# real-stanford/dgdm

Hardware: AMD Instinct MI355X
Metric: guided samples/sec (full DDIM chain) (higher is better)
Workload: dtype f32_split_f16x3; 1 GPU; 3d_guided BASELINE configs[2] (configs[3] at 8 GPUs): B=32 G=45 P=5 R=36000 sub_bs=512 N=512 T=15/S=5, fresh object per pair; contraction_flag=f32, fingers_per_pair=32, denoise_steps=5, rows_per_cond_fn=36000, cond_fn_per_chain_step=1, eps_net_form=f32_f16x3 batched, parallelism=pairs-sharded x1

## Files before the change

### dgdm_amd/_lib.py

```python
from __future__ import annotations

import ctypes as C
import os
from typing import Dict, List, Sequence

import numpy as np
import torch

_HERE = os.path.dirname(os.path.abspath(__file__))
LIB_PATH = os.path.join(_HERE, "csrc", "libdgdm_hip.so")

OK, EINVAL, EKEY, EHIP, EOBJECTIVE, EMODE, ENODEVICE = 0, -1, -2, -3, -4, -5, -6


class DgdmError(RuntimeError):
    pass


class Tensor(C.Structure):
    _fields_ = [("name", C.c_char_p), ("data", C.c_void_p), ("numel", C.c_int64), ("dtype", C.c_int32)]


class Objective(C.Structure):
    _fields_ = [("lin", C.c_float * 3), ("quad", C.c_float * 3), ("use_rowcoef", C.c_int32), ("object", C.c_int32)]


class GoalSpec(C.Structure):
    _fields_ = [("weight", C.c_float * 3), ("ori_window", C.c_float), ("pos_window", C.c_float), ("profile", C.c_int32)]


OBJ_ROWFIELD = 2


class TrainGroups(C.Structure):
    _fields_ = [("t_index_dev", C.c_void_p), ("t_values_dev", C.c_void_p), ("n_t", C.c_int32), ("rows_per_object", C.c_int32)]


class DynamicsStore(C.Structure):
    _fields_ = [("ctrl_dev", C.c_void_p), ("object_dev", C.c_void_p), ("scores_dev", C.c_void_p), ("ori_dev", C.c_void_p), ("pos_dev", C.c_void_p),
                ("object_of_sample_host", C.c_void_p), ("n_samples", C.c_int64), ("n_objects", C.c_int64), ("cells", C.c_int32),
                ("n_ctrl", C.c_int32), ("n_object_points", C.c_int32), ("fingers_3d", C.c_int32)]


class GuidanceConfig(C.Structure):
    _fields_ = [("batch", C.c_int32), ("grid_size", C.c_int32), ("num_pos", C.c_int32), ("ori_lo", C.c_float),
                ("ori_hi", C.c_float), ("max_chains", C.c_int32), ("num_train_timesteps", C.c_int32),
                ("sub_batch_size", C.c_int32), ("num_object_points", C.c_int32), ("max_objects", C.c_int32)]


_P = C.c_void_p
PROTOTYPES = {
    "dgdm_version": (C.c_int, []),
    "dgdm_last_error": (C.c_char_p, []),
    "dgdm_device_init": (C.c_int, [C.c_int]),
    "dgdm_objective_from_name": (C.c_int, [C.c_char_p, C.POINTER(Objective)]),
    "dgdm_unet1d_create": (C.c_int, [C.POINTER(_P), C.POINTER(Tensor), C.c_int, C.POINTER(C.c_int32), C.c_int, C.c_int, C.c_int, C.c_int]),
    "dgdm_unet1d_destroy": (None, [_P]),
    "dgdm_unet1d_forward": (C.c_int, [_P, _P, _P, _P, C.c_int, C.c_int, _P]),
    "dgdm_unet1d_global_cond_dim": (C.c_int, [_P]),
    "dgdm_unet1d_forward_cond": (C.c_int, [_P, _P, _P, _P, _P, C.c_int, C.c_int, _P]),
    "dgdm_cfg_mix": (C.c_int, [_P, _P, C.c_float, _P, C.c_int64, _P]),
    "dgdm_ddim_guided_step": (C.c_int, [_P, _P, _P, C.c_int, _P, C.c_int64, C.c_float, C.c_float, C.c_float, C.c_float, C.c_float, _P]),
    "dgdm_ddim_add_noise": (C.c_int, [_P, _P, _P, C.c_int64, C.c_float, C.c_float, _P]),
    "dgdm_dynamics_create": (C.c_int, [C.POINTER(_P), C.c_int, C.POINTER(Tensor), C.c_int, C.c_int, C.c_int]),
    "dgdm_dynamics_destroy": (None, [_P]),
    "dgdm_dyn2d_forward": (C.c_int, [_P, _P, _P, _P, _P, _P, _P, C.c_int, _P]),
    "dgdm_pointnet2_forward": (C.c_int, [_P, _P, _P, _P, _P, C.c_int, C.c_int, _P]),
    "dgdm_dyn3d_forward": (C.c_int, [_P, _P, _P, _P, _P, _P, _P, _P, _P, C.c_int, C.c_int, _P]),
    "dgdm_farthest_point_sample": (C.c_int, [_P, _P, C.c_int, C.c_int, C.c_int, _P, _P]),
    "dgdm_query_ball_point": (C.c_int, [C.c_float, C.c_int, _P, _P, C.c_int, C.c_int, C.c_int, _P, _P]),
    "dgdm_square_distance": (C.c_int, [_P, _P, C.c_int, C.c_int, C.c_int, _P, _P]),
    "dgdm_index_points": (C.c_int, [_P, _P, C.c_int, C.c_int, C.c_int, C.c_int, _P, _P]),
    "dgdm_linear_act": (C.c_int, [_P, C.c_int, _P, _P, _P, C.c_int, C.c_int, C.c_int, C.c_int, C.c_int, _P]),
    "dgdm_group_max": (C.c_int, [_P, C.c_int64, C.c_int, C.c_int, _P, _P]),
    "dgdm_guidance_create": (C.c_int, [C.POINTER(_P), _P, C.POINTER(GuidanceConfig)]),
    "dgdm_guidance_destroy": (None, [_P]),
    "dgdm_debug_chain_layer": (C.c_int, [_P, _P, _P, _P, _P]),
    "dgdm_unet1d_set_contraction_dtype": (C.c_int, [_P, C.c_int]),
    "dgdm_unet1d_effective_form": (C.c_int, [_P, C.c_int, C.c_int]),
    "dgdm_finger_decode_2d": (C.c_int, [_P, C.c_int, C.c_int, C.c_int, C.c_float, C.c_float, _P, _P]),
    "dgdm_finger_decode_3d": (C.c_int, [_P, C.c_int, C.c_int, C.c_int, C.c_float, C.c_float, _P, _P]),
    "dgdm_guidance_set_contraction_dtype": (C.c_int, [_P, C.c_int]),
    "dgdm_guidance_set_objects": (C.c_int, [_P, _P, C.c_int, _P]),
    "dgdm_guidance_rows": (C.c_int64, [_P]),
    "dgdm_guidance_starts_per_call": (C.c_int64, [_P]),
    "dgdm_dyn2d_guidance_grad": (C.c_int, [_P, _P, C.c_int, C.POINTER(Objective), _P, C.c_int, _P, _P]),
    "dgdm_dyn3d_guidance_grad": (C.c_int, [_P, _P, C.c_int, C.POINTER(Objective), _P, _P, C.c_int, _P, _P]),
    "dgdm_guidance_set_row_field": (C.c_int, [_P, _P, C.c_int, _P]),
    "dgdm_guidance_goal_field": (C.c_int, [_P, _P, C.POINTER(GoalSpec), C.c_int, _P, _P]),
    "dgdm_guidance_score": (C.c_int, [_P, _P, C.c_int, C.POINTER(C.c_int32), _P, C.POINTER(C.c_float), C.c_int, _P, _P, _P, _P]),
    "dgdm_guided_chains_run": (C.c_int, [_P, _P, _P, C.c_int, C.c_int, C.POINTER(Objective), _P, _P, C.POINTER(C.c_int32), C.POINTER(C.c_float),
                                         C.POINTER(C.c_float), C.c_int, _P, _P]),
    "dgdm_guided_chains_run_cond": (C.c_int, [_P, _P, _P, C.c_int, C.c_int, C.POINTER(Objective), _P, _P, C.POINTER(C.c_int32), C.POINTER(C.c_float),
                                              C.POINTER(C.c_float), C.c_int, _P, _P, C.c_int64, C.c_float, _P]),
    "dgdm_guidance_orientation_sweep": (C.c_int, [_P, _P, _P, _P, C.c_int, _P, _P]),
    "dgdm_guidance_rollout": (C.c_int, [_P, _P, C.POINTER(C.c_int32), _P, C.POINTER(C.c_double), C.c_int, C.c_int, _P, _P, _P, _P, _P, _P]),
    "dgdm_guidance_debug_rollout_table": (C.c_int, [_P, C.c_int, _P, _P, C.POINTER(C.c_int32), C.POINTER(C.c_int32), _P]),
    "dgdm_convergence_rowcoef": (C.c_int, [_P, C.c_int, C.c_int, C.c_int, C.c_int64, C.c_int64, _P]),
    "dgdm_torch_rng_seed": (C.c_int, [_P, C.c_int64, C.c_uint64]),
    "dgdm_torch_rng_randint": (C.c_int, [_P, C.c_int64, C.c_uint32, C.c_int64, _P]),
    "dgdm_torch_rng_fps_starts": (C.c_int, [_P, C.c_int64, C.c_int, C.c_int64, C.c_int64, C.c_int64, _P, C.c_int64]),
    "dgdm_prof_enable": (C.c_int, [C.c_int]),
    "dgdm_guidance_debug_fps_path": (C.c_int, [_P, C.c_int, C.POINTER(C.c_int32)]),
    "dgdm_debug_pointnet_indices": (C.c_int, [_P, _P, C.c_int, _P, C.c_int, _P, _P, _P, _P, _P, _P, _P, _P]),
    "dgdm_guidance_debug_partials": (C.c_int, [_P, C.c_int, _P, C.POINTER(C.c_int32), C.POINTER(C.c_int32), _P]),
    "dgdm_prof_read_stage": (C.c_int, [C.c_int, C.POINTER(C.c_int64), C.POINTER(C.c_double), C.POINTER(C.c_double)]),
    "dgdm_prof_read": (C.c_int, [C.POINTER(C.c_int64), C.POINTER(C.c_double), C.POINTER(C.c_double)]),
    "dgdm_trainer2d_create": (C.c_int, [C.POINTER(_P), C.POINTER(Tensor), C.c_int, C.c_int, C.c_int, C.c_float, C.c_float, C.c_float, C.c_float]),
    "dgdm_trainer2d_destroy": (None, [_P]),
    "dgdm_trainer2d_step": (C.c_int, [_P, _P, _P, _P, _P, _P, _P, _P, _P, _P, C.c_int64, C.c_float, C.c_int, _P, C.POINTER(C.c_float), _P]),
    "dgdm_trainer2d_forward_backward": (C.c_int, [_P, _P, _P, _P, _P, _P, _P, _P, _P, _P, C.c_int64, C.c_int64, _P, C.POINTER(C.c_float), _P]),
    "dgdm_trainer2d_set_groups": (C.c_int, [_P, C.POINTER(TrainGroups)]),
    "dgdm_trainer2d_gradient_count": (C.c_int64, [_P]),
    "dgdm_trainer2d_gradients": (C.c_int, [_P, _P, C.c_int64, C.c_int, _P]),
    "dgdm_trainer2d_apply": (C.c_int, [_P, C.c_float, _P]),
    "dgdm_trainer2d_running_stats": (C.c_int, [_P, _P, C.c_int64, C.c_int, _P]),
    "dgdm_trainer2d_export": (C.c_int, [_P, C.c_int, C.POINTER(Tensor), C.c_int]),
    "dgdm_trainer2d_steps": (C.c_int64, [_P]),
    "dgdm_dynamics_batch_rows": (C.c_int, [C.POINTER(DynamicsStore), _P, C.c_int, _P, _P, _P, _P, _P, _P, _P]),
    "dgdm_class_agreement": (C.c_int, [_P, _P, C.c_int64, C.POINTER(C.c_float), _P, _P]),
    "dgdm_unet_trainer_create": (C.c_int, [C.POINTER(_P), C.POINTER(Tensor), C.c_int, C.c_int, C.POINTER(C.c_int32), C.c_int, C.c_int, C.c_int, C.c_int,
                                           C.c_float, C.c_float, C.c_float, C.c_float]),
    "dgdm_unet_trainer_destroy": (None, [_P]),
    "dgdm_unet_trainer_step": (C.c_int, [_P, _P, _P, _P, _P, _P, C.c_int, C.c_float, _P, C.POINTER(C.c_float), _P]),
    "dgdm_unet_trainer_forward_backward": (C.c_int, [_P, _P, _P, _P, _P, _P, C.c_int, C.c_int64, C.c_int, _P, C.POINTER(C.c_float), _P]),
    "dgdm_unet_trainer_step_cond": (C.c_int, [_P, _P, _P, _P, _P, _P, _P, C.c_int, C.c_float, _P, C.POINTER(C.c_float), _P]),
    "dgdm_unet_trainer_forward_backward_cond": (C.c_int, [_P, _P, _P, _P, _P, _P, _P, C.c_int, C.c_int64, C.c_int, _P, C.POINTER(C.c_float), _P]),
    "dgdm_unet_trainer_global_cond_dim": (C.c_int, [_P]),
    "dgdm_unet_trainer_gradient_count": (C.c_int64, [_P]),
    "dgdm_unet_trainer_gradients": (C.c_int, [_P, _P, C.c_int64, C.c_int, C.c_float, _P]),
    "dgdm_unet_trainer_apply": (C.c_int, [_P, C.c_float, _P]),
    "dgdm_unet_trainer_ema_step": (C.c_int, [_P, C.c_float, C.c_float, _P]),
    "dgdm_unet_trainer_export": (C.c_int, [_P, C.c_int, C.POINTER(Tensor), C.c_int]),
    "dgdm_unet_trainer_import": (C.c_int, [_P, C.c_int, C.POINTER(Tensor), C.c_int, C.c_int64]),
    "dgdm_unet_trainer_steps": (C.c_int64, [_P]),
    "dgdm_trainer3d_create": (C.c_int, [C.POINTER(_P), C.POINTER(Tensor), C.c_int, C.c_int, C.c_int, C.c_float, C.c_float, C.c_float, C.c_float]),
    "dgdm_trainer3d_destroy": (None, [_P]),
    "dgdm_trainer3d_step": (C.c_int, [_P, _P, _P, _P, _P, _P, _P, _P, _P, _P, _P, _P, C.c_int64, C.c_float, C.c_int, _P, C.POINTER(C.c_float), _P]),
    "dgdm_trainer3d_export": (C.c_int, [_P, C.c_int, C.POINTER(Tensor), C.c_int]),
    "dgdm_trainer3d_steps": (C.c_int64, [_P]),
    "dgdm_trainer3d_forward_backward": (C.c_int, [_P, _P, _P, _P, _P, _P, _P, _P, _P, _P, _P, _P, C.c_int64, C.c_int64, _P, C.POINTER(C.c_float), _P]),
    "dgdm_trainer3d_gradient_count": (C.c_int64, [_P]),
    "dgdm_trainer3d_gradients": (C.c_int, [_P, _P, C.c_int64, C.c_int, _P]),
    "dgdm_trainer3d_apply": (C.c_int, [_P, C.c_float, _P]),
    "dgdm_trainer3d_running_stats_count": (C.c_int64, [_P]),
    "dgdm_trainer3d_running_stats": (C.c_int, [_P, _P, C.c_int64, C.c_int, _P]),
    "dgdm_trainer3d_debug_read": (C.c_int, [_P, C.c_int, _P, C.c_int64, _P]),
    "dgdm_mesh_read_obj": (C.c_int, [C.c_char_p, C.POINTER(_P)]),
    "dgdm_mesh_num_vertices": (C.c_int64, [_P]),
    "dgdm_mesh_num_triangles": (C.c_int64, [_P]),
    "dgdm_mesh_copy": (C.c_int, [_P, _P, _P]),
    "dgdm_mesh_destroy": (None, [_P]),
    "dgdm_mesh_sample_workspace_bytes": (C.c_int64, [_P, C.c_int]),
    "dgdm_mesh_sample_points": (C.c_int, [_P, _P, _P, _P, C.c_int, C.c_uint64, _P, C.c_int64, _P, _P, C.c_int64, _P]),
    "dgdm_finger_mesh_counts": (C.c_int, [C.c_int, C.c_int, C.POINTER(C.c_int64), C.POINTER(C.c_int64)]),
    "dgdm_finger_mesh_faces": (C.c_int, [C.c_int, C.c_int, _P]),
    "dgdm_finger_mesh_vertices_2d": (C.c_int, [_P, C.c_int, C.c_int, C.c_int, C.c_float, C.c_float, C.c_float, C.c_float, _P, _P]),
    "dgdm_finger_mesh_vertices_3d": (C.c_int, [_P, C.c_int, C.c_int, C.c_int, C.c_float, C.c_float, C.c_float, _P, _P]),
    "dgdm_finger_mesh_stats": (C.c_int, [_P, _P, C.c_int64, C.c_int, C.c_int, C.c_double, _P, _P]),
    "dgdm_finger_pieces_2d": (C.c_int, [_P, C.c_int, C.c_int, C.c_int, _P, _P, _P]),
    "dgdm_finger_pieces_3d": (C.c_int, [_P, C.c_int, C.c_int, C.c_int, C.c_int, _P, _P, _P]),
    "dgdm_mesh_write_obj": (C.c_int, [C.c_char_p, _P, C.c_int64, _P, C.c_int64]),
    "dgdm_icon_workspace_bytes": (C.c_int64, [C.c_int]),
    "dgdm_icon_trace": (C.c_int, [_P, C.c_int, C.c_int, C.c_int, C.c_int, _P, C.c_int64, _P, _P]),
    "dgdm_icon_fetch_contours": (C.c_int, [_P, C.c_int64, C.c_int, _P, _P, _P, C.c_int64, _P]),
    "dgdm_contour_resample_workspace_bytes": (C.c_int64, [_P, C.c_int]),
    "dgdm_contour_resample": (C.c_int, [_P, _P, C.c_int, C.c_int, C.c_int, _P, _P, C.c_int64, _P]),
    "dgdm_polygon_triangulate": (C.c_int, [_P, C.c_int, C.c_int, _P, _P, _P, _P, _P, _P]),
    "dgdm_polygon_convex_pieces": (C.c_int, [_P, C.c_int, C.c_int, _P, _P, _P, _P, _P, _P, _P, _P, _P]),
    "dgdm_render_workspace_bytes": (C.c_int64, [_P, _P, C.c_int, _P, C.c_int, C.c_int]),
    "dgdm_render_meshes": (C.c_int, [_P, _P, _P, _P, C.c_int, _P, _P, _P, _P, _P, _P, C.c_int, C.c_int, C.c_int, C.c_int, _P, _P, _P, _P, _P, _P,
                                     C.c_int64, _P]),
}

_lib = None


def lib() -> C.CDLL:
    global _lib
    if _lib is None:
        if not os.path.exists(LIB_PATH):
            raise DgdmError(f"{LIB_PATH} is missing: the HIP library has not been built (run `python -m dgdm_amd.build`). "
                            "dgdm_amd has no CPU fallback.")
        _lib = C.CDLL(LIB_PATH)
        for name, (res, args) in PROTOTYPES.items():
            fn = getattr(_lib, name)
            fn.restype, fn.argtypes = res, args
    return _lib


def check(rc: int) -> None:
    if rc == OK:
        return
    msg = lib().dgdm_last_error().decode("utf-8", "replace")
    if rc == EOBJECTIVE:
        raise ValueError('opt obj not supported')
    if rc == EMODE:
        raise ValueError('model type not supported')
    raise DgdmError(f"libdgdm_hip error {rc}: {msg}")


def device_init(ordinal: int = 0) -> None:
    check(lib().dgdm_device_init(ordinal))


def stream_ptr() -> int:
    return torch.cuda.current_stream().cuda_stream


def dptr(t: torch.Tensor | None) -> int | None:
    if t is None:
        return None
    assert t.is_cuda and t.is_contiguous(), "device tensors handed to libdgdm_hip must be contiguous CUDA tensors"
    return t.data_ptr()


class PackedStateDict:

    def __init__(self, sd: Dict[str, torch.Tensor], strip_prefix: Sequence[str] = ("module.",)):
        self.keep: List[np.ndarray] = []
        self.names: List[bytes] = []
        items = []
        for k, v in sd.items():
            if not isinstance(v, torch.Tensor):
                continue
            for p in strip_prefix:
                if k.startswith(p):
# ... 16 lines not shown
```

### dgdm_amd/csrc/common.h

```cpp
#pragma once
#include <hip/hip_runtime.h>
#include <stdint.h>
#include <stdio.h>
#include <string>
#include <vector>
#include <map>

#include "../../include/dgdm_hip.h"

#define DGDM_MAX_CHAINS 256

namespace dgdm {

#if defined(__HIP_DEVICE_COMPILE__)
__device__ __forceinline__ float mul_rn(float a, float b) { float r; asm("v_mul_f32 %0, %1, %2" : "=v"(r) : "v"(a), "v"(b)); return r; }
__device__ __forceinline__ float add_rn(float a, float b) { float r; asm("v_add_f32 %0, %1, %2" : "=v"(r) : "v"(a), "v"(b)); return r; }
__device__ __forceinline__ float sub_rn(float a, float b) { float r; asm("v_sub_f32 %0, %1, %2" : "=v"(r) : "v"(a), "v"(b)); return r; }
#else
__device__ __forceinline__ float mul_rn(float a, float b) { return a * b; }
__device__ __forceinline__ float add_rn(float a, float b) { return a + b; }
__device__ __forceinline__ float sub_rn(float a, float b) { return a - b; }
#endif

void set_error(const char *fmt, ...);

#define DGDM_HIP_CHECK(expr)                                                              \
    do {                                                                                  \
        hipError_t _e = (expr);                                                           \
        if (_e != hipSuccess) {                                                           \
            dgdm::set_error("%s failed: %s (%s:%d)", #expr, hipGetErrorString(_e), __FILE__, __LINE__); \
            return DGDM_EHIP;                                                             \
        }                                                                                 \
    } while (0)

#define DGDM_REQUIRE(cond, code, ...)                                                     \
    do {                                                                                  \
        if (!(cond)) {                                                                    \
            dgdm::set_error(__VA_ARGS__);                                                 \
            return (code);                                                                \
        }                                                                                 \
    } while (0)

struct DevBuf {
    void  *p = nullptr;
    size_t bytes = 0;
    DevBuf() = default;
    DevBuf(const DevBuf &) = delete;
    DevBuf &operator=(const DevBuf &) = delete;
    ~DevBuf() { if (p) (void)hipFree(p); }
    int alloc(size_t n) {
        if (p && bytes >= n) return DGDM_OK;
        if (p) { (void)hipFree(p); p = nullptr; bytes = 0; }
        if (n == 0) return DGDM_OK;
        DGDM_HIP_CHECK(hipMalloc(&p, n));
        bytes = n;
        return DGDM_OK;
    }
    int upload(const void *host, size_t n) {
        int rc = alloc(n);
        if (rc) return rc;
        DGDM_HIP_CHECK(hipMemcpy(p, host, n, hipMemcpyHostToDevice));
        return DGDM_OK;
    }
    template <class T> T *as() const { return reinterpret_cast<T *>(p); }
};

struct StateDict {
    std::map<std::string, const DgdmTensor *> m;
    StateDict(const DgdmTensor *t, int n) { for (int i = 0; i < n; ++i) m[t[i].name] = &t[i]; }
    const float *f32(const std::string &k, int64_t numel) const;
    bool has(const std::string &k) const { return m.count(k) != 0; }
};

struct Folded {
    int out = 0, in = 0;
    std::vector<float> w;
    std::vector<float> b;
};
int fold_linear(const StateDict &sd, const std::string &lin, const std::string &bn , int out, int in,
                Folded *dst);
struct Folded64 {
    int out = 0, in = 0;
    std::vector<double> w;
    std::vector<double> b;
};
int fold_linear64(const StateDict &sd, const std::string &lin, const std::string &bn , int out, int in, Folded64 *dst);
std::vector<double> transpose64(const double *src, int rows, int cols);
std::vector<double> pack_mfma64(const double *src, int M, int K);

std::vector<float> pack_chain(const float *src, int M, int K);
uint16_t f32_to_bf16(float x);
std::vector<uint16_t> pack_chain_bf16(const float *src, int M, int K);
std::vector<float> transpose(const float *src, int rows, int cols);

constexpr int PROF_BUCKETS = DGDM_STAGE_COUNT;
void prof_begin(hipStream_t s, int stage);
void prof_end(hipStream_t s, int stage, double work);

}
```

### dgdm_amd/csrc/debug.hip

```cpp
#include "common.h"
#include "mfma_chain.h"
#include "models.h"
#include "smallnet.h"

namespace dgdm {
__global__ __launch_bounds__(64, 1) void debug_chain_kernel(const float4 *__restrict__ Wimg, const float *__restrict__ bias,
                                                           const float *__restrict__ X, float *__restrict__ Y) {
    const int lane = threadIdx.x & 63, n = lane & 31, h4 = (lane >> 5) * 4;
    f32x16 in[8], out[8];
#pragma unroll
    for (int o = 0; o < 8; ++o)
#pragma unroll
        for (int q = 0; q < 4; ++q) {
            const float4 v = feat4(X + n * 256, o, q, h4);
            in[o][4 * q + 0] = v.x; in[o][4 * q + 1] = v.y; in[o][4 * q + 2] = v.z; in[o][4 * q + 3] = v.w;
        }
    chain_layer<8, 8, CHAIN_BIAS>(Wimg, bias, in, out, lane);
#pragma unroll
    for (int o = 0; o < 8; ++o)
#pragma unroll
        for (int q = 0; q < 4; ++q) {
            float4 v;
            v.x = out[o][4 * q + 0]; v.y = out[o][4 * q + 1]; v.z = out[o][4 * q + 2]; v.w = out[o][4 * q + 3];
            *reinterpret_cast<float4 *>(Y + n * 256 + 32 * o + 8 * q + h4) = v;
        }
}
}

extern "C" int dgdm_debug_chain_layer(const float *W_host, const float *bias_host, const float *X_dev, float *Y_dev, void *stream) {
    using namespace dgdm;
    std::vector<float> img = pack_chain(W_host, 256, 256);
    DevBuf dw, db;
    int rc;
    if ((rc = dw.upload(img.data(), img.size() * 4)) || (rc = db.upload(bias_host, 256 * 4))) return rc;
    hipLaunchKernelGGL(debug_chain_kernel, dim3(1), dim3(64), 0, (hipStream_t)stream, dw.as<float4>(), db.as<float>(), X_dev, Y_dev);
    DGDM_HIP_CHECK(hipGetLastError());
    DGDM_HIP_CHECK(hipStreamSynchronize((hipStream_t)stream));
    return DGDM_OK;
}

extern "C" int dgdm_debug_pointnet_indices(DgdmDynamics *m, const float *xyz_dev, int N, const int32_t *perm_dev, int perm_len,
                                           int32_t *fps512_dev, int32_t *fps128_dev, int32_t *fps128_flags_dev, int32_t *ball1_dev,
                                           int32_t *ball2_dev, int32_t *ball2_count_dev, int32_t *crowded_dev, void *stream) {
    using namespace dgdm;
    DGDM_REQUIRE(m && xyz_dev && perm_dev && fps512_dev && fps128_dev && fps128_flags_dev && ball1_dev && ball2_dev && ball2_count_dev && crowded_dev,
                 DGDM_EINVAL, "dgdm_debug_pointnet_indices: null argument");
    if (m->kind != 3) { set_error("model type not supported: PointNet++ belongs to the 3-D model"); return DGDM_EMODE; }
    DGDM_REQUIRE(N >= 128 && N <= 1024 && perm_len > 0 && perm_len <= N, DGDM_EINVAL, "dgdm_debug_pointnet_indices: N %d / perm_len %d unsupported", N, perm_len);
    hipStream_t s = (hipStream_t)stream;
    int rc;
    if ((rc = pn_fps_tables(xyz_dev, N, N, fps512_dev, fps128_dev, fps128_flags_dev, s))) return rc;
    return pn_debug_indices(xyz_dev, N, m->pn(), perm_dev, perm_len, ball1_dev, ball2_dev, ball2_count_dev, crowded_dev, s);
}

extern "C" int dgdm_farthest_point_sample(const float *xyz_dev, const int64_t *start_host, int B, int N, int npoint, int32_t *out_dev, void *stream) {
    using namespace dgdm;
    DGDM_REQUIRE(xyz_dev && start_host && out_dev && B >= 0 && npoint > 0, DGDM_EINVAL, "dgdm_farthest_point_sample: bad argument");
    DGDM_REQUIRE(N > 0 && N <= 1024, DGDM_EINVAL, "clouds of %d points unsupported (1..1024)", N);
    if (B == 0) return DGDM_OK;
    std::vector<int> st(B);
    for (int i = 0; i < B; ++i) {
        DGDM_REQUIRE(start_host[i] >= 0 && start_host[i] < N, DGDM_EINVAL, "FPS start %lld outside [0, %d)", (long long)start_host[i], N);
        st[i] = (int)start_host[i];
    }
    DevBuf d;
    int rc;
    if ((rc = d.upload(st.data(), sizeof(int) * B))) return rc;
    if ((rc = pn_fps_rows(xyz_dev, d.as<int>(), B, N, npoint, out_dev, (hipStream_t)stream))) return rc;
    DGDM_HIP_CHECK(hipStreamSynchronize((hipStream_t)stream));
    return DGDM_OK;
}

extern "C" int dgdm_query_ball_point(float radius_squared, int nsample, const float *xyz_dev, const float *new_xyz_dev, int B, int N, int S, int32_t *out_dev,
                                     void *stream) {
    using namespace dgdm;
    DGDM_REQUIRE(xyz_dev && new_xyz_dev && out_dev && B >= 0 && N > 0 && S >= 0 && nsample > 0, DGDM_EINVAL, "dgdm_query_ball_point: bad argument");
    if (B == 0 || S == 0) return DGDM_OK;
    return pn_ball_rows(xyz_dev, new_xyz_dev, B, N, S, radius_squared, nsample, out_dev, (hipStream_t)stream);
}

extern "C" int dgdm_square_distance(const float *src_dev, const float *dst_dev, int B, int S, int N, float *out_dev, void *stream) {
    using namespace dgdm;
    DGDM_REQUIRE(src_dev && dst_dev && out_dev && B >= 0 && S >= 0 && N >= 0, DGDM_EINVAL, "dgdm_square_distance: bad argument");
    if (B == 0 || S == 0 || N == 0) return DGDM_OK;
    return pn_sqdist_rows(src_dev, dst_dev, B, S, N, out_dev, (hipStream_t)stream);
}

extern "C" int dgdm_index_points(const float *points_dev, const int32_t *idx_dev, int B, int N, int M, int C, float *out_dev, void *stream) {
    using namespace dgdm;
    DGDM_REQUIRE(points_dev && idx_dev && out_dev && B >= 0 && N > 0 && M >= 0 && C > 0, DGDM_EINVAL, "dgdm_index_points: bad argument");
    if (B == 0 || M == 0) return DGDM_OK;
    return pn_index_rows(points_dev, idx_dev, B, N, M, C, out_dev, (hipStream_t)stream);
}


namespace dgdm {
__global__ void group_max_kernel(const float *__restrict__ x, int64_t G, int ns, int C, float *__restrict__ out) {
    const int64_t e = (int64_t)blockIdx.x * blockDim.x + threadIdx.x;
    if (e >= G * C) return;
    const int64_t g = e / C;
    const int c = (int)(e - g * C);
    const float *p = x + g * ns * C + c;
    float best = p[0];
    for (int n = 1; n < ns; ++n) best = fmaxf(best, p[(int64_t)n * C]);
    out[e] = best;
}
}

extern "C" int dgdm_linear_act(const float *x_dev, int ldx, const float *wt_dev, const float *bias_dev, float *y_dev, int ldy, int rows, int K, int N, int act,
                               void *stream) {
    using namespace dgdm;
    DGDM_REQUIRE(x_dev && wt_dev && y_dev && rows >= 0 && K > 0 && N > 0 && ldx >= K && ldy >= N, DGDM_EINVAL, "dgdm_linear_act: bad argument");
    DGDM_REQUIRE(act == ACT_NONE || act == ACT_RELU || act == ACT_SILU, DGDM_EINVAL, "dgdm_linear_act: activation %d", act);
    return linear(x_dev, ldx, wt_dev, bias_dev, nullptr, 1, y_dev, ldy, rows, K, N, act, false, (hipStream_t)stream);
}

extern "C" int dgdm_group_max(const float *x_dev, int64_t groups, int nsample, int C, float *out_dev, void *stream) {
    using namespace dgdm;
    DGDM_REQUIRE(x_dev && out_dev && groups >= 0 && nsample > 0 && C > 0, DGDM_EINVAL, "dgdm_group_max: bad argument");
    if (groups == 0) return DGDM_OK;
    hipLaunchKernelGGL(group_max_kernel, dim3((unsigned)((groups * C + 255) / 256)), dim3(256), 0, (hipStream_t)stream, x_dev, groups, nsample, C, out_dev);
    DGDM_HIP_CHECK(hipGetLastError());
    return DGDM_OK;
}
```

### dgdm_amd/csrc/guidance_api.hip

```cpp
#include "common.h"
#include "models.h"
#include <algorithm>
#include <cmath>
#include <cstring>
#include <unordered_map>
#include <atomic>
#include <thread>

using namespace dgdm;

namespace {

std::vector<float> linspace_f32(float start, float end, int steps) {
    std::vector<float> v(steps);
    if (steps == 1) { v[0] = start; return v; }
    const float step = (end - start) / (float)(steps - 1);
    const int half = steps / 2;
    for (int i = 0; i < steps; ++i) v[i] = i < half ? start + step * (float)i : end - step * (float)(steps - i - 1);
    return v;
}

struct ObjectTables {
    const float *xyz = nullptr;
    const int   *fps1 = nullptr;
    const int   *fps2 = nullptr;
    const int   *flags = nullptr;
    DevBuf Z;
    bool   fast_ok = false;
    int *crowded = nullptr, *clist = nullptr;
    DevBuf M0, cl2, cnt2;
    DevBuf cl2s;
    DevBuf cl2o;
    DevBuf pcf;
    DevBuf X, X16;
    bool   has_x = false, has_x16 = false;
    int    ncr = 0;
    DevBuf Z16, M0_16;
    bool   has16 = false;
};

struct PoseGrid {
    DevBuf tab, tiled;
    DevBuf pmax;
    int cells = 0, tiles_per_b = 0;
    int64_t rows = 0;
};

}

struct DgdmGuidance {
    DgdmDynamics *m = nullptr;
    DgdmGuidanceConfig cfg{};
    int B = 0;
    PoseGrid grid, sweep;
    DevBuf objpart;
    DevBuf objtmp;
    std::vector<std::unique_ptr<ObjectTables>> tables;
    bool bf16 = false;
    bool f32_mfma = false;
    static constexpr int NBUILD = 3;
    DevBuf pool_crowded, pool_clist, pool_off, pool_pairs, pool_rank, pool_F1, pool_U;
    DevBuf pool_xyz, pool_fps1, pool_fps2, pool_flags, pool_ncr;
    DevBuf tmpY[NBUILD], tmpL2[NBUILD], vlist;
    DevBuf tmpShare[NBUILD];
    hipStream_t bstream[NBUILD] = {};
    hipEvent_t bev[NBUILD] = {}, bstart = nullptr, pooled = nullptr, ldone = nullptr;
    DevBuf V, genc, atab, chainbias, timepart, ttmp, ttmp64, partial, objdev, objidx, xobj, xobj16, starts, order, xchains, todo, groupoff;
    DevBuf loopx[2], loopeps, loopgrad, loopxrep, loopts;
    DevBuf loopcond, loopx2, loopeps2;
    DevBuf scorelogits;
    DevBuf sweep_ori, rollstate, rolllogits, rolltiles, rollpmax;
    const float *rowfield = nullptr;
    int rowfield_chains = 0;
    DevBuf pos_lin, goalspecs;
    int rolltiles_chains = 0;
    DevBuf xidx, xidxchains, xtabptrs;
    bool xtab_enabled = true;
    int xtab_policy = 0;
    int grads_since_set = 0;
    static constexpr int XTAB_AFTER = 5;
    int l2_gather_mode = 0;
    int xobj_mode = 0;
    int n_objects = 0;
    bool force_slow_xobj = false;
    void *pinned = nullptr; size_t pinned_bytes = 0; hipEvent_t pinned_ev = nullptr;
    int64_t todo_capacity = 0;
    int *ro_host = nullptr; size_t ro_ints = 0; hipEvent_t ro_ev = nullptr; bool ro_pending = false;
    int finish_objects();
    hipStream_t cstream = nullptr; hipEvent_t up_ready = nullptr, up_consumed = nullptr; bool consumed_recorded = false;
    ~DgdmGuidance() {
        if (pinned) (void)hipHostFree(pinned);
        if (pinned_ev) (void)hipEventDestroy(pinned_ev);
        if (ro_host) (void)hipHostFree(ro_host);
        if (ro_ev) (void)hipEventDestroy(ro_ev);
        if (cstream) (void)hipStreamDestroy(cstream);
        if (up_ready) (void)hipEventDestroy(up_ready);
        if (up_consumed) (void)hipEventDestroy(up_consumed);
        for (int i = 0; i < NBUILD; ++i) {
            if (bstream[i]) (void)hipStreamDestroy(bstream[i]);
            if (bev[i]) (void)hipEventDestroy(bev[i]);
        }
        if (bstart) (void)hipEventDestroy(bstart);
        if (ldone) (void)hipEventDestroy(ldone);
        if (pooled) (void)hipEventDestroy(pooled);
    }
    int build_pose_table(const std::vector<float> &ori, const std::vector<float> &pos, PoseGrid *dst, hipStream_t s);
    void set_grid(dgdm::TrunkParams *p, const PoseGrid &g, int n_chains) const;
    int check_objects(const int *oidx, int n_chains) const;
    bool tables_wanted() const { return xtab_enabled && !force_slow_xobj && xobj_mode == 0; }
    int common_pre(const float *x_dev, float t_scaled, const int *objidx_host, int n_chains, hipStream_t s);
    int upload_starts(const int64_t *starts_host, int n_chains, int64_t rows, hipStream_t s, bool need_order = true, int n_calls = 1,
                      int64_t call_stride = 0);
    int ensure_rows(int n_chains, int64_t rows_per_chain);
    int use_xtab(const int *objidx_host, int n_chains, int64_t rows, bool want16, hipStream_t s);
    int build_object(int oi, int slot, hipStream_t s);
    int build_xtab(int oi, hipStream_t s);
    int run_xobj(const int *objidx_host, int n_chains, int64_t rows, bool want16, bool *used16, bool *via_tab, hipStream_t s);
    struct Embedded {
        bool tab = false, used16 = false;
        int64_t rows_per_chain = 0;
        void point(dgdm::TrunkParams *p, const DgdmGuidance &g, int call, int64_t rows_per_call) const;
    };
    int embed_rows(const int *objidx_host, int n_chains, const int64_t *starts_host, int64_t rows_per_call, int n_calls, int64_t call_stride,
                   bool want16, Embedded *e, hipStream_t s);
    int embed(const int *objidx_host, int n_chains, const int64_t *starts_host, int n_calls, int64_t call_stride, Embedded *e, hipStream_t s);
    int trunk_front(int kind, const float *x_dev, int timestep, const int *objidx_host, const int64_t *starts_host, int n_chains, const Embedded *emb,
                    int call, dgdm::TrunkParams *p, hipStream_t s);
};

int DgdmGuidance::build_pose_table(const std::vector<float> &ori, const std::vector<float> &pos, PoseGrid *dst, hipStream_t s) {
    const int n = (int)ori.size(), W1 = m->W1;
    dst->cells = n; dst->tiles_per_b = (n + 31) / 32; dst->rows = (int64_t)B * n;
    DevBuf d_ori, d_pos, d_emb;
    int rc;
    if ((rc = d_ori.upload(ori.data(), sizeof(float) * n))) return rc;
    if ((rc = d_pos.upload(pos.data(), sizeof(float) * 2 * n))) return rc;
    if ((rc = d_emb.alloc(sizeof(float) * 27 * n))) return rc;
    if ((rc = dst->tab.alloc(sizeof(float) * (size_t)W1 * n))) return rc;
    if ((rc = pose_embed(d_ori.as<float>(), d_pos.as<float>(), d_emb.as<float>(), n, s))) return rc;
    if ((rc = linear64(d_emb.as<float>(), nullptr, 27, m->blob64.at(m->off64.w1p_wt), nullptr, nullptr, 1, nullptr, dst->tab.as<float>(), W1, n, 27, W1, ACT_NONE, s))) return rc;
    if ((rc = dst->tiled.alloc(sizeof(float) * (size_t)W1 * dst->tiles_per_b * 32))) return rc;
    if ((rc = tile_table(dst->tab.as<float>(), n, W1, dst->tiled.as<float>(), s))) return rc;
    DGDM_HIP_CHECK(hipStreamSynchronize(s));
    return DGDM_OK;
}

void DgdmGuidance::set_grid(TrunkParams *p, const PoseGrid &g, int n_chains) const {
    p->Atab = atab.as<float>(); p->Ptab = g.tab.as<float>(); p->PtabT = g.tiled.as<float>(); p->Pmax = g.pmax.as<float>();
    p->B = B; p->C = g.cells; p->tiles_per_b = g.tiles_per_b; p->ntiles = n_chains * B * g.tiles_per_b; p->R = g.rows;
    p->xstride = g.rows;
}

int DgdmGuidance::check_objects(const int *oidx, int n_chains) const {
    DGDM_REQUIRE(n_objects > 0, DGDM_EINVAL, "dgdm_guidance_set_objects has not been called");
    for (int i = 0; i < n_chains; ++i)
        DGDM_REQUIRE(oidx[i] >= 0 && oidx[i] < n_objects, DGDM_EINVAL, "chain %d refers to object %d of %d", i, oidx[i], n_objects);
    return DGDM_OK;
}

extern "C" int dgdm_guidance_create(DgdmGuidance **out, DgdmDynamics *model, const DgdmGuidanceConfig *cfg) {
    DGDM_REQUIRE(out && model && cfg, DGDM_EINVAL, "dgdm_guidance_create: null argument");
    DGDM_REQUIRE(cfg->batch > 0 && cfg->grid_size > 0 && cfg->num_pos > 0 && cfg->max_chains > 0 && cfg->num_train_timesteps > 0,
                 DGDM_EINVAL, "dgdm_guidance_create: bad config");
    DGDM_REQUIRE(cfg->max_chains <= DGDM_MAX_CHAINS, DGDM_EINVAL, "max_chains %d > %d", cfg->max_chains, DGDM_MAX_CHAINS);
    if (model->kind == 3) {
        DGDM_REQUIRE(cfg->sub_batch_size > 0, DGDM_EINVAL, "3-D guidance needs sub_batch_size (it partitions the FPS start draws)");
        DGDM_REQUIRE(cfg->num_object_points > 0 && cfg->num_object_points <= 1024, DGDM_EINVAL, "object clouds of %d points unsupported (1..1024)", cfg->num_object_points);
    } else {
        DGDM_REQUIRE(2 * cfg->num_object_points == model->object_ch, DGDM_EINVAL, "2*num_object_points (%d) != object_ch (%d)", 2 * cfg->num_object_points, model->object_ch);
    }
    std::unique_ptr<DgdmGuidance> g(new DgdmGuidance());
    g->m = model; g->cfg = *cfg;
    g->B = cfg->batch;
    const int G = cfg->grid_size, P = cfg->num_pos, C = G * P * P;
    const std::vector<float> lo = linspace_f32(cfg->ori_lo, cfg->ori_hi, G), lp = linspace_f32(-1.f, 1.f, P);
    std::vector<float> ori(C), pos(2 * (size_t)C);
    for (int gi = 0; gi < G; ++gi)
        for (int a = 0; a < P; ++a)
            for (int b = 0; b < P; ++b) {
                const int c = (gi * P + a) * P + b;
                ori[c] = lo[gi]; pos[2 * c] = lp[a]; pos[2 * c + 1] = lp[b];
            }
    int rc;
    if ((rc = g->build_pose_table(ori, pos, &g->grid, nullptr))) return rc;
    {
        std::vector<float> tab((size_t)C * model->W1), mx(C, 0.f);
        DGDM_HIP_CHECK(hipMemcpy(tab.data(), g->grid.tab.p, tab.size() * sizeof(float), hipMemcpyDeviceToHost));
        for (int c = 0; c < C; ++c)
            for (int j = 0; j < model->W1; ++j) mx[c] = std::max(mx[c], std::fabs(tab[(size_t)c * model->W1 + j]));
        if ((rc = g->grid.pmax.upload(mx.data(), mx.size() * sizeof(float)))) return rc;
    }
    std::vector<float> pos0(2 * (size_t)G, 0.f);
    if ((rc = g->build_pose_table(lo, pos0, &g->sweep, nullptr))) return rc;
    if ((rc = g->sweep_ori.upload(lo.data(), lo.size() * sizeof(float)))) return rc;
    if ((rc = g->pos_lin.upload(lp.data(), lp.size() * sizeof(float)))) return rc;
    const int W1 = model->W1, nc = cfg->max_chains;
    const size_t rows = (size_t)nc * g->B;
    const int64_t R = g->grid.rows;
    if ((rc = g->V.alloc(rows * 256 * 8)) || (rc = g->genc.alloc(rows * 256 * 8)) || (rc = g->atab.alloc(rows * W1 * 4)) ||
        (rc = g->chainbias.alloc((size_t)nc * W1 * 8)) || (rc = g->timepart.alloc((size_t)W1 * 8)) || (rc = g->ttmp.alloc(768 * 4)) ||
        (rc = g->ttmp64.alloc(512 * 8)) ||
        (rc = g->partial.alloc(rows * g->grid.tiles_per_b * W1 * 4)) || (rc = g->objdev.alloc(sizeof(TrunkObjective) * nc)) ||
        (rc = g->objidx.alloc(sizeof(int) * nc)))
        return rc;
    if (model->kind == 2) {
        if ((rc = g->objpart.alloc((size_t)std::max(1, cfg->max_objects) * W1 * 8))) return rc;
    } else {
        if ((rc = g->starts.alloc((size_t)nc * R * 2 * sizeof(int))) ||
            (rc = g->order.alloc((size_t)nc * R * sizeof(int))) || (rc = g->xchains.alloc(sizeof(XobjChain) * nc)) ||
            (rc = g->todo.alloc(((size_t)nc * R + 1) * sizeof(int))))
            return rc;
        g->todo_capacity = (int64_t)nc * R;
        g->pinned_bytes = ((size_t)nc * R * 3 + (size_t)nc * (cfg->num_object_points + 1)) * sizeof(int);
        if ((rc = g->groupoff.alloc((size_t)nc * (cfg->num_object_points + 1) * sizeof(int))) || (rc = g->xidx.alloc((size_t)nc * R * sizeof(int))) ||
            (rc = g->xidxchains.alloc(sizeof(XidxChain) * nc)) || (rc = g->xtabptrs.alloc(sizeof(void *) * nc)))
            return rc;
        DGDM_HIP_CHECK(hipHostMalloc(&g->pinned, g->pinned_bytes, hipHostMallocDefault));
        DGDM_HIP_CHECK(hipEventCreateWithFlags(&g->pinned_ev, hipEventDisableTiming));
    }
    *out = g.release();
    return DGDM_OK;
}

extern "C" void dgdm_guidance_destroy(DgdmGuidance *g) { delete g; }

extern "C" int dgdm_guidance_set_contraction_dtype(DgdmGuidance *g, int dtype) {
    DGDM_REQUIRE(g, DGDM_EINVAL, "dgdm_guidance_set_contraction_dtype: null handle");
    DGDM_REQUIRE(dtype >= DGDM_DTYPE_F32 && dtype <= DGDM_DTYPE_F32_F16X3, DGDM_EINVAL,
                 "contraction dtype %d unsupported (0 = f32 (default form), 1 = bf16, 2 = f32 on the float32 MFMA, 3 = f32 as 3 f16 products = the default form)", dtype);
    g->bf16 = dtype == DGDM_DTYPE_BF16;
    g->f32_mfma = dtype == DGDM_DTYPE_F32_MFMA;
    return DGDM_OK;
}

extern "C" int dgdm_guidance_debug_fps_path(DgdmGuidance *g, int force_per_row, int32_t *out_fast_ok) {
    DGDM_REQUIRE(g, DGDM_EINVAL, "dgdm_guidance_debug_fps_path: null handle");
    g->force_slow_xobj = force_per_row == 1;
    g->xobj_mode = force_per_row == 2 ? 2 : 0;
    g->l2_gather_mode = force_per_row == 4 ? 1 : 0;
    g->xtab_enabled = force_per_row == 0 || force_per_row == 4 || force_per_row == 5;
    g->xtab_policy = force_per_row == 5 ? 1 : 0;
    if (force_per_row == 3) g->xobj_mode = 0;
    if (out_fast_ok) {
        int rc = g->finish_objects();
        if (rc) return rc;
        for (int i = 0; i < g->n_objects && i < (int)g->tables.size(); ++i) out_fast_ok[i] = g->tables[i]->fast_ok ? 1 : 0;
    }
    return DGDM_OK;
}
__global__ void partials_true_units_kernel(float *p, const float *unit, size_t n, int W1) {
    const size_t i = (size_t)blockIdx.x * blockDim.x + threadIdx.x;
    if (i < n) p[i] *= unit[i % W1];
}
extern "C" int dgdm_guidance_debug_partials(DgdmGuidance *g, int n_chains, float *out_dev, int32_t *tiles_per_finger, int32_t *width, void *stream) {
    DGDM_REQUIRE(g && n_chains > 0 && n_chains <= g->cfg.max_chains, DGDM_EINVAL, "dgdm_guidance_debug_partials: bad argument");
    if (tiles_per_finger) *tiles_per_finger = g->grid.tiles_per_b;
    if (width) *width = g->m->W1;
    if (out_dev) {
        const size_t n = (size_t)n_chains * g->B * g->grid.tiles_per_b * g->m->W1;
        DGDM_HIP_CHECK(hipMemcpyAsync(out_dev, g->partial.p, n * sizeof(float), hipMemcpyDeviceToDevice, (hipStream_t)stream));
        hipLaunchKernelGGL(partials_true_units_kernel, dim3((unsigned)((n + 255) / 256)), dim3(256), 0, (hipStream_t)stream, out_dev, g->m->z1_unit.as<float>(), n, g->m->W1);
        DGDM_HIP_CHECK(hipGetLastError());
    }
    return DGDM_OK;
}
extern "C" int64_t dgdm_guidance_rows(const DgdmGuidance *g) { return g ? g->grid.rows : 0; }
extern "C" int64_t dgdm_guidance_starts_per_call(const DgdmGuidance *g) { return (g && g->m->kind == 3) ? 2 * g->grid.rows : 0; }

int DgdmGuidance::build_object(int oi, int slot, hipStream_t s) {
    const int N = cfg.num_object_points;
    ObjectTables &t = *tables[oi];
    const PnWeights w = m->pn();
    int rc;
    if ((rc = t.Z.alloc((size_t)N * N * 256 * 4)) ||
        (rc = t.M0.alloc((size_t)N * 256 * 4)) || (rc = t.cl2.alloc((size_t)N * 128 * sizeof(int))) || (rc = t.cnt2.alloc((size_t)N * sizeof(int))) ||
        (rc = t.cl2s.alloc((size_t)N * 128 * sizeof(int))) || (rc = t.cl2o.alloc((size_t)N * 256 * sizeof(unsigned short))) ||
        (rc = t.pcf.alloc((size_t)N * 512 * sizeof(int))))
        return rc;
    t.has16 = bf16;
    if (bf16 && ((rc = t.Z16.alloc((size_t)N * N * 128 * 4)) || (rc = t.M0_16.alloc((size_t)N * 128 * 4)))) return rc;
    uint32_t *z16 = bf16 ? t.Z16.as<uint32_t>() : nullptr;
    DevBuf &tY = tmpY[slot], &tL2 = tmpL2[slot];
    if ((rc = tY.alloc((size_t)N * N * 256 * 4)) || (rc = tL2.alloc((size_t)N * N * 256 * 4))) return rc;
    const float *xyz = t.xyz;
    const int *off = pool_off.as<int>() + (size_t)oi * (N + 1), *pairs = pool_pairs.as<int>() + (size_t)oi * N * N;
    const short *rank = pool_rank.as<short>() + (size_t)oi * N * N;
    const char *U = static_cast<const char *>(pool_U.p) + (size_t)oi * N * 128 * (bf16 ? 4 : 8);
    if (bf16) {
        if ((rc = pn_pairs(xyz, N, reinterpret_cast<const float *>(U), w, pairs, off, tY.as<float>(), tY.as<uint32_t>(), s))) return rc;
        if ((rc = pn_l2(xyz, N, w, t.fps1, vlist.as<int>(), N, tY.as<float>(), tL2.as<float>(), t.clist, t.clist + N,
                        off, rank, true, s, l2_gather_mode ? 0 : 1))) return rc;
        if ((rc = pn_z16(xyz, N, N, w, tL2.as<uint32_t>(), t.Z.as<float>(), z16, t.clist, t.clist + N, s))) return rc;
    } else {
        const PnWeights64 w64 = m->pn64();
        if ((rc = pn_pairs64(xyz, N, reinterpret_cast<const double *>(U), w64, pairs, off, tY.as<float>(), s))) return rc;
        const bool shared = !l2_gather_mode && N <= 512;
        L2Share sh{};
        if (shared) {
            const size_t NN = (size_t)N * N;
            if ((rc = tmpShare[slot].alloc(NN * 64 + NN + NN * sizeof(short) + NN * sizeof(int) + (2 * (size_t)N + 4) * sizeof(int)))) return rc;
            char *b = static_cast<char *>(tmpShare[slot].p);
            sh.sel = reinterpret_cast<unsigned char *>(b); b += NN * 64;
            sh.items = reinterpret_cast<int *>(b); b += NN * sizeof(int);
            sh.coff = reinterpret_cast<int *>(b); b += N * sizeof(int);
            sh.ccnt = reinterpret_cast<int *>(b); b += N * sizeof(int);
            sh.nitems = reinterpret_cast<int *>(b); b += 4 * sizeof(int);
            sh.rep = reinterpret_cast<short *>(b); b += NN * sizeof(short);
            sh.cnt = reinterpret_cast<unsigned char *>(b);
        }
        if ((rc = pn_l2(xyz, N, w, t.fps1, vlist.as<int>(), N, tY.as<float>(), tL2.as<float>(), t.clist, t.clist + N,
                        off, rank, false, s, shared ? 1 : 0, shared ? &sh : nullptr))) return rc;
        if ((rc = pn_z64(xyz, N, N, w64, tL2.as<float>(), t.Z.as<float>(), t.clist, t.clist + N, s, sh.items, sh.nitems))) return rc;
        if (shared && N > 1 && (rc = pn_zfill(N, N, t.Z.as<float>(), t.clist, t.clist + N, sh.rep, s))) return rc;
    }
    if ((rc = pn_m0(t.fps2, t.crowded, N, t.Z.as<float>(), t.M0.as<float>(), t.cl2.as<int>(), t.cnt2.as<int>(), z16,
                    bf16 ? t.M0_16.as<uint32_t>() : nullptr, t.clist, t.clist + N, t.cl2s.as<int>(), t.cl2o.as<unsigned short>(), s))) return rc;
    if ((rc = pn_pcf(t.fps1, t.cnt2.as<int>(), t.flags, N, t.pcf.as<int>(), s))) return rc;
    t.has_x = t.has_x16 = false;
    return xtab_policy == 1 ? build_xtab(oi, s) : DGDM_OK;
}

int DgdmGuidance::build_xtab(int oi, hipStream_t s) {
    const int N = cfg.num_object_points;
    ObjectTables &t = *tables[oi];
    if (N < 128) return DGDM_OK;
    const bool b16 = t.has16;
    int rc;
    if (b16) { if ((rc = t.X16.alloc((size_t)N * N * 128 * 4))) return rc; }
    else if ((rc = t.X.alloc((size_t)N * N * 256 * 4))) return rc;
    XtabObj xo{};
    xo.xyz = t.xyz; xo.fps1 = t.fps1; xo.Z = t.Z.as<float>(); xo.M0 = t.M0.as<float>();
    xo.Z16 = b16 ? t.Z16.as<uint32_t>() : nullptr; xo.M0_16 = b16 ? t.M0_16.as<uint32_t>() : nullptr;
    xo.clist = t.clist; xo.ncr = t.clist + N; xo.cl2s = t.cl2s.as<int>(); xo.cnt2 = t.cnt2.as<int>(); xo.flags = t.flags;
    xo.crowded = t.crowded; xo.X = b16 ? nullptr : t.X.as<float>(); xo.X16 = b16 ? t.X16.as<uint32_t>() : nullptr; xo.N = N;
    if ((rc = pn_xtab(xo, b16, s))) return rc;
    (b16 ? t.has_x16 : t.has_x) = true;
    return DGDM_OK;
}

extern "C" int dgdm_guidance_set_objects(DgdmGuidance *g, const float *objects_dev, int n_objects, void *stream) {
    DGDM_REQUIRE(g && objects_dev && n_objects > 0, DGDM_EINVAL, "dgdm_guidance_set_objects: bad argument");
    DGDM_REQUIRE(n_objects <= std::max(1, g->cfg.max_objects), DGDM_EINVAL, "%d objects > max_objects %d", n_objects, g->cfg.max_objects);
    hipStream_t s = (hipStream_t)stream;
    int rc;
    prof_begin(s, DGDM_STAGE_TABLES);
    if (g->m->kind == 2) {
        if ((rc = g->objtmp.alloc((size_t)n_objects * 512 * 8))) return rc;
        if ((rc = g->m->object_part_2d64(objects_dev, g->objtmp.as<double>(), g->objpart.as<double>(), n_objects, s))) return rc;
        prof_end(s, DGDM_STAGE_TABLES, 0.0);
    } else {
        while ((int)g->tables.size() < n_objects) g->tables.emplace_back(new ObjectTables());
        const int N = g->cfg.num_object_points;
        if (g->vlist.bytes < (size_t)N * sizeof(int)) {
            std::vector<int> v(N);
            for (int i = 0; i < N; ++i) v[i] = i;
            if ((rc = g->vlist.upload(v.data(), sizeof(int) * N))) return rc;
        }
        const int nb = std::min<int>(DgdmGuidance::NBUILD, n_objects);
        if (!g->bstart) DGDM_HIP_CHECK(hipEventCreateWithFlags(&g->bstart, hipEventDisableTiming));
        if (!g->ldone) DGDM_HIP_CHECK(hipEventCreateWithFlags(&g->ldone, hipEventDisableTiming));
        for (int i = 0; i < nb; ++i) {
            if (!g->bstream[i]) DGDM_HIP_CHECK(hipStreamCreateWithFlags(&g->bstream[i], hipStreamNonBlocking));
            if (!g->bev[i]) DGDM_HIP_CHECK(hipEventCreateWithFlags(&g->bev[i], hipEventDisableTiming));
        }
        const size_t no = (size_t)n_objects;
        if ((rc = g->pool_xyz.alloc(no * N * 3 * 4)) || (rc = g->pool_fps1.alloc(no * N * 512 * sizeof(int))) ||
            (rc = g->pool_fps2.alloc(no * N * 128 * sizeof(int))) || (rc = g->pool_flags.alloc(no * N * sizeof(int))) ||
            (rc = g->pool_ncr.alloc(no * sizeof(int))) || (rc = g->pool_crowded.alloc(no * N * sizeof(int))) ||
            (rc = g->pool_clist.alloc(no * (N + 1) * sizeof(int))) || (rc = g->pool_off.alloc(no * (N + 1) * sizeof(int))) ||
            (rc = g->pool_pairs.alloc(no * N * N * sizeof(int))) || (rc = g->pool_rank.alloc(no * N * N * sizeof(short))) ||
            (rc = g->pool_F1.alloc(no * N * 128 * 8)) || (rc = g->pool_U.alloc(no * N * 128 * 8)))
            return rc;
        if (!g->pooled) DGDM_HIP_CHECK(hipEventCreateWithFlags(&g->pooled, hipEventDisableTiming));
        DGDM_HIP_CHECK(hipMemcpyAsync(g->pool_xyz.p, objects_dev, no * N * 3 * 4, hipMemcpyDeviceToDevice, s));
        DGDM_HIP_CHECK(hipEventRecord(g->pooled, s));
        if ((rc = pn_fps_tables(g->pool_xyz.as<float>(), N, N, g->pool_fps1.as<int>(), g->pool_fps2.as<int>(), g->pool_flags.as<int>(), s, n_objects)))
            return rc;
        for (int i = 0; i < n_objects; ++i) {
            ObjectTables &t = *g->tables[i];
            t.xyz = g->pool_xyz.as<float>() + (size_t)i * N * 3; t.fps1 = g->pool_fps1.as<int>() + (size_t)i * N * 512;
            t.fps2 = g->pool_fps2.as<int>() + (size_t)i * N * 128; t.flags = g->pool_flags.as<int>() + (size_t)i * N;
            t.crowded = g->pool_crowded.as<int>() + (size_t)i * N; t.clist = g->pool_clist.as<int>() + (size_t)i * (N + 1);
        }
        {
            hipStream_t ls = g->bstream[0];
            DGDM_HIP_CHECK(hipStreamWaitEvent(ls, g->pooled, 0));
            const PnWeights w = g->m->pn();
            if ((rc = pn_crowd(g->pool_xyz.as<float>(), N, w, g->pool_crowded.as<int>(), g->pool_clist.as<int>(), g->pool_clist.as<int>() + N,
                               g->pool_off.as<int>(), g->pool_pairs.as<int>(), g->pool_rank.as<short>(), ls, g->pool_ncr.as<int>(), n_objects)))
                return rc;
            if (g->bf16) {
                if ((rc = pn_sa1(g->pool_xyz.as<float>(), N, w, g->pool_F1.as<float>(), ls, n_objects))) return rc;
                if ((rc = linear(g->pool_F1.as<float>(), 128, w.sa2_wf_t, w.sa2_b0, nullptr, 1, g->pool_U.as<float>(), 128, n_objects * N, 128, 128,
                                 ACT_NONE, false, ls))) return rc;
            } else {
                const PnWeights64 w64 = g->m->pn64();
                if ((rc = pn_sa1_64(g->pool_xyz.as<float>(), N, w.r1sq, w64, g->pool_F1.as<double>(), ls, n_objects))) return rc;
                if ((rc = linear64(nullptr, g->pool_F1.as<double>(), 128, w64.sa2_wf_t, w64.sa2_b0, nullptr, 1, g->pool_U.as<double>(), nullptr, 128,
                                   n_objects * N, 128, 128, ACT_NONE, ls))) return rc;
            }
            DGDM_HIP_CHECK(hipEventRecord(g->ldone, ls));
        }
        DGDM_HIP_CHECK(hipEventRecord(g->bstart, s));
        for (int i = 0; i < nb; ++i) {
            DGDM_HIP_CHECK(hipStreamWaitEvent(g->bstream[i], g->bstart, 0));
            DGDM_HIP_CHECK(hipStreamWaitEvent(g->bstream[i], g->ldone, 0));
        }
        for (int i = 0; i < n_objects; ++i)
            if ((rc = g->build_object(i, i % nb, g->bstream[i % nb]))) return rc;
        for (int i = 0; i < nb; ++i) {
            DGDM_HIP_CHECK(hipEventRecord(g->bev[i], g->bstream[i]));
            DGDM_HIP_CHECK(hipStreamWaitEvent(s, g->bev[i], 0));
        }
        prof_end(s, DGDM_STAGE_TABLES, 0.0);
        const size_t need = no * N + no;
        if (need > g->ro_ints) {
            if (g->ro_host) DGDM_HIP_CHECK(hipHostFree(g->ro_host));
            g->ro_host = nullptr;
            DGDM_HIP_CHECK(hipHostMalloc(reinterpret_cast<void **>(&g->ro_host), need * sizeof(int), hipHostMallocDefault));
            g->ro_ints = need;
        }
        if (!g->ro_ev) DGDM_HIP_CHECK(hipEventCreateWithFlags(&g->ro_ev, hipEventDisableTiming));
        DGDM_HIP_CHECK(hipMemcpyAsync(g->ro_host, g->pool_flags.p, sizeof(int) * no * N, hipMemcpyDeviceToHost, s));
        DGDM_HIP_CHECK(hipMemcpyAsync(g->ro_host + no * N, g->pool_ncr.p, sizeof(int) * no, hipMemcpyDeviceToHost, s));
        DGDM_HIP_CHECK(hipEventRecord(g->ro_ev, s));
        g->ro_pending = true;
    }
    g->n_objects = n_objects;
    g->grads_since_set = 0;
    return DGDM_OK;
}

int DgdmGuidance::common_pre(const float *x_dev, float t_scaled, const int *objidx_host, int n_chains, hipStream_t s) {
    const int rows = n_chains * B, W1 = m->W1;
    int rc;
    if ((rc = m->gripper_forward64(x_dev, m->L, V.as<double>(), genc.as<double>(), rows, s))) return rc;
    if ((rc = m->time_part64(t_scaled, ttmp.as<float>(), ttmp64.as<double>(), timepart.as<double>(), s))) return rc;
    if (m->kind == 2) {
        DGDM_HIP_CHECK(hipMemcpyAsync(objidx.p, objidx_host, sizeof(int) * n_chains, hipMemcpyHostToDevice, s));
        if ((rc = gather_add64(objpart.as<double>(), objidx.as<int>(), timepart.as<double>(), chainbias.as<double>(), n_chains, W1, s))) return rc;
        return linear64(nullptr, genc.as<double>(), 256, m->blob64.at(m->off64.w1c_wt), nullptr, chainbias.as<double>(), B, nullptr, atab.as<float>(), W1, rows, 256, W1,
                        ACT_NONE, s);
    }
    return linear64(nullptr, genc.as<double>(), 256, m->blob64.at(m->off64.w1c_wt), timepart.as<double>(), nullptr, 1, nullptr, atab.as<float>(), W1, rows, 256, W1,
                    ACT_NONE, s);
}

int DgdmGuidance::finish_objects() {
    if (!ro_pending) return DGDM_OK;
    DGDM_HIP_CHECK(hipEventSynchronize(ro_ev));
    const int N = cfg.num_object_points;
    for (int i = 0; i < n_objects; ++i) {
        bool ok = N >= 128;
        for (int k = 0; k < N; ++k) ok = ok && ro_host[(size_t)i * N + k] == 0;
        tables[i]->fast_ok = ok;
        tables[i]->ncr = ro_host[(size_t)n_objects * N + i];
    }
    ro_pending = false;
    return DGDM_OK;
}

int DgdmGuidance::ensure_rows(int n_chains, int64_t rows_per_chain) {
    const int N = cfg.num_object_points;
    const size_t nr = (size_t)n_chains * rows_per_chain;
    int rc;
    if ((rc = starts.alloc(nr * 2 * sizeof(int))) || (rc = order.alloc(nr * sizeof(int))) ||
        (rc = todo.alloc((nr + 1) * sizeof(int))) || (rc = xidx.alloc(nr * sizeof(int))))
        return rc;
    todo_capacity = (int64_t)nr;
    const size_t need = (nr * 3 + (size_t)n_chains * (N + 1)) * sizeof(int);
    if (need > pinned_bytes) {
        if (pinned) { DGDM_HIP_CHECK(hipEventSynchronize(pinned_ev)); DGDM_HIP_CHECK(hipHostFree(pinned)); pinned = nullptr; pinned_bytes = 0; }
        DGDM_HIP_CHECK(hipHostMalloc(&pinned, need, hipHostMallocDefault));
        pinned_bytes = need;
    }
    return DGDM_OK;
}

int DgdmGuidance::upload_starts(const int64_t *starts_host, int n_chains, int64_t rows, hipStream_t s, bool need_order, int n_calls,
                                int64_t call_stride) {
    const int N = cfg.num_object_points;
    const int64_t sb = cfg.sub_batch_size;
    const int64_t rt = rows * n_calls;
    int rc;
    DGDM_REQUIRE(!need_order || rt < ((int64_t)1 << 22), DGDM_EINVAL, "%lld rows per chain in one gather launch (limit 4194303)", (long long)rt);
    if ((rc = ensure_rows(n_chains, rt))) return rc;
    DGDM_HIP_CHECK(hipEventSynchronize(pinned_ev));
    int *dst = static_cast<int *>(pinned);
    int *ord = dst + (size_t)n_chains * 2 * rt;
    int *goff = ord + (size_t)n_chains * rt;
    std::atomic<int> bad{0};
    auto work = [&](int c0, int c1) {
        std::vector<int> cnt(N + 1), cnt2(513), tmp;
        for (int c = c0; c < c1; ++c) {
            int *d = dst + (size_t)c * 2 * rt;
            for (int k = 0; k < n_calls; ++k) {
                const int64_t *src = starts_host + (size_t)k * call_stride + (size_t)c * 2 * rows;
                int *dk = d + 2 * (size_t)k * rows;
                for (int64_t r0 = 0; r0 < rows; r0 += sb) {
                    const int64_t n = std::min(sb, rows - r0);
                    const int64_t *s1 = src + 2 * r0, *s2 = s1 + n;
                    for (int64_t i = 0; i < n; ++i) {
                        const int64_t a = s1[i], b = s2[i];
                        if (!(a >= 0 && a < N && b >= 0 && b < 512)) { bad.store(1); return; }
                        dk[2 * (r0 + i)] = (int)a; dk[2 * (r0 + i) + 1] = (int)b;
                    }
                }
            }
            if (!need_order) continue;
            int *o = ord + (size_t)c * rt;
            tmp.resize((size_t)rt);
            std::fill(cnt2.begin(), cnt2.end(), 0);
            for (int64_t r = 0; r < rt; ++r) ++cnt2[d[2 * r + 1] + 1];
            for (int k = 0; k < 512; ++k) cnt2[k + 1] += cnt2[k];
            for (int64_t r = 0; r < rt; ++r) tmp[cnt2[d[2 * r + 1]]++] = (int)r;
            std::fill(cnt.begin(), cnt.end(), 0);
            for (int64_t r = 0; r < rt; ++r) ++cnt[d[2 * r] + 1];
            for (int k = 0; k < N; ++k) cnt[k + 1] += cnt[k];
            memcpy(goff + (size_t)c * (N + 1), cnt.data(), sizeof(int) * (N + 1));
            for (int64_t i = 0; i < rt; ++i) { const int r = tmp[i]; o[cnt[d[2 * r]]++] = r | (d[2 * r + 1] << 22); }
        }
    };
    const int hw = (int)std::max(2u, std::thread::hardware_concurrency());
    const int nthreads = (int)std::min<int64_t>(std::min(16, hw / 2), std::max<int64_t>(1, std::min<int64_t>(n_chains, (int64_t)n_chains * rt / 65536)));
    if (nthreads <= 1) {
        work(0, n_chains);
    } else {
        std::vector<std::thread> pool;
        for (int t = 0; t < nthreads; ++t) pool.emplace_back(work, (int)((int64_t)n_chains * t / nthreads), (int)((int64_t)n_chains * (t + 1) / nthreads));
        for (auto &th : pool) th.join();
    }
    DGDM_REQUIRE(!bad.load(), DGDM_EINVAL, "FPS start out of range (sa1 must be in [0, %d), sa2 in [0, 512))", N);
    if (!cstream) {
        DGDM_HIP_CHECK(hipStreamCreateWithFlags(&cstream, hipStreamNonBlocking));
        DGDM_HIP_CHECK(hipEventCreateWithFlags(&up_ready, hipEventDisableTiming));
        DGDM_HIP_CHECK(hipEventCreateWithFlags(&up_consumed, hipEventDisableTiming));
    }
    if (consumed_recorded) DGDM_HIP_CHECK(hipStreamWaitEvent(cstream, up_consumed, 0));
    DGDM_HIP_CHECK(hipMemcpyAsync(starts.p, pinned, (size_t)n_chains * rt * 2 * sizeof(int), hipMemcpyHostToDevice, cstream));
    if (need_order) {
        DGDM_HIP_CHECK(hipMemcpyAsync(order.p, ord, (size_t)n_chains * rt * sizeof(int), hipMemcpyHostToDevice, cstream));
        DGDM_HIP_CHECK(hipMemcpyAsync(groupoff.p, goff, (size_t)n_chains * (N + 1) * sizeof(int), hipMemcpyHostToDevice, cstream));
    }
    DGDM_HIP_CHECK(hipEventRecord(pinned_ev, cstream));
    DGDM_HIP_CHECK(hipEventRecord(up_ready, cstream));
    DGDM_HIP_CHECK(hipStreamWaitEvent(s, up_ready, 0));
    return DGDM_OK;
}

int DgdmGuidance::use_xtab(const int *objidx_host, int n_chains, int64_t rows, bool want16, hipStream_t s) {
    std::vector<XidxChain> xc(n_chains);
    std::vector<const void *> base(n_chains);
    for (int i = 0; i < n_chains; ++i) {
        const ObjectTables &t = *tables[objidx_host[i]];
        xc[i].fps1 = t.fps1; xc[i].N = cfg.num_object_points; xc[i].m0_only = t.ncr == 0;
        base[i] = want16 ? (t.ncr == 0 ? (const void *)t.M0_16.p : (const void *)t.X16.p) : (t.ncr == 0 ? (const void *)t.M0.p : (const void *)t.X.p);
    }
    DGDM_HIP_CHECK(hipMemcpyAsync(xidxchains.p, xc.data(), sizeof(XidxChain) * n_chains, hipMemcpyHostToDevice, s));
    DGDM_HIP_CHECK(hipMemcpyAsync(xtabptrs.p, base.data(), sizeof(void *) * n_chains, hipMemcpyHostToDevice, s));
    return pn_xidx(xidxchains.as<XidxChain>(), starts.as<int>(), rows, n_chains, xidx.as<int>(), s);
}

int DgdmGuidance::run_xobj(const int *objidx_host, int n_chains, int64_t rows, bool want16, bool *used16, bool *via_tab, hipStream_t s) {
    *via_tab = false;
    std::vector<XobjChain> ch(n_chains);
    for (int i = 0; i < n_chains; ++i) {
        const ObjectTables &t = *tables[objidx_host[i]];
        ch[i].xyz = t.xyz; ch[i].fps1 = t.fps1; ch[i].slot_of_start = nullptr; ch[i].Z = t.Z.as<float>();
        ch[i].fps2 = t.fps2; ch[i].flags = t.flags; ch[i].crowded = t.crowded; ch[i].N = cfg.num_object_points;
        ch[i].M0 = t.M0.as<float>(); ch[i].cl2 = t.cl2.as<int>(); ch[i].cnt2 = t.cnt2.as<int>();
        ch[i].Z16 = t.has16 ? t.Z16.as<uint32_t>() : nullptr; ch[i].M0_16 = t.has16 ? t.M0_16.as<uint32_t>() : nullptr;
        want16 = want16 && t.has16;
    }
    {
        const size_t nrows = (size_t)n_chains * rows;
        int rc = want16 ? xobj16.alloc(nrows * 512) : xobj.alloc(nrows * 256 * 4);
        if (rc) return rc;
    }
    *used16 = want16;
    XobjParams xp{};
    xp.chains = xchains.as<XobjChain>(); xp.starts = starts.as<int>(); xp.order = order.as<int>(); xp.xobj = xobj.as<float>();
    xp.xobj16 = want16 ? xobj16.as<uint32_t>() : nullptr;
    xp.R = rows; xp.total_rows = rows * n_chains; xp.use_table = force_slow_xobj ? 0 : 1;
    xp.todo = todo.as<int>(); xp.todo_count = todo.as<int>() + todo_capacity; xp.todo_capacity = todo_capacity;
    bool all_fast = true;
    for (int i = 0; i < n_chains; ++i) all_fast = all_fast && tables[objidx_host[i]]->fast_ok;
    bool groups = !force_slow_xobj && xobj_mode == 0 && cfg.num_object_points >= 128;
    for (int i = 0; i < n_chains && groups; ++i) {
        const ObjectTables &t = *tables[objidx_host[i]];
        const int lpr = xobj_rows_lpr(t.ncr, want16);
        groups = lpr > 0 && want16 == t.has16;
        ch[i].clist = t.clist; ch[i].cl2s = t.cl2s.as<int>(); ch[i].cl2o = t.cl2o.as<unsigned short>(); ch[i].pcf = t.pcf.as<int>(); ch[i].ncr = t.ncr; ch[i].lpr = lpr;
    }
    DGDM_HIP_CHECK(hipMemcpyAsync(xchains.p, ch.data(), sizeof(XobjChain) * n_chains, hipMemcpyHostToDevice, s));
    if (groups) {
        const bool by_index = tables_wanted() && (want16 || !bf16);
        std::vector<int> rank;
        std::vector<XidxChain> xc(n_chains);
        std::vector<const void *> base(n_chains);
        for (int i = 0; i < n_chains; ++i) {
            const ObjectTables &t = *tables[objidx_host[i]];
            const bool m0_only = by_index && t.ncr == 0 && t.fast_ok;
            if (!m0_only) rank.push_back(i);
            xc[i].fps1 = m0_only ? t.fps1 : nullptr; xc[i].N = cfg.num_object_points; xc[i].m0_only = 1;
            base[i] = m0_only ? (want16 ? (const void *)t.M0_16.p : (const void *)t.M0.p)
                              : (want16 ? (const void *)(xobj16.as<uint32_t>() + (size_t)i * rows * 128) : (const void *)(xobj.as<float>() + (size_t)i * rows * 256));
        }
        xp.group_off = groupoff.as<int>(); xp.nchain = n_chains; xp.group_N = cfg.num_object_points; xp.use_table = 1;
        xp.total_items = (int)rank.size() * xp.group_N;
        std::stable_sort(rank.begin(), rank.end(), [&](int a, int b) { return ch[a].ncr > ch[b].ncr; });
        for (size_t i = 0; i < rank.size(); ++i) xp.chain_of_rank[i] = (unsigned char)rank[i];
        int rc = pn_xobj_groups(xp, s);
        if (rc || !by_index) return rc;
        *via_tab = true;
        DGDM_HIP_CHECK(hipMemcpyAsync(xidxchains.p, xc.data(), sizeof(XidxChain) * n_chains, hipMemcpyHostToDevice, s));
        DGDM_HIP_CHECK(hipMemcpyAsync(xtabptrs.p, base.data(), sizeof(void *) * n_chains, hipMemcpyHostToDevice, s));
        return pn_xidx(xidxchains.as<XidxChain>(), starts.as<int>(), rows, n_chains, xidx.as<int>(), s);
    }
    return pn_xobj(xp, all_fast, s);
}

int DgdmGuidance::embed_rows(const int *oidx, int n_chains, const int64_t *starts_host, int64_t rows_per_call, int n_calls, int64_t call_stride,
                             bool want16, Embedded *e, hipStream_t s) {
    bool tab = tables_wanted();
    for (int i = 0; i < n_chains && tab; ++i) tab = want16 ? tables[oidx[i]]->has_x16 : tables[oidx[i]]->has_x;
    const int64_t rt = rows_per_call * n_calls;
    int rc;
    if ((rc = upload_starts(starts_host, n_chains, rows_per_call, s, !tab, n_calls, call_stride))) return rc;
    if ((rc = finish_objects())) return rc;
    e->tab = tab; e->used16 = want16; e->rows_per_chain = rt;
    if ((rc = tab ? use_xtab(oidx, n_chains, rt, want16, s) : run_xobj(oidx, n_chains, rt, want16, &e->used16, &e->tab, s))) return rc;
    DGDM_HIP_CHECK(hipEventRecord(up_consumed, s));
    consumed_recorded = true;
    return DGDM_OK;
}

void DgdmGuidance::Embedded::point(TrunkParams *p, const DgdmGuidance &g, int call, int64_t rows_per_call) const {
    const size_t row0 = (size_t)call * rows_per_call;
    p->xstride = rows_per_chain;
    if (tab) {
        p->xidx = g.xidx.as<int>() + row0;
        if (used16) p->xtab16 = g.xtabptrs.as<const uint32_t *>();
        else p->xtab = g.xtabptrs.as<const float *>();
    } else {
        p->xobj = g.xobj.as<float>() + row0 * 256;
        p->xobj16 = used16 ? g.xobj16.as<uint32_t>() + row0 * 128 : nullptr;
    }
}

int DgdmGuidance::embed(const int *oidx, int n_chains, const int64_t *starts_host, int n_calls, int64_t call_stride, Embedded *e, hipStream_t s) {
    DGDM_REQUIRE(starts_host, DGDM_EINVAL, "3-D guidance needs the FPS start indices");
    int rc;
    prof_begin(s, DGDM_STAGE_XOBJ);
    if (tables_wanted()) {
        const bool crosses = grads_since_set <= XTAB_AFTER && grads_since_set + n_calls > XTAB_AFTER;
        grads_since_set += n_calls;
        if (crosses)
            for (int i = 0; i < n_objects; ++i) {
                ObjectTables &t = *tables[i];
                if (!(t.has16 ? t.has_x16 : t.has_x) && (rc = build_xtab(i, s))) return rc;
            }
    }
    if ((rc = embed_rows(oidx, n_chains, starts_host, grid.rows, n_calls, call_stride, bf16, e, s))) return rc;
    prof_end(s, DGDM_STAGE_XOBJ, 0.0);
    return DGDM_OK;
}

int DgdmGuidance::trunk_front(int kind, const float *x_dev, int timestep, const int *oidx, const int64_t *starts_host, int n_chains, const Embedded *emb,
                              int call, TrunkParams *pp, hipStream_t s) {
    const float t_scaled = (float)timestep / (float)cfg.num_train_timesteps;
    int rc;
    if ((rc = check_objects(oidx, n_chains))) return rc;
    prof_begin(s, DGDM_STAGE_GUIDE_MISC);
    if ((rc = common_pre(x_dev, t_scaled, oidx, n_chains, s))) return rc;
    prof_end(s, DGDM_STAGE_GUIDE_MISC, 0.0);
    m->fill_trunk(pp);
    set_grid(pp, grid, n_chains);
    if (kind == 3) {
        Embedded own;
        if (!emb) {
            if ((rc = embed(oidx, n_chains, starts_host, 1, 0, &own, s))) return rc;
            emb = &own;
            call = 0;
        }
        emb->point(pp, *this, call, grid.rows);
    }
    return DGDM_OK;
}

static int check_objectives(const DgdmGuidance *g, const DgdmObjective *objectives, const float *rowcoef_dev, int n_chains) {
    for (int i = 0; i < n_chains; ++i) {
        const int u = objectives[i].use_rowcoef;
        DGDM_REQUIRE(u >= 0 && u <= DGDM_OBJ_ROWFIELD, DGDM_EINVAL, "chain %d: use_rowcoef %d (0, 1 or %d)", i, u, DGDM_OBJ_ROWFIELD);
        DGDM_REQUIRE(u != 1 || rowcoef_dev, DGDM_EINVAL, "chain %d uses rowcoef but rowcoef_dev is null", i);
        if (u == DGDM_OBJ_ROWFIELD) {
            DGDM_REQUIRE(g->rowfield, DGDM_EINVAL, "chain %d uses the row field but none is set (dgdm_guidance_set_row_field)", i);
            DGDM_REQUIRE(i < g->rowfield_chains, DGDM_EINVAL, "chain %d uses the row field, which was set for %d chains", i, g->rowfield_chains);
        }
    }
    return DGDM_OK;
}

static int guidance_grad(DgdmGuidance *g, int kind, const float *x_dev, int timestep, const DgdmObjective *objectives, const float *rowcoef_dev,
                         const int64_t *starts_host, int n_chains, float *grad_dev, hipStream_t s, const DgdmGuidance::Embedded *emb = nullptr,
                         int call = 0) {
    DGDM_REQUIRE(g && x_dev && objectives && grad_dev, DGDM_EINVAL, "guidance_grad: null argument");
    if (g->m->kind != kind) { set_error("model type not supported: %d-D entry point on a %d-D model", kind, g->m->kind); return DGDM_EMODE; }
    DGDM_REQUIRE(n_chains > 0 && n_chains <= g->cfg.max_chains, DGDM_EINVAL, "n_chains %d outside 1..%d", n_chains, g->cfg.max_chains);
    int rc;
    if ((rc = check_objectives(g, objectives, rowcoef_dev, n_chains))) return rc;
    std::vector<int> oidx(n_chains);
    std::vector<TrunkObjective> tob(n_chains);
    for (int i = 0; i < n_chains; ++i) {
        oidx[i] = objectives[i].object;
        for (int j = 0; j < 3; ++j) { tob[i].lin[j] = objectives[i].lin[j]; tob[i].quad[j] = objectives[i].quad[j]; }
        tob[i].use_rowcoef = objectives[i].use_rowcoef; tob[i].pad = 0;
    }
    TrunkParams p;
    if ((rc = g->trunk_front(kind, x_dev, timestep, oidx.data(), starts_host, n_chains, emb, call, &p, s))) return rc;
    DGDM_HIP_CHECK(hipMemcpyAsync(g->objdev.p, tob.data(), sizeof(TrunkObjective) * n_chains, hipMemcpyHostToDevice, s));
    p.obj = g->objdev.as<TrunkObjective>(); p.rowcoef = rowcoef_dev; p.rowfield = g->rowfield;
    p.partial = g->partial.as<float>();
    if (g->bf16) {
        g->m->fill_trunk_bf16(&p);
        if ((rc = trunk_bf16_launch(kind, p, s))) return rc;
    } else if (g->f32_mfma) {
        if ((rc = trunk_launch(kind, false, false, p, s))) return rc;
    } else {
        TrunkF16Scales sc;
        g->m->fill_trunk_f16(&p, &sc);
        if ((rc = trunk_f16l_launch(kind, TrunkF16Mode::Grad, p, sc, s))) return rc;
    }
    prof_begin(s, DGDM_STAGE_GUIDE_MISC);
    rc = dyn_post64(g->m->W1, g->partial.as<float>(), g->grid.tiles_per_b, g->m->blob64.at(g->m->off64.w1c_w), g->m->blob64.at(g->m->off64.g2_w),
                    g->m->blob64.at(g->m->off64.g0_w), g->V.as<double>(), grad_dev, n_chains * g->B, g->m->L, s);
    prof_end(s, DGDM_STAGE_GUIDE_MISC, 0.0);
    return rc;
}

extern "C" int dgdm_dyn2d_guidance_grad(DgdmGuidance *g, const float *x_dev, int timestep, const DgdmObjective *objectives,
                                        const float *rowcoef_dev, int n_chains, float *grad_dev, void *stream) {
    return guidance_grad(g, 2, x_dev, timestep, objectives, rowcoef_dev, nullptr, n_chains, grad_dev, (hipStream_t)stream);
}

extern "C" int dgdm_dyn3d_guidance_grad(DgdmGuidance *g, const float *x_dev, int timestep, const DgdmObjective *objectives,
                                        const float *rowcoef_dev, const int64_t *starts_host, int n_chains, float *grad_dev, void *stream) {
    return guidance_grad(g, 3, x_dev, timestep, objectives, rowcoef_dev, starts_host, n_chains, grad_dev, (hipStream_t)stream);
}

extern "C" int dgdm_guidance_set_row_field(DgdmGuidance *g, const float *field_dev, int n_chains, void *stream) {
    (void)stream;
    DGDM_REQUIRE(g, DGDM_EINVAL, "dgdm_guidance_set_row_field: null handle");
    if (!field_dev) { g->rowfield = nullptr; g->rowfield_chains = 0; return DGDM_OK; }
    DGDM_REQUIRE(n_chains > 0 && n_chains <= g->cfg.max_chains, DGDM_EINVAL, "dgdm_guidance_set_row_field: n_chains %d outside 1..%d", n_chains,
                 g->cfg.max_chains);
    g->rowfield = field_dev; g->rowfield_chains = n_chains;
    return DGDM_OK;
}

extern "C" int dgdm_guidance_goal_field(DgdmGuidance *g, const float *goals_dev, const DgdmGoalSpec *specs_host, int n_chains, float *field_dev,
                                        void *stream) {
    DGDM_REQUIRE(g && goals_dev && specs_host && field_dev, DGDM_EINVAL, "dgdm_guidance_goal_field: null argument");
    DGDM_REQUIRE(n_chains > 0 && n_chains <= g->cfg.max_chains, DGDM_EINVAL, "dgdm_guidance_goal_field: n_chains %d outside 1..%d", n_chains,
                 g->cfg.max_chains);
    hipStream_t s = (hipStream_t)stream;
    for (int i = 0; i < n_chains; ++i) {
        const DgdmGoalSpec &q = specs_host[i];
        DGDM_REQUIRE(q.ori_window > 0.f && q.ori_window <= 1.f, DGDM_EINVAL, "goal %d: ori_window %g outside (0, 1]", i, (double)q.ori_window);
        DGDM_REQUIRE(q.pos_window > 0.f && std::isfinite(q.pos_window), DGDM_EINVAL, "goal %d: pos_window %g is not a positive number", i, (double)q.pos_window);
        DGDM_REQUIRE(q.profile == 0 || q.profile == 1, DGDM_EINVAL, "goal %d: profile %d (0 sign, 1 linear)", i, q.profile);
        for (int j = 0; j < 3; ++j) DGDM_REQUIRE(std::isfinite(q.weight[j]), DGDM_EINVAL, "goal %d: weight %d is not finite", i, j);
    }
    std::vector<float> goals((size_t)n_chains * g->B * 3);
    DGDM_HIP_CHECK(hipMemcpyAsync(goals.data(), goals_dev, goals.size() * sizeof(float), hipMemcpyDeviceToHost, s));
    DGDM_HIP_CHECK(hipStreamSynchronize(s));
    for (size_t k = 0; k < goals.size(); ++k)
        DGDM_REQUIRE(std::isfinite(goals[k]), DGDM_EINVAL, "goal %d, finger %d: coordinate %d is not finite", (int)(k / ((size_t)g->B * 3)),
                     (int)(k / 3 % g->B), (int)(k % 3));
    int rc;
    if ((rc = g->goalspecs.alloc(sizeof(DgdmGoalSpec) * g->cfg.max_chains))) return rc;
    DGDM_HIP_CHECK(hipMemcpyAsync(g->goalspecs.p, specs_host, sizeof(DgdmGoalSpec) * n_chains, hipMemcpyHostToDevice, s));
    return goal_field_build(g->sweep_ori.as<float>(), g->pos_lin.as<float>(), goals_dev, g->goalspecs.as<DgdmGoalSpec>(), n_chains, g->B,
                            g->cfg.grid_size, g->cfg.num_pos, field_dev, s);
}

extern "C" int dgdm_guidance_score(DgdmGuidance *g, const float *x_dev, int timestep, const int32_t *object_of_chain, const int64_t *starts_host,
                                   const float thr[3], int n_chains, float *logits_dev, int32_t *counts_dev, float *sums_dev, void *stream) {
    DGDM_REQUIRE(g && x_dev && object_of_chain && thr && counts_dev && sums_dev, DGDM_EINVAL, "dgdm_guidance_score: null argument");
    DGDM_REQUIRE(!g->bf16, DGDM_EINVAL, "dgdm_guidance_score: the bf16 trunk has no forward-only form (contraction dtypes f32 / f32_f16x3 / f32_mfma)");
    hipStream_t s = (hipStream_t)stream;
    const int kind = g->m->kind;
    DGDM_REQUIRE(kind == 2 || starts_host, DGDM_EINVAL, "3-D scoring needs the FPS start indices");
    DGDM_REQUIRE(n_chains > 0 && n_chains <= g->cfg.max_chains, DGDM_EINVAL, "n_chains %d outside 1..%d", n_chains, g->cfg.max_chains);
    int rc;
    if (!logits_dev) {
        if ((rc = g->scorelogits.alloc((size_t)n_chains * g->grid.rows * 3 * sizeof(float)))) return rc;
        logits_dev = g->scorelogits.as<float>();
    }
    const std::vector<int> oidx(object_of_chain, object_of_chain + n_chains);
    TrunkParams p;
    if ((rc = g->trunk_front(kind, x_dev, timestep, oidx.data(), starts_host, n_chains, nullptr, 0, &p, s))) return rc;
    p.logits = logits_dev;
    if (g->f32_mfma) {
        if ((rc = trunk_launch(kind, false, true, p, s))) return rc;
    } else {
        TrunkF16Scales sc;
        g->m->fill_trunk_f16(&p, &sc);
        if ((rc = trunk_f16l_launch(kind, TrunkF16Mode::Forward, p, sc, s))) return rc;
    }
    return score_tally(logits_dev, n_chains, g->B, g->grid.cells, thr, counts_dev, sums_dev, s);
}

namespace {
__global__ void fill_i32_kernel(int *p, int v, int n) {
    const int i = blockIdx.x * blockDim.x + threadIdx.x;
    if (i < n) p[i] = v;
}
__global__ void repeat_rows_kernel(const float *__restrict__ src, float *__restrict__ dst, int64_t n_src, int reps) {
    const int64_t i = (int64_t)blockIdx.x * blockDim.x + threadIdx.x;
    if (i < n_src * reps) dst[i] = src[i % n_src];
}
__global__ void cfg_mix_kernel(const float *ec, const float *eu, float w, float *out, int64_t n) {
    const int64_t i = (int64_t)blockIdx.x * blockDim.x + threadIdx.x;
    if (i >= n) return;
    const float u = eu[i];
    out[i] = add_rn(u, mul_rn(w, sub_rn(ec[i], u)));
}
}

extern "C" int dgdm_cfg_mix(const float *eps_c_dev, const float *eps_u_dev, float w, float *out_dev, int64_t numel, void *stream) {
    DGDM_REQUIRE(eps_c_dev && eps_u_dev && out_dev && numel >= 0, DGDM_EINVAL, "dgdm_cfg_mix: bad argument");
    if (numel == 0) return DGDM_OK;
    hipLaunchKernelGGL(cfg_mix_kernel, dim3((unsigned)((numel + 255) / 256)), dim3(256), 0, (hipStream_t)stream, eps_c_dev, eps_u_dev, w, out_dev, numel);
    DGDM_HIP_CHECK(hipGetLastError());
    return DGDM_OK;
}

extern "C" int dgdm_guided_chains_run(DgdmUnet1d *unet, DgdmGuidance *g, const float *noise_dev, int n_chains, int n_grad,
                                      const DgdmObjective *objectives, const float *rowcoef_dev, const int64_t *starts_host,
                                      const int32_t *timesteps, const float *coef, const float *scales, int n_steps, float *x_out_dev,
                                      void *stream) {
    return dgdm_guided_chains_run_cond(unet, g, noise_dev, n_chains, n_grad, objectives, rowcoef_dev, starts_host, timesteps, coef, scales, n_steps, x_out_dev,
                                       nullptr, 0, 1.f, stream);
}

extern "C" int dgdm_guided_chains_run_cond(DgdmUnet1d *unet, DgdmGuidance *g, const float *noise_dev, int n_chains, int n_grad,
                                           const DgdmObjective *objectives, const float *rowcoef_dev, const int64_t *starts_host,
                                           const int32_t *timesteps, const float *coef, const float *scales, int n_steps, float *x_out_dev,
                                           const float *global_cond_dev, int64_t cond_chain_stride, float cfg_weight, void *stream) {
    DGDM_REQUIRE(unet && g && noise_dev && objectives && timesteps && coef && scales && x_out_dev, DGDM_EINVAL, "dgdm_guided_chains_run: null argument");
    DGDM_REQUIRE(n_chains > 0 && n_grad > 0 && n_chains * n_grad <= g->cfg.max_chains && n_steps > 0, DGDM_EINVAL,
                 "dgdm_guided_chains_run: %d chains x %d gradients outside 1..%d", n_chains, n_grad, g->cfg.max_chains);
    hipStream_t s = (hipStream_t)stream;
    const int B = g->B, L = g->m->L, kind = g->m->kind;
    const size_t per_chain = (size_t)B * L, nx = per_chain * n_chains, ng = nx * n_grad;
    DGDM_REQUIRE(kind == 2 || starts_host, DGDM_EINVAL, "3-D guidance needs the FPS start indices");
    const int gc = dgdm_unet1d_global_cond_dim(unet);
    DGDM_REQUIRE(gc == 0 || global_cond_dev, DGDM_EINVAL, "dgdm_guided_chains_run: the eps-net has global_cond_dim %d and needs a condition", gc);
    DGDM_REQUIRE(cfg_weight == cfg_weight && std::fabs(cfg_weight) <= 3.0e38f, DGDM_EINVAL, "dgdm_guided_chains_run: cfg_weight is not finite");
    const bool conditional = gc > 0;
    DGDM_REQUIRE(!conditional || cond_chain_stride == 0 || cond_chain_stride == (int64_t)B * gc, DGDM_EINVAL,
                 "dgdm_guided_chains_run: cond_chain_stride %lld is neither 0 (one [B][%d] block for all chains) nor B * gc = %lld", (long long)cond_chain_stride, gc,
                 (long long)B * gc);
    const bool per_chain_cond = conditional && cond_chain_stride != 0 && n_chains > 1;
    const int cfg = !conditional ? 1 : cfg_weight == 1.f ? 1 : cfg_weight == 0.f ? 0 : 2;
    int rc;
    if ((rc = check_objectives(g, objectives, rowcoef_dev, n_chains * n_grad))) return rc;
    if ((rc = g->loopx[0].alloc(nx * 4)) || (rc = g->loopx[1].alloc(nx * 4)) || (rc = g->loopeps.alloc(nx * 4)) || (rc = g->loopgrad.alloc(ng * 4)) ||
        (rc = g->loopxrep.alloc(ng * 4)) || (rc = g->loopts.alloc((size_t)2 * n_chains * B * sizeof(int))))
        return rc;
    const size_t ncond = (size_t)n_chains * B * gc;
    const float *cond_rows = nullptr, *zero_rows = nullptr;
    if (conditional) {
        if ((rc = g->loopcond.alloc(2 * ncond * 4))) return rc;
        float *cr = g->loopcond.as<float>();
        if (cond_chain_stride == 0) hipLaunchKernelGGL(repeat_rows_kernel, dim3((unsigned)((ncond + 255) / 256)), dim3(256), 0, s, global_cond_dev, cr, (int64_t)B * gc, n_chains);
        else DGDM_HIP_CHECK(hipMemcpyAsync(cr, global_cond_dev, ncond * 4, hipMemcpyDeviceToDevice, s));
        DGDM_HIP_CHECK(hipMemsetAsync(cr + ncond, 0, ncond * 4, s));
        cond_rows = cr; zero_rows = cr + ncond;
        if (cfg == 2 && ((rc = g->loopx2.alloc(2 * nx * 4)) || (rc = g->loopeps2.alloc(2 * nx * 4)))) return rc;
    }
    hipLaunchKernelGGL(repeat_rows_kernel, dim3((unsigned)((nx + 255) / 256)), dim3(256), 0, s, noise_dev, g->loopx[0].as<float>(), (int64_t)per_chain, n_chains);
    bool same_scale = true;
    for (int c = 1; c < n_chains; ++c) same_scale = same_scale && scales[c] == scales[0];
    const int64_t spc = kind == 3 ? 2 * g->grid.rows : 0;
    DgdmGuidance::Embedded emb;
    std::vector<int> oidx(n_chains * n_grad);
    const int64_t call_stride = (int64_t)n_chains * n_grad * spc;
    int cpe = kind == 3 ? (int)std::min<int64_t>(n_steps, std::max<int64_t>(1, (((int64_t)1 << 22) - 1) / std::max<int64_t>(1, g->grid.rows))) : n_steps;
    if (const char *e = getenv("DGDM_EMBED_CALLS")) cpe = std::max(1, std::min(cpe, atoi(e)));
    if (kind == 3) {
        for (int i = 0; i < n_chains * n_grad; ++i) oidx[i] = objectives[i].object;
        if ((rc = g->check_objects(oidx.data(), n_chains * n_grad))) return rc;
    }
    for (int si = 0; si < n_steps; ++si) {
        float *x = g->loopx[si & 1].as<float>(), *xn = (si + 1 == n_steps) ? x_out_dev : g->loopx[(si + 1) & 1].as<float>();
        const int t = timesteps[si];
        if (kind == 3 && si % cpe == 0 &&
            (rc = g->embed(oidx.data(), n_chains * n_grad, starts_host + (size_t)si * call_stride, std::min(cpe, n_steps - si), call_stride, &emb, s))) return rc;
        const int nb = (si == 0 && n_chains > 1 && !per_chain_cond) ? B : n_chains * B;
        const int ne = cfg == 2 ? 2 * nb : nb;
        hipLaunchKernelGGL(fill_i32_kernel, dim3((ne + 255) / 256), dim3(256), 0, s, g->loopts.as<int>(), t, ne);
        if (cfg == 2) {
            const size_t n = (size_t)nb * L, nc = (size_t)nb * gc;
            float *x2 = g->loopx2.as<float>(), *e2 = g->loopeps2.as<float>(), *c2 = g->loopcond.as<float>();
            DGDM_HIP_CHECK(hipMemcpyAsync(x2, x, n * 4, hipMemcpyDeviceToDevice, s));
            DGDM_HIP_CHECK(hipMemcpyAsync(x2 + n, x, n * 4, hipMemcpyDeviceToDevice, s));
            if (nc != ncond) DGDM_HIP_CHECK(hipMemsetAsync(c2 + nc, 0, nc * 4, s));
            if ((rc = dgdm_unet1d_forward_cond(unet, x2, g->loopts.as<int>(), c2, e2, 2 * nb, L, s))) return rc;
            if (nc != ncond) {
                if (cond_chain_stride == 0) hipLaunchKernelGGL(repeat_rows_kernel, dim3((unsigned)((ncond + 255) / 256)), dim3(256), 0, s, global_cond_dev, c2, (int64_t)B * gc, n_chains);
                else DGDM_HIP_CHECK(hipMemcpyAsync(c2, global_cond_dev, ncond * 4, hipMemcpyDeviceToDevice, s));
            }
            if ((rc = dgdm_cfg_mix(e2, e2 + n, cfg_weight, g->loopeps.as<float>(), (int64_t)n, s))) return rc;
        } else if ((rc = dgdm_unet1d_forward_cond(unet, x, g->loopts.as<int>(), cfg == 0 ? zero_rows : cond_rows, g->loopeps.as<float>(), nb, L, s))) return rc;
        if (nb != n_chains * B) {
            hipLaunchKernelGGL(repeat_rows_kernel, dim3((unsigned)((nx + 255) / 256)), dim3(256), 0, s, g->loopeps.as<float>(), g->loopgrad.as<float>(), (int64_t)per_chain, n_chains);
            DGDM_HIP_CHECK(hipMemcpyAsync(g->loopeps.p, g->loopgrad.p, nx * 4, hipMemcpyDeviceToDevice, s));
        }
        const float *xg = x;
        if (n_grad > 1) {
            hipLaunchKernelGGL(repeat_rows_kernel, dim3((unsigned)((ng + 255) / 256)), dim3(256), 0, s, x, g->loopxrep.as<float>(), (int64_t)nx, n_grad);
            xg = g->loopxrep.as<float>();
        }
        if ((rc = guidance_grad(g, kind, xg, t, objectives, rowcoef_dev, nullptr, n_chains * n_grad, g->loopgrad.as<float>(), s,
                                kind == 3 ? &emb : nullptr, si % cpe))) return rc;
        const float *cf = coef + 4 * si;
        if (same_scale) {
            if ((rc = dgdm_ddim_guided_step(x, g->loopeps.as<float>(), g->loopgrad.as<float>(), n_grad, xn, (int64_t)nx, cf[0], cf[1], cf[2], cf[3], scales[0], s))) return rc;
        } else {
            DGDM_REQUIRE(n_grad == 1, DGDM_EINVAL, "per-chain guidance scales with averaged gradients are not supported");
            for (int c = 0; c < n_chains; ++c)
                if ((rc = dgdm_ddim_guided_step(x + c * per_chain, g->loopeps.as<float>() + c * per_chain, g->loopgrad.as<float>() + c * per_chain, 1,
                                                xn + c * per_chain, (int64_t)per_chain, cf[0], cf[1], cf[2], cf[3], scales[c], s))) return rc;
        }
    }
    DGDM_HIP_CHECK(hipGetLastError());
    return DGDM_OK;
}

extern "C" int dgdm_guidance_orientation_sweep(DgdmGuidance *g, const float *x_dev, const int32_t *object_of_chain, const int64_t *starts_host,
                                               int n_chains, float *logits_dev, void *stream) {
    DGDM_REQUIRE(g && x_dev && object_of_chain && logits_dev, DGDM_EINVAL, "dgdm_guidance_orientation_sweep: null argument");
    DGDM_REQUIRE(n_chains > 0 && n_chains <= g->cfg.max_chains, DGDM_EINVAL, "n_chains %d outside 1..%d", n_chains, g->cfg.max_chains);
    hipStream_t s = (hipStream_t)stream;
    const int kind = g->m->kind;
    int rc;
    if ((rc = g->check_objects(object_of_chain, n_chains))) return rc;
    if ((rc = g->common_pre(x_dev, 0.f, object_of_chain, n_chains, s))) return rc;
    TrunkParams p;
    g->m->fill_trunk(&p);
    g->set_grid(&p, g->sweep, n_chains);
    if (kind == 3) {
        DGDM_REQUIRE(starts_host, DGDM_EINVAL, "3-D sweep needs the FPS start indices");
        DgdmGuidance::Embedded emb;
        if ((rc = g->embed_rows(object_of_chain, n_chains, starts_host, g->sweep.rows, 1, 0, false, &emb, s))) return rc;
        emb.point(&p, *g, 0, g->sweep.rows);
    }
    p.logits = logits_dev;
    return trunk_launch(kind, false, true, p, s);
}

extern "C" int dgdm_guidance_rollout(DgdmGuidance *g, const float *x_dev, const int32_t *object_of_chain, const int64_t *starts_host,
                                     const double scale[3], int n_interactions, int n_chains, double *final_dev, float *first_logits_dev,
                                     int32_t *left_dev, double *traj_pose_dev, float *traj_logits_dev, void *stream) {
    DGDM_REQUIRE(g && x_dev && object_of_chain && scale && final_dev && first_logits_dev && left_dev, DGDM_EINVAL, "dgdm_guidance_rollout: null argument");
    DGDM_REQUIRE(!g->bf16, DGDM_EINVAL, "dgdm_guidance_rollout: the bf16 trunk has no forward-only form (contraction dtypes f32 / f32_f16x3)");
    DGDM_REQUIRE(!g->f32_mfma, DGDM_EINVAL, "dgdm_guidance_rollout: the float32 MFMA trunk has no per-row pose form (contraction dtypes f32 / f32_f16x3)");
    DGDM_REQUIRE(n_interactions >= 1, DGDM_EINVAL, "dgdm_guidance_rollout: %d interactions (at least 1)", n_interactions);
    DGDM_REQUIRE(n_chains > 0 && n_chains <= g->cfg.max_chains, DGDM_EINVAL, "n_chains %d outside 1..%d", n_chains, g->cfg.max_chains);
    int rc;
    if ((rc = g->check_objects(object_of_chain, n_chains))) return rc;
    hipStream_t s = (hipStream_t)stream;
    const int kind = g->m->kind, K = n_interactions, W1 = g->m->W1, G = g->sweep.cells;
    DGDM_REQUIRE(kind == 2 || starts_host, DGDM_EINVAL, "3-D roll-out needs the FPS start indices");
    const int64_t Rs = g->sweep.rows, rows = (int64_t)n_chains * Rs;
    const int ntiles = n_chains * g->B * g->sweep.tiles_per_b;
    if ((rc = g->rollstate.alloc((size_t)rows * 3 * sizeof(double))) || (rc = g->rolltiles.alloc((size_t)ntiles * 32 * W1 * sizeof(float))) ||
        (kind == 3 && (rc = g->rollpmax.alloc((size_t)ntiles * 32 * sizeof(float)))) ||
        (!traj_logits_dev && (rc = g->rolllogits.alloc((size_t)rows * 3 * sizeof(float)))))
        return rc;
    if ((rc = g->common_pre(x_dev, 0.f, object_of_chain, n_chains, s))) return rc;
    TrunkParams p;
    g->m->fill_trunk(&p);
    DgdmGuidance::Embedded emb;
    if (kind == 3 && (rc = g->embed_rows(object_of_chain, n_chains, starts_host, Rs, K, (int64_t)n_chains * 2 * Rs, false, &emb, s))) return rc;
    TrunkF16Scales sc;
    g->m->fill_trunk_f16(&p, &sc);
    g->set_grid(&p, g->sweep, n_chains);
    p.Ptab = nullptr; p.PtabT = g->rolltiles.as<float>(); p.Pmax = kind == 3 ? g->rollpmax.as<float>() : nullptr;
    double *state = g->rollstate.as<double>();
    if ((rc = rollout_start(g->sweep_ori.as<float>(), n_chains, g->B, G, state, left_dev, traj_pose_dev, s))) return rc;
    g->rolltiles_chains = n_chains;
    for (int k = 0; k < K; ++k) {
        if ((rc = rollout_pose_table(state, g->m->blob64.at(g->m->off64.w1p_wt), W1, n_chains, g->B, G, g->rolltiles.as<float>(), p.Pmax ? g->rollpmax.as<float>() : nullptr, s)))
            return rc;
        p.logits = traj_logits_dev ? traj_logits_dev + (size_t)k * rows * 3 : g->rolllogits.as<float>();
        if (kind == 3) emb.point(&p, *g, k, Rs);
        if ((rc = trunk_f16l_launch(kind, TrunkF16Mode::ForwardRowPose, p, sc, s))) return rc;
        if ((rc = rollout_update(p.logits, scale, k, rows, state, left_dev, traj_pose_dev ? traj_pose_dev + (size_t)(k + 1) * rows * 3 : nullptr,
                                 k == K - 1 ? final_dev : nullptr, k == 0 ? first_logits_dev : nullptr, s)))
            return rc;
    }
    return DGDM_OK;
}

extern "C" int dgdm_guidance_debug_rollout_table(DgdmGuidance *g, int n_chains, float *rollout_tiles_dev, float *sweep_tiles_dev,
                                                 int32_t *tiles_per_finger, int32_t *width, void *stream) {
    DGDM_REQUIRE(g && n_chains > 0 && n_chains <= g->cfg.max_chains, DGDM_EINVAL, "dgdm_guidance_debug_rollout_table: bad argument");
    if (tiles_per_finger) *tiles_per_finger = g->sweep.tiles_per_b;
    if (width) *width = g->m->W1;
    const size_t per_tile = (size_t)g->m->W1 * 32 * sizeof(float);
    if (rollout_tiles_dev) {
        DGDM_REQUIRE(n_chains <= g->rolltiles_chains, DGDM_EINVAL, "dgdm_guidance_debug_rollout_table: the last roll-out had %d chains", g->rolltiles_chains);
        DGDM_HIP_CHECK(hipMemcpyAsync(rollout_tiles_dev, g->rolltiles.p, (size_t)n_chains * g->B * g->sweep.tiles_per_b * per_tile, hipMemcpyDeviceToDevice, (hipStream_t)stream));
    }
    if (sweep_tiles_dev)
        DGDM_HIP_CHECK(hipMemcpyAsync(sweep_tiles_dev, g->sweep.tiled.p, (size_t)g->sweep.tiles_per_b * per_tile, hipMemcpyDeviceToDevice, (hipStream_t)stream));
    return DGDM_OK;
}

namespace {

struct CloudGroup { std::vector<int> rows; };

int pointnet_rows(DgdmDynamics *m, const float *xyz_dev , const int64_t *s1, const int64_t *s2, float *emb_dev, int rows,
                  int N, hipStream_t s) {
    DGDM_REQUIRE(N > 0 && N <= 1024, DGDM_EINVAL, "clouds of %d points unsupported (1..1024)", N);
    std::vector<float> host((size_t)rows * 3 * N);
    DGDM_HIP_CHECK(hipMemcpyAsync(host.data(), xyz_dev, host.size() * 4, hipMemcpyDeviceToHost, s));
    DGDM_HIP_CHECK(hipStreamSynchronize(s));
    std::unordered_map<std::string, int> seen;
    std::vector<CloudGroup> groups;
    std::vector<int> rep;
    for (int r = 0; r < rows; ++r) {
        std::string key(reinterpret_cast<const char *>(host.data() + (size_t)r * 3 * N), (size_t)3 * N * 4);
        auto it = seen.find(key);
        int gid;
        if (it == seen.end()) {
            gid = (int)groups.size();
            seen.emplace(std::move(key), gid);
            groups.emplace_back();
            rep.push_back(r);
        } else {
            gid = it->second;
        }
        groups[gid].rows.push_back(r);
    }
    const PnWeights w = m->pn();
    DevBuf xyz, fps1, F1, U, Y, L2, Z, vlist, slotmap, starts, chains, out, crowded, clist, poff, pairs, prank;
    int rc;
    const PnWeights64 w64 = m->pn64();
    if ((rc = xyz.alloc((size_t)N * 12)) || (rc = fps1.alloc((size_t)N * 512 * 4)) || (rc = F1.alloc((size_t)N * 128 * 8)) || (rc = U.alloc((size_t)N * 128 * 8)) ||
        (rc = Y.alloc((size_t)N * N * 1024)) || (rc = chains.alloc(sizeof(XobjChain))) || (rc = crowded.alloc((size_t)N * 4)) ||
        (rc = clist.alloc((size_t)(N + 1) * 4)) || (rc = poff.alloc((size_t)(N + 1) * 4)) || (rc = pairs.alloc((size_t)N * N * 4)) ||
        (rc = prank.alloc((size_t)N * N * 2)))
        return rc;
    for (size_t gi = 0; gi < groups.size(); ++gi) {
        const std::vector<int> &rws = groups[gi].rows;
        std::vector<float> pts((size_t)N * 3);
        const float *src = host.data() + (size_t)rep[gi] * 3 * N;
        for (int i = 0; i < N; ++i) { pts[3 * i] = src[i]; pts[3 * i + 1] = src[N + i]; pts[3 * i + 2] = src[2 * N + i]; }
        std::vector<int> slot_of(N, -1), vl, st(2 * rws.size());
        for (size_t k = 0; k < rws.size(); ++k) {
            const int64_t a = s1[rws[k]], b = s2[rws[k]];
            DGDM_REQUIRE(a >= 0 && a < N && b >= 0 && b < 512, DGDM_EINVAL, "FPS start out of range");
            if (slot_of[a] < 0) { slot_of[a] = (int)vl.size(); vl.push_back((int)a); }
            st[2 * k] = (int)a; st[2 * k + 1] = (int)b;
        }
        const int nv = (int)vl.size();
        if ((rc = xyz.upload(pts.data(), pts.size() * 4)) || (rc = vlist.upload(vl.data(), vl.size() * 4)) ||
            (rc = slotmap.upload(slot_of.data(), slot_of.size() * 4)) || (rc = starts.upload(st.data(), st.size() * 4)) ||
            (rc = L2.alloc((size_t)nv * N * 1024)) || (rc = Z.alloc((size_t)nv * N * 1024)) || (rc = out.alloc(rws.size() * 1024)))
            return rc;
        const float *x = xyz.as<float>();
        if ((rc = pn_fps_table(x, N, N, 512, fps1.as<int>(), nullptr, s))) return rc;
        if ((rc = pn_sa1_64(x, N, w.r1sq, w64, F1.as<double>(), s))) return rc;
        if ((rc = linear64(nullptr, F1.as<double>(), 128, w64.sa2_wf_t, w64.sa2_b0, nullptr, 1, U.as<double>(), nullptr, 128, N, 128, 128, ACT_NONE, s))) return rc;
        if ((rc = pn_crowd(x, N, w, crowded.as<int>(), clist.as<int>(), clist.as<int>() + N, poff.as<int>(), pairs.as<int>(), prank.as<short>(), s))) return rc;
        if ((rc = pn_pairs64(x, N, U.as<double>(), w64, pairs.as<int>(), poff.as<int>(), Y.as<float>(), s))) return rc;
        if ((rc = pn_l2(x, N, w, fps1.as<int>(), vlist.as<int>(), nv, Y.as<float>(), L2.as<float>(), clist.as<int>(), clist.as<int>() + N,
                        poff.as<int>(), prank.as<short>(), false, s))) return rc;
        if ((rc = pn_z64(x, N, nv, w64, L2.as<float>(), Z.as<float>(), clist.as<int>(), clist.as<int>() + N, s))) return rc;
        XobjChain ch{};
        ch.xyz = x; ch.fps1 = fps1.as<int>(); ch.slot_of_start = slotmap.as<int>(); ch.Z = Z.as<float>(); ch.fps2 = nullptr; ch.flags = nullptr; ch.crowded = crowded.as<int>(); ch.N = N;
        DGDM_HIP_CHECK(hipMemcpyAsync(chains.p, &ch, sizeof ch, hipMemcpyHostToDevice, s));
        XobjParams xp{};
        xp.chains = chains.as<XobjChain>(); xp.starts = starts.as<int>(); xp.xobj = out.as<float>(); xp.R = (int64_t)rws.size(); xp.total_rows = xp.R;
        if ((rc = pn_xobj(xp, false, s))) return rc;
// ... 48 lines not shown
```

### dgdm_amd/csrc/host_util.hip

```cpp
#include "common.h"
#include "blob.h"
#include <cmath>
#include <cstdarg>
#include <cstring>

namespace dgdm {

static thread_local std::string g_err;

void set_error(const char *fmt, ...) {
    char buf[1024];
    va_list ap;
    va_start(ap, fmt);
    vsnprintf(buf, sizeof buf, fmt, ap);
    va_end(ap);
    g_err = buf;
}

const float *StateDict::f32(const std::string &k, int64_t numel) const {
    auto it = m.find(k);
    if (it == m.end()) { set_error("state_dict key '%s' missing", k.c_str()); return nullptr; }
    if (it->second->dtype != 0 || it->second->numel != numel) {
        set_error("state_dict key '%s': expected %lld float32 values, got %lld (dtype %d)", k.c_str(), (long long)numel,
                  (long long)it->second->numel, it->second->dtype);
        return nullptr;
    }
    return static_cast<const float *>(it->second->data);
}

int fold_linear(const StateDict &sd, const std::string &lin, const std::string &bn, int out, int in, Folded *dst) {
    const float *w = sd.f32(lin + ".weight", (int64_t)out * in);
    const float *b = sd.f32(lin + ".bias", out);
    if (!w || !b) return DGDM_EKEY;
    dst->out = out; dst->in = in;
    dst->w.resize((size_t)out * in);
    dst->b.resize(out);
    if (bn.empty()) {
        memcpy(dst->w.data(), w, sizeof(float) * out * in);
        memcpy(dst->b.data(), b, sizeof(float) * out);
        return DGDM_OK;
    }
    const float *g = sd.f32(bn + ".weight", out), *be = sd.f32(bn + ".bias", out);
    const float *mu = sd.f32(bn + ".running_mean", out), *var = sd.f32(bn + ".running_var", out);
    if (!g || !be || !mu || !var) return DGDM_EKEY;
    for (int o = 0; o < out; ++o) {
        const double s = (double)g[o] / std::sqrt((double)var[o] + 1e-5);
        for (int i = 0; i < in; ++i) dst->w[(size_t)o * in + i] = (float)(s * (double)w[(size_t)o * in + i]);
        dst->b[o] = (float)(s * ((double)b[o] - (double)mu[o]) + (double)be[o]);
    }
    return DGDM_OK;
}

int fold_linear64(const StateDict &sd, const std::string &lin, const std::string &bn, int out, int in, Folded64 *dst) {
    const float *w = sd.f32(lin + ".weight", (int64_t)out * in);
    const float *b = sd.f32(lin + ".bias", out);
    if (!w || !b) return DGDM_EKEY;
    dst->out = out; dst->in = in;
    dst->w.resize((size_t)out * in);
    dst->b.resize(out);
    const float *g = nullptr, *be = nullptr, *mu = nullptr, *var = nullptr;
    if (!bn.empty()) {
        g = sd.f32(bn + ".weight", out); be = sd.f32(bn + ".bias", out);
        mu = sd.f32(bn + ".running_mean", out); var = sd.f32(bn + ".running_var", out);
        if (!g || !be || !mu || !var) return DGDM_EKEY;
    }
    for (int o = 0; o < out; ++o) {
        const double s = g ? (double)g[o] / std::sqrt((double)var[o] + 1e-5) : 1.0;
        for (int i = 0; i < in; ++i) dst->w[(size_t)o * in + i] = s * (double)w[(size_t)o * in + i];
        dst->b[o] = g ? s * ((double)b[o] - (double)mu[o]) + (double)be[o] : (double)b[o];
    }
    return DGDM_OK;
}

std::vector<double> transpose64(const double *src, int rows, int cols) {
    std::vector<double> t((size_t)rows * cols);
    for (int r = 0; r < rows; ++r)
        for (int c = 0; c < cols; ++c) t[(size_t)c * rows + r] = src[(size_t)r * cols + c];
    return t;
}

std::vector<double> pack_mfma64(const double *src, int M, int K) {
    const int MP = M / 32, KS = K / 4;
    std::vector<double> img((size_t)M * K);
    for (int ks = 0; ks < KS; ++ks)
        for (int mp = 0; mp < MP; ++mp)
            for (int lane = 0; lane < 64; ++lane)
                for (int j = 0; j < 2; ++j) {
                    const int m = lane & 15, kq = lane >> 4, f = 16 * (2 * mp + j) + 4 * (m & 3) + (m >> 2);
                    img[(((size_t)ks * MP + mp) * 64 + lane) * 2 + j] = src[(size_t)f * K + kq * KS + ks];
                }
    return img;
}

std::vector<float> pack_chain(const float *src, int M, int K) {
    const int MB = M / 32, KB = K / 32;
    std::vector<float> img((size_t)M * K);
    for (int op = 0; op < MB; ++op)
        for (int o = 0; o < KB; ++o)
            for (int q = 0; q < 4; ++q)
                for (int lane = 0; lane < 64; ++lane) {
                    const int i = lane & 31, h = lane >> 5;
                    const float *s = src + (size_t)(32 * op + i) * K + 32 * o + 8 * q + 4 * h;
                    float *d = img.data() + ((((size_t)op * KB + o) * 4 + q) * 64 + lane) * 4;
                    d[0] = s[0]; d[1] = s[1]; d[2] = s[2]; d[3] = s[3];
                }
    return img;
}

uint16_t f32_to_bf16(float x) {
    uint32_t u;
    memcpy(&u, &x, 4);
    if ((u & 0x7fffffffu) > 0x7f800000u) return (uint16_t)((u >> 16) | 0x40u);
    return (uint16_t)((u + 0x7fffu + ((u >> 16) & 1u)) >> 16);
}

std::vector<uint16_t> pack_chain_bf16(const float *src, int M, int K) {
    const int MB = M / 32, KB = K / 32;
    std::vector<uint16_t> img((size_t)M * K);
    for (int op = 0; op < MB; ++op)
        for (int ib = 0; ib < KB; ++ib)
            for (int s = 0; s < 2; ++s)
                for (int lane = 0; lane < 64; ++lane) {
                    const int i = lane & 31, h = lane >> 5;
                    uint16_t *d = img.data() + ((((size_t)op * KB + ib) * 2 + s) * 64 + lane) * 8;
                    for (int j = 0; j < 8; ++j) {
                        const int r = 8 * s + j, f = (r & 3) + 8 * (r >> 2) + 4 * h;
                        d[j] = f32_to_bf16(src[(size_t)(32 * op + i) * K + 32 * ib + f]);
                    }
                }
    return img;
}

std::vector<float> transpose(const float *src, int rows, int cols) {
    std::vector<float> t((size_t)rows * cols);
    for (int r = 0; r < rows; ++r)
        for (int c = 0; c < cols; ++c) t[(size_t)c * rows + r] = src[(size_t)r * cols + c];
    return t;
}

struct ProfRec { hipEvent_t a, b; double work; };
static bool g_prof_on = false;
static std::vector<ProfRec> g_prof[PROF_BUCKETS];

void prof_begin(hipStream_t s, int bucket) {
    if (!g_prof_on) return;
    ProfRec r{};
    if (hipEventCreate(&r.a) != hipSuccess || hipEventCreate(&r.b) != hipSuccess) return;
    (void)hipEventRecord(r.a, s);
    g_prof[bucket].push_back(r);
}

void prof_end(hipStream_t s, int bucket, double work) {
    if (!g_prof_on || g_prof[bucket].empty()) return;
    g_prof[bucket].back().work = work;
    (void)hipEventRecord(g_prof[bucket].back().b, s);
}

}

using namespace dgdm;

extern "C" int dgdm_version(void) { return 100; }
extern "C" const char *dgdm_last_error(void) { return g_err.c_str(); }

extern "C" int dgdm_device_init(int ordinal) {
    int n = 0;
    if (hipGetDeviceCount(&n) != hipSuccess || n <= 0) { set_error("no HIP device visible"); return DGDM_ENODEVICE; }
    DGDM_REQUIRE(ordinal >= 0 && ordinal < n, DGDM_EINVAL, "device ordinal %d out of range (%d devices)", ordinal, n);
    hipDeviceProp_t prop;
    DGDM_HIP_CHECK(hipGetDeviceProperties(&prop, ordinal));
    if (strncmp(prop.gcnArchName, "gfx950", 6) != 0) {
        set_error("device %d is %s; this library is built for gfx950 (MI355X) only", ordinal, prop.gcnArchName);
        return DGDM_ENODEVICE;
    }
    DGDM_HIP_CHECK(hipSetDevice(ordinal));
    return DGDM_OK;
}

extern "C" int dgdm_prof_enable(int on) {
    g_prof_on = on != 0;
    for (auto &b : g_prof) {
        for (auto &r : b) { (void)hipEventDestroy(r.a); (void)hipEventDestroy(r.b); }
        b.clear();
    }
    return DGDM_OK;
}

extern "C" int dgdm_prof_read_stage(int stage, int64_t *launches, double *total_ms, double *total_work) {
    DGDM_REQUIRE(stage >= 0 && stage < PROF_BUCKETS, DGDM_EINVAL, "dgdm_prof_read_stage: stage %d outside 0..%d", stage, PROF_BUCKETS - 1);
    double ms = 0, fl = 0;
    int64_t n = 0;
    for (auto &r : g_prof[stage]) {
        DGDM_HIP_CHECK(hipEventSynchronize(r.b));
        float t = 0;
        DGDM_HIP_CHECK(hipEventElapsedTime(&t, r.a, r.b));
        ms += t; fl += r.work; ++n;
        (void)hipEventDestroy(r.a); (void)hipEventDestroy(r.b);
    }
    g_prof[stage].clear();
    if (launches) *launches = n;
    if (total_ms) *total_ms = ms;
    if (total_work) *total_work = fl;
    return DGDM_OK;
}

extern "C" int dgdm_prof_read(int64_t *launches, double *total_ms, double *total_flops) {
    return dgdm_prof_read_stage(DGDM_STAGE_TRUNK, launches, total_ms, total_flops);
}

extern "C" int dgdm_objective_from_name(const char *name, DgdmObjective *out) {
    DGDM_REQUIRE(name && out, DGDM_EINVAL, "dgdm_objective_from_name: null argument");
    struct Row { const char *n; float l0, l1, l2; };
    static const Row rows[] = {
        {"rotate_clockwise", -1, 0, 0}, {"rotate_counterclockwise", 1, 0, 0}, {"shift_up", 0, -1, 0}, {"shift_down", 0, 1, 0},
        {"shift_left", 0, 0, -1}, {"shift_right", 0, 0, 1}, {"clockwise_up", -1, -1, 0}, {"clockwise_down", -1, 1, 0},
        {"clockwise_left", -1, 0, -1}, {"clockwise_right", -1, 0, 1}, {"counterclockwise_up", 1, -1, 0},
        {"counterclockwise_down", 1, 1, 0}, {"counterclockwise_left", 1, 0, -1}, {"counterclockwise_right", 1, 0, 1},
    };
    const int obj = out->object;
    memset(out, 0, sizeof *out);
    out->object = obj;
    if (!strcmp(name, "rotate")) { out->quad[0] = 1.f; return DGDM_OK; }
    if (!strcmp(name, "convergence")) { out->use_rowcoef = 1; return DGDM_OK; }
    for (const Row &r : rows)
        if (!strcmp(name, r.n)) { out->lin[0] = r.l0; out->lin[1] = r.l1; out->lin[2] = r.l2; return DGDM_OK; }
    set_error("opt obj not supported: %s", name);
    return DGDM_EOBJECTIVE;
}

static void add_slice(float *coef, int64_t base, int64_t n, bool has_start, int64_t start, bool has_stop, int64_t stop, float sign) {
    int64_t lo = 0, hi = n;
    if (has_start) { lo = start < 0 ? start + n : start; lo = lo < 0 ? 0 : (lo > n ? n : lo); }
    if (has_stop) { hi = stop < 0 ? stop + n : stop; hi = hi < 0 ? 0 : (hi > n ? n : hi); }
    for (int64_t i = lo; i < hi; ++i) coef[base + i] += sign;
}

static void add_slicer(float *coef, int64_t base, int64_t n, int64_t lower, int64_t upper, float sign) {
    if (lower < 0) {
        add_slice(coef, base, n, true, lower, false, 0, sign);
        add_slice(coef, base, n, false, 0, true, upper, sign);
    } else if (upper > n) {
        add_slice(coef, base, n, true, lower, false, 0, sign);
        add_slice(coef, base, n, false, 0, true, upper - n, sign);
    } else {
        add_slice(coef, base, n, true, lower, true, upper, sign);
    }
}

extern "C" int dgdm_convergence_rowcoef(const int64_t *centers, int n_centers, int grid_size, int num_pos, int64_t total_rows,
                                        int64_t sub_batch_size, float *rowcoef) {
    DGDM_REQUIRE(centers && rowcoef && n_centers >= 0 && total_rows >= 0, DGDM_EINVAL, "dgdm_convergence_rowcoef: bad argument");
    const int64_t pp = (int64_t)num_pos * num_pos, cells = (int64_t)grid_size * pp, half = (int64_t)(grid_size / 2) * pp;
    for (int64_t i = 0; i < total_rows; ++i) rowcoef[i] = 0.f;
    const int64_t sb = sub_batch_size > 0 ? sub_batch_size : (total_rows > 0 ? total_rows : 1);
    for (int64_t s0 = 0; s0 < total_rows; s0 += sb) {
        const int64_t n_call = std::min(sb, total_rows - s0);
        for (int i = 0; i < n_centers; ++i) {
            int64_t a0 = (int64_t)i * cells, a1 = a0 + cells;
            a0 = std::min(a0, n_call); a1 = std::min(a1, n_call);
            const int64_t n = a1 - a0, c = centers[i] * pp;
            add_slicer(rowcoef, s0 + a0, n, c - half, c, +1.f);
            add_slicer(rowcoef, s0 + a0, n, c, c + half, -1.f);
        }
    }
    return DGDM_OK;
}
```

### dgdm_amd/csrc/smallnet.hip

```cpp
#include "common.h"
#include "smallnet.h"

#pragma clang fp contract(off)

namespace dgdm {

template <int ACT, int RB>
__global__ __launch_bounds__(256) void linear_kernel(const float *__restrict__ X, int ldx, const float *__restrict__ WT,
                                                     const float *__restrict__ bias, const float *__restrict__ rowbias,
                                                     int rb_div, float *__restrict__ Y, int ldy, int rows, int K, int N,
                                                     int accumulate) {
    constexpr int KC = 128;
    __shared__ __attribute__((aligned(16))) float xs[RB][KC];
    const int r0 = blockIdx.x * RB;
    const int n = blockIdx.y * 256 + threadIdx.x;
    const int nn = min(n, N - 1);
    float acc[RB];
#pragma unroll
    for (int r = 0; r < RB; ++r) acc[r] = 0.f;
    for (int k0 = 0; k0 < K; k0 += KC) {
        const int kc = min(KC, K - k0);
        __syncthreads();
        for (int i = threadIdx.x; i < RB * KC; i += 256) {
            const int r = i / KC, k = i - r * KC;
// ... 8 lines not shown
            for (int r = 0; r < RB; ++r) {
                const float4 x = *reinterpret_cast<const float4 *>(&xs[r][k]);
                acc[r] = fmaf(x.w, w3, fmaf(x.z, w2, fmaf(x.y, w1, fmaf(x.x, w0, acc[r]))));
            }
        }
    }
    if (n >= N) return;
    const float bn = bias ? bias[n] : 0.f;
#pragma unroll
    for (int r = 0; r < RB; ++r) {
        if (r0 + r >= rows) break;
        float v = acc[r] + bn;
        if (rowbias) v += rowbias[(size_t)((r0 + r) / rb_div) * N + n];
        if (accumulate) v += Y[(size_t)(r0 + r) * ldy + n];
        if (ACT == ACT_RELU) v = fmaxf(v, 0.f);
        if (ACT == ACT_SILU) v = v / (1.f + expf(-v));
        Y[(size_t)(r0 + r) * ldy + n] = v;
    }
}

template <int RB>
static void linear_launch(const float *X, int ldx, const float *WT, const float *bias, const float *rowbias, int rb_div, float *Y, int ldy,
                          int rows, int K, int N, int act, bool accumulate, hipStream_t s) {
    dim3 grid((rows + RB - 1) / RB, (N + 255) / 256);
    if (act == ACT_NONE)
        hipLaunchKernelGGL((linear_kernel<ACT_NONE, RB>), grid, dim3(256), 0, s, X, ldx, WT, bias, rowbias, rb_div, Y, ldy, rows, K, N, (int)accumulate);
    else if (act == ACT_RELU)
        hipLaunchKernelGGL((linear_kernel<ACT_RELU, RB>), grid, dim3(256), 0, s, X, ldx, WT, bias, rowbias, rb_div, Y, ldy, rows, K, N, (int)accumulate);
    else
        hipLaunchKernelGGL((linear_kernel<ACT_SILU, RB>), grid, dim3(256), 0, s, X, ldx, WT, bias, rowbias, rb_div, Y, ldy, rows, K, N, (int)accumulate);
}

int linear(const float *X, int ldx, const float *WT, const float *bias, const float *rowbias, int rb_div, float *Y, int ldy,
           int rows, int K, int N, int act, bool accumulate, hipStream_t s) {
    if (rows <= 0) return DGDM_OK;
    if (rows >= 64) linear_launch<32>(X, ldx, WT, bias, rowbias, rb_div, Y, ldy, rows, K, N, act, accumulate, s);
    else linear_launch<8>(X, ldx, WT, bias, rowbias, rb_div, Y, ldy, rows, K, N, act, accumulate, s);
    DGDM_HIP_CHECK(hipGetLastError());
    return DGDM_OK;
}

__global__ void pose_embed_kernel(const float *__restrict__ ori, const float *__restrict__ pos, float *__restrict__ out, int rows) {
    const int r = blockIdx.x * blockDim.x + threadIdx.x;
    if (r >= rows) return;
    const float o = ori[r], px = pos[2 * r], py = pos[2 * r + 1];
    float *e = out + (size_t)r * 27;
    e[0] = o;
    e[9] = px; e[10] = py;
    float f = 1.f;
#pragma unroll
    for (int k = 0; k < 4; ++k) {
        e[1 + 2 * k] = sinf(o * f);
        e[2 + 2 * k] = cosf(o * f);
        e[11 + 4 * k] = sinf(px * f); e[12 + 4 * k] = sinf(py * f);
        e[13 + 4 * k] = cosf(px * f); e[14 + 4 * k] = cosf(py * f);
        f *= 2.f;
    }
}

__global__ void tile_table_kernel(const float *__restrict__ T, int rows, int W, float4 *__restrict__ out, int64_t total) {
    const int64_t e = (int64_t)blockIdx.x * blockDim.x + threadIdx.x;
    if (e >= total) return;
    const int lane = (int)(e & 63), n = lane & 31, h = lane >> 5;
    const int64_t t = e >> 6;
    const int q = (int)(t & 3);
    const int wb = W / 32;
    const int o = (int)((t >> 2) % wb);
    const int64_t g = (t >> 2) / wb;
    const int64_t r = min((int64_t)32 * g + n, (int64_t)rows - 1);
    out[e] = *reinterpret_cast<const float4 *>(T + r * W + 32 * o + 8 * q + 4 * h);
}

int tile_table(const float *T, int rows, int W, float *out, hipStream_t s) {
    const int64_t total = (int64_t)((rows + 31) / 32) * (W / 32) * 4 * 64;
    hipLaunchKernelGGL(tile_table_kernel, dim3((unsigned)((total + 255) / 256)), dim3(256), 0, s, T, rows, W, reinterpret_cast<float4 *>(out), total);
    DGDM_HIP_CHECK(hipGetLastError());
    return DGDM_OK;
}

int pose_embed(const float *ori, const float *pos, float *out, int rows, hipStream_t s) {
    if (rows <= 0) return DGDM_OK;
    hipLaunchKernelGGL(pose_embed_kernel, dim3((rows + 255) / 256), dim3(256), 0, s, ori, pos, out, rows);
    DGDM_HIP_CHECK(hipGetLastError());
    return DGDM_OK;
}

__global__ void time_embed_kernel(const float *__restrict__ t, float t_scalar, const float *__restrict__ freqs, float *__restrict__ out,
                                  int rows, int half) {
    const int i = blockIdx.x * blockDim.x + threadIdx.x;
    if (i >= rows * half) return;
    const int r = i / half, j = i - r * half;
    const float a = (t ? t[r] : t_scalar) * freqs[j];
    out[(size_t)r * 2 * half + j] = cosf(a);
    out[(size_t)r * 2 * half + half + j] = sinf(a);
}

int time_embed(const float *t_dev, float t_scalar, const float *freqs, float *out, int rows, int half, hipStream_t s) {
    if (rows <= 0) return DGDM_OK;
    hipLaunchKernelGGL(time_embed_kernel, dim3((rows * half + 255) / 256), dim3(256), 0, s, t_dev, t_scalar, freqs, out, rows, half);
    DGDM_HIP_CHECK(hipGetLastError());
    return DGDM_OK;
}

template <int W1>
__global__ __launch_bounds__(256) void dyn_post_kernel(const float *__restrict__ partial, int tiles_per_b,
                                                       const float *__restrict__ w1c ,
                                                       const float *__restrict__ g2w ,
                                                       const float *__restrict__ g0w ,
                                                       const float *__restrict__ V ,
                                                       float *__restrict__ grad , int L) {
    __shared__ float da[W1];
    __shared__ float v1[256];
    __shared__ float v2[256];
    const int row = blockIdx.x, t = threadIdx.x;
    for (int f = t; f < W1; f += 256) {
        const float *src = partial + (size_t)row * tiles_per_b * W1 + f;
        float acc = 0.f;
        for (int ct = 0; ct < tiles_per_b; ++ct) acc += src[(size_t)ct * W1];
        da[f] = acc;
    }
    __syncthreads();
    float acc = 0.f;
    for (int f = 0; f < W1; ++f) acc = fmaf(w1c[(size_t)f * 256 + t], da[f], acc);
    v1[t] = acc;
    __syncthreads();
    acc = 0.f;
    for (int f = 0; f < 256; ++f) acc = fmaf(g2w[(size_t)f * 256 + t], v1[f], acc);
    v2[t] = V[(size_t)row * 256 + t] > 0.f ? acc : 0.f;
    __syncthreads();
    if (t < L) {
        acc = 0.f;
        for (int f = 0; f < 256; ++f) acc = fmaf(g0w[(size_t)f * L + t], v2[f], acc);
        grad[(size_t)row * L + t] = acc;
    }
}

int dyn_post(int W1, const float *partial, int tiles_per_b, const float *w1c, const float *g2w, const float *g0w, const float *V,
             float *grad, int rows, int L, hipStream_t s) {
    if (rows <= 0) return DGDM_OK;
    DGDM_REQUIRE(L <= 256, DGDM_EINVAL, "params_ch %d > 256 not supported", L);
    if (W1 == 256)
        hipLaunchKernelGGL(dyn_post_kernel<256>, dim3(rows), dim3(256), 0, s, partial, tiles_per_b, w1c, g2w, g0w, V, grad, L);
    else
        hipLaunchKernelGGL(dyn_post_kernel<512>, dim3(rows), dim3(256), 0, s, partial, tiles_per_b, w1c, g2w, g0w, V, grad, L);
    DGDM_HIP_CHECK(hipGetLastError());
    return DGDM_OK;
}

template <int ACT, int RB>
__global__ __launch_bounds__(256) void linear64_kernel(const float *__restrict__ Xf, const double *__restrict__ Xd, int ldx,
                                                       const double *__restrict__ WT, const double *__restrict__ bias,
                                                       const double *__restrict__ rowbias, int rb_div, double *__restrict__ Yd,
                                                       float *__restrict__ Yf, int ldy, int rows, int K, int N) {
    constexpr int KC = 64;
    __shared__ double xs[RB][KC];
    const int r0 = blockIdx.x * RB;
    const int n = blockIdx.y * 256 + threadIdx.x;
    const int nn = min(n, N - 1);
    double acc[RB];
#pragma unroll
    for (int r = 0; r < RB; ++r) acc[r] = 0.0;
    for (int k0 = 0; k0 < K; k0 += KC) {
        const int kc = min(KC, K - k0);
        __syncthreads();
        for (int i = threadIdx.x; i < RB * KC; i += 256) {
            const int r = i / KC, k = i - r * KC;
            double v = 0.0;
            if (r0 + r < rows && k < kc) v = Xd ? Xd[(size_t)(r0 + r) * ldx + k0 + k] : (double)Xf[(size_t)(r0 + r) * ldx + k0 + k];
            xs[r][k] = v;
        }
        __syncthreads();
        const double *wp = WT + (size_t)k0 * N + nn;
        for (int k = 0; k < kc; k += 8) {
            double w[8];
#pragma unroll
            for (int j = 0; j < 8; ++j) w[j] = wp[(size_t)min(k + j, kc - 1) * N];
#pragma unroll
            for (int j = 0; j < 8; ++j) {
                if (k + j < kc) {
#pragma unroll
                    for (int r = 0; r < RB; ++r) acc[r] = fma(xs[r][k + j], w[j], acc[r]);
                }
            }
        }
    }
    if (n >= N) return;
    const double bn = bias ? bias[n] : 0.0;
#pragma unroll
    for (int r = 0; r < RB; ++r) {
        if (r0 + r >= rows) break;
        double v = acc[r] + bn;
        if (rowbias) v += rowbias[(size_t)((r0 + r) / rb_div) * N + n];
        if (ACT == ACT_RELU) v = fmax(v, 0.0);
        if (ACT == ACT_SILU) v = v / (1.0 + exp(-v));
        if (Yd) Yd[(size_t)(r0 + r) * ldy + n] = v;
        if (Yf) Yf[(size_t)(r0 + r) * ldy + n] = (float)v;
    }
}

int linear64(const float *Xf, const double *Xd, int ldx, const double *WT, const double *bias, const double *rowbias, int rb_div,
             double *Yd, float *Yf, int ldy, int rows, int K, int N, int act, hipStream_t s) {
    if (rows <= 0) return DGDM_OK;
    constexpr int RB = 8;
    dim3 grid((rows + RB - 1) / RB, (N + 255) / 256);
    if (act == ACT_NONE)
        hipLaunchKernelGGL((linear64_kernel<ACT_NONE, RB>), grid, dim3(256), 0, s, Xf, Xd, ldx, WT, bias, rowbias, rb_div, Yd, Yf, ldy, rows, K, N);
    else if (act == ACT_RELU)
        hipLaunchKernelGGL((linear64_kernel<ACT_RELU, RB>), grid, dim3(256), 0, s, Xf, Xd, ldx, WT, bias, rowbias, rb_div, Yd, Yf, ldy, rows, K, N);
    else
        hipLaunchKernelGGL((linear64_kernel<ACT_SILU, RB>), grid, dim3(256), 0, s, Xf, Xd, ldx, WT, bias, rowbias, rb_div, Yd, Yf, ldy, rows, K, N);
    DGDM_HIP_CHECK(hipGetLastError());
    return DGDM_OK;
}

__global__ void gather_add64_kernel(const double *__restrict__ a, const int *__restrict__ idx, const double *__restrict__ b,
                                    double *__restrict__ out, int groups, int N) {
    const int i = blockIdx.x * blockDim.x + threadIdx.x;
    if (i >= groups * N) return;
    const int g = i / N, n = i - g * N;
    out[i] = a[(size_t)idx[g] * N + n] + b[n];
}

int gather_add64(const double *a, const int *idx, const double *b, double *out, int groups, int N, hipStream_t s) {
    if (groups <= 0) return DGDM_OK;
    hipLaunchKernelGGL(gather_add64_kernel, dim3((groups * N + 255) / 256), dim3(256), 0, s, a, idx, b, out, groups, N);
    DGDM_HIP_CHECK(hipGetLastError());
    return DGDM_OK;
}

template <int W1>
__global__ __launch_bounds__(256) void dyn_post64_kernel(const float *__restrict__ partial, int tiles_per_b,
                                                         const double *__restrict__ w1c ,
                                                         const double *__restrict__ g2w ,
                                                         const double *__restrict__ g0w ,
                                                         const double *__restrict__ V ,
                                                         float *__restrict__ grad , int L) {
    __shared__ double da[W1];
    __shared__ double v1[256];
    __shared__ double v2[256];
    const int row = blockIdx.x, t = threadIdx.x;
    for (int f = t; f < W1; f += 256) {
        const float *src = partial + (size_t)row * tiles_per_b * W1 + f;
        double acc = 0.0;
        for (int ct = 0; ct < tiles_per_b; ++ct) acc += (double)src[(size_t)ct * W1];
        da[f] = acc;
    }
    __syncthreads();
    auto dot = [&](const double *__restrict__ w, int ld, const double *x, int F) {
        double acc = 0.0;
        for (int f = 0; f < F; f += 8) {
            double wv[8];
#pragma unroll
            for (int j = 0; j < 8; ++j) wv[j] = w[(size_t)(f + j) * ld + t];
#pragma unroll
            for (int j = 0; j < 8; ++j) acc = fma(wv[j], x[f + j], acc);
        }
        return acc;
    };
    v1[t] = dot(w1c, 256, da, W1);
    __syncthreads();
    const double a2 = dot(g2w, 256, v1, 256);
    v2[t] = V[(size_t)row * 256 + t] > 0.0 ? a2 : 0.0;
    __syncthreads();
    if (t < L) grad[(size_t)row * L + t] = (float)dot(g0w, L, v2, 256);
}

int dyn_post64(int W1, const float *partial, int tiles_per_b, const double *w1c, const double *g2w, const double *g0w, const double *V64,
               float *grad, int rows, int L, hipStream_t s) {
    if (rows <= 0) return DGDM_OK;
    DGDM_REQUIRE(L <= 256, DGDM_EINVAL, "params_ch %d > 256 not supported", L);
    if (W1 == 256)
        hipLaunchKernelGGL(dyn_post64_kernel<256>, dim3(rows), dim3(256), 0, s, partial, tiles_per_b, w1c, g2w, g0w, V64, grad, L);
    else
        hipLaunchKernelGGL(dyn_post64_kernel<512>, dim3(rows), dim3(256), 0, s, partial, tiles_per_b, w1c, g2w, g0w, V64, grad, L);
    DGDM_HIP_CHECK(hipGetLastError());
    return DGDM_OK;
}

__global__ void ddim_step_kernel(const float *__restrict__ x, const float *__restrict__ eps, const float *__restrict__ grad,
                                 int n_grad, float *__restrict__ out, int64_t n, float sa, float sb, float sap, float sbp,
                                 float scale) {
    const int64_t i = (int64_t)blockIdx.x * blockDim.x + threadIdx.x;
    if (i >= n) return;
    float e = eps[i];
    if (grad) {
        float g = grad[i];
        if (n_grad > 1) {
            g = 0.f + g;
            for (int k = 1; k < n_grad; ++k) g += grad[(size_t)k * n + i];
            g = g / (float)n_grad;
        }
        e = sub_rn(e, mul_rn(mul_rn(sb, g), scale));
    }
    float x0 = __fdiv_rn(sub_rn(x[i], mul_rn(sb, e)), sa);
    x0 = fminf(fmaxf(x0, -1.f), 1.f);
    out[i] = add_rn(mul_rn(sap, x0), mul_rn(sbp, e));
}

__global__ void add_noise_kernel(const float *__restrict__ x0, const float *__restrict__ noise, float *__restrict__ out, int64_t n,
                                 float sa, float sb) {
    const int64_t i = (int64_t)blockIdx.x * blockDim.x + threadIdx.x;
    if (i < n) out[i] = add_rn(mul_rn(sa, x0[i]), mul_rn(sb, noise[i]));
}

}

extern "C" int dgdm_ddim_guided_step(const float *x_dev, const float *eps_dev, const float *grad_dev, int n_grad, float *x_next_dev,
                                     int64_t n, float sqrt_abar_t, float sqrt_1m_abar_t, float sqrt_abar_prev,
                                     float sqrt_1m_abar_prev, float guidance_scale, void *stream) {
    DGDM_REQUIRE(x_dev && eps_dev && x_next_dev && n >= 0, DGDM_EINVAL, "dgdm_ddim_guided_step: null argument");
    if (n == 0) return DGDM_OK;
    dgdm::prof_begin((hipStream_t)stream, DGDM_STAGE_DDIM);
    hipLaunchKernelGGL(dgdm::ddim_step_kernel, dim3((unsigned)((n + 255) / 256)), dim3(256), 0, (hipStream_t)stream, x_dev, eps_dev,
                       grad_dev, n_grad, x_next_dev, n, sqrt_abar_t, sqrt_1m_abar_t, sqrt_abar_prev, sqrt_1m_abar_prev, guidance_scale);
    dgdm::prof_end((hipStream_t)stream, DGDM_STAGE_DDIM, (double)n * 4.0 * (3 + n_grad));
    DGDM_HIP_CHECK(hipGetLastError());
    return DGDM_OK;
}

extern "C" int dgdm_ddim_add_noise(const float *x0_dev, const float *noise_dev, float *out_dev, int64_t n, float sqrt_abar,
                                   float sqrt_1m_abar, void *stream) {
    DGDM_REQUIRE(x0_dev && noise_dev && out_dev && n >= 0, DGDM_EINVAL, "dgdm_ddim_add_noise: null argument");
    if (n == 0) return DGDM_OK;
    hipLaunchKernelGGL(dgdm::add_noise_kernel, dim3((unsigned)((n + 255) / 256)), dim3(256), 0, (hipStream_t)stream, x0_dev, noise_dev,
                       out_dev, n, sqrt_abar, sqrt_1m_abar);
    DGDM_HIP_CHECK(hipGetLastError());
    return DGDM_OK;
}
```

### dgdm_amd/engine.py

```python
from __future__ import annotations

import ctypes as C
import os
from typing import Dict, List, Optional, Sequence, Tuple

import numpy as np
import torch

from . import _lib
from ._lib import check, dptr, lib, stream_ptr


def _f32(t: torch.Tensor) -> torch.Tensor:
    return t.detach().to(dtype=torch.float32).contiguous()


def check_global_cond(global_cond: Optional[torch.Tensor], gc: int, rows: int, what: str = "global_cond") -> Optional[torch.Tensor]:
    if gc == 0:
        if global_cond is not None:
            raise ValueError(f"{what}: this eps-net has global_cond_dim 0 and takes no condition")
        return None
    if global_cond is None:
        raise ValueError(f"{what}: this eps-net has global_cond_dim {gc} and needs a condition of shape ({rows}, {gc})")
    if global_cond.dim() != 2 or global_cond.shape[1] != gc:
# ... 113 lines not shown

    def step(self, x0, noise, sqrt_abar, sqrt_1m_abar, timesteps, lr: float, want_pred: bool = False, want_loss: bool = True, global_cond=None):
        c = self._cond(global_cond, x0.shape[0])
        a = self._args(x0, noise, sqrt_abar, sqrt_1m_abar, timesteps)
        B = a[0].shape[0]
        pred = torch.empty_like(a[0]) if want_pred else None
        loss = C.c_float()
        check(lib().dgdm_unet_trainer_step_cond(self._h, *[dptr(v) for v in a], dptr(c), B, float(lr), dptr(pred), C.byref(loss) if want_loss else None,
                                                stream_ptr()))
        return (float(loss.value) if want_loss else None), (pred.reshape(B, -1, 1) if want_pred else None)

    def forward_backward(self, x0, noise, sqrt_abar, sqrt_1m_abar, timesteps, total_samples: Optional[int] = None, backward: bool = True,
                         want_pred: bool = False, global_cond=None):
        c = self._cond(global_cond, x0.shape[0])
        a = self._args(x0, noise, sqrt_abar, sqrt_1m_abar, timesteps)
        B = a[0].shape[0]
        pred = torch.empty_like(a[0]) if want_pred else None
        loss = C.c_float()
        check(lib().dgdm_unet_trainer_forward_backward_cond(self._h, *[dptr(v) for v in a], dptr(c), B, int(total_samples or B), 1 if backward else 0,
                                                            dptr(pred), C.byref(loss), stream_ptr()))
        return float(loss.value), (pred.reshape(B, -1, 1) if want_pred else None)

    def gradient_count(self) -> int:
        return int(lib().dgdm_unet_trainer_gradient_count(self._h))

    def read_gradients(self) -> torch.Tensor:
        flat = torch.empty(self.gradient_count(), dtype=torch.float32, device=torch.device("cuda", torch.cuda.current_device()))
        check(lib().dgdm_unet_trainer_gradients(self._h, dptr(flat), flat.numel(), 0, 1.0, stream_ptr()))
        return flat

    def write_gradients(self, flat: torch.Tensor, scale: float = 1.0) -> None:
        check(lib().dgdm_unet_trainer_gradients(self._h, dptr(flat), flat.numel(), 1, float(scale), stream_ptr()))

    def apply(self, lr: float) -> None:
        check(lib().dgdm_unet_trainer_apply(self._h, float(lr), stream_ptr()))

    def ema_step(self, decay: float) -> None:
        check(lib().dgdm_unet_trainer_ema_step(self._h, float(decay), float(1 - decay), stream_ptr()))

    def steps(self) -> int:
        return int(lib().dgdm_unet_trainer_steps(self._h))

    def export(self, which: int = 0) -> Dict[str, torch.Tensor]:
        host = {k: torch.empty(shp, dtype=torch.float32) for k, shp in self._keys.items()}
        packed = _lib.PackedStateDict(host)
        check(lib().dgdm_unet_trainer_export(self._h, which, packed.array, packed.n))
        return {n.decode(): torch.from_numpy(a.copy()).reshape(self._keys[n.decode()]) for n, a in zip(packed.names, packed.keep)}

    def load(self, which: int, state_dict: Dict[str, torch.Tensor], adam_steps: int = -1) -> None:
        packed = _lib.PackedStateDict(state_dict)
        check(lib().dgdm_unet_trainer_import(self._h, which, packed.array, packed.n, adam_steps))


class Dynamics:

    def __init__(self, kind: int, state_dict: Dict[str, torch.Tensor], params_ch: int, object_ch: int = 0):
        packed = _lib.PackedStateDict(state_dict)
        h = C.c_void_p()
        check(lib().dgdm_dynamics_create(C.byref(h), kind, packed.array, packed.n, params_ch, object_ch))
        self._h, self.kind, self.params_ch, self.object_ch = h, kind, params_ch, object_ch

    def __del__(self):
        if getattr(self, "_h", None) and lib is not None:
            lib().dgdm_dynamics_destroy(self._h)
            self._h = None

    def forward2d(self, x_ctrl, x_ori, x_pos, timesteps, object_vertices) -> torch.Tensor:
        rows = x_ctrl.shape[0]
        a = [_f32(v) for v in (x_ctrl, x_ori, x_pos, timesteps, object_vertices)]
        out = torch.empty((rows, 3), dtype=torch.float32, device=a[0].device)
        check(lib().dgdm_dyn2d_forward(self._h, *[dptr(v) for v in a], dptr(out), rows, stream_ptr()))
        return out

    @staticmethod
    def _starts(s: torch.Tensor) -> np.ndarray:
        return np.ascontiguousarray(s.detach().cpu().numpy().astype(np.int64))

    def pointnet2(self, xyz: torch.Tensor, start_sa1: torch.Tensor, start_sa2: torch.Tensor) -> torch.Tensor:
        x = _f32(xyz)
        rows, _, N = x.shape
        s1, s2 = self._starts(start_sa1), self._starts(start_sa2)
        out = torch.empty((rows, 256), dtype=torch.float32, device=x.device)
        check(lib().dgdm_pointnet2_forward(self._h, dptr(x), s1.ctypes.data, s2.ctypes.data, dptr(out), rows, N, stream_ptr()))
        return out

    def forward3d(self, x_ctrl, x_ori, x_pos, timesteps, xyz, start_sa1, start_sa2) -> torch.Tensor:
        rows, _, N = xyz.shape
        a = [_f32(v) for v in (x_ctrl, x_ori, x_pos, timesteps, xyz)]
        s1, s2 = self._starts(start_sa1), self._starts(start_sa2)
        out = torch.empty((rows, 3), dtype=torch.float32, device=a[0].device)
        check(lib().dgdm_dyn3d_forward(self._h, *[dptr(v) for v in a], s1.ctypes.data, s2.ctypes.data, dptr(out), rows, N, stream_ptr()))
        return out


def debug_pointnet_indices(dyn: "Dynamics", cloud: torch.Tensor, perm: Optional[torch.Tensor] = None) -> Dict[str, np.ndarray]:
    x = _f32(cloud)
    N = x.shape[0]
    pm = (torch.arange(N) if perm is None else perm).to(device=x.device, dtype=torch.int32).contiguous()
    mk = lambda *shape: torch.empty(shape, dtype=torch.int32, device=x.device)
    out = dict(fps512=mk(N, 512), fps128=mk(N, 128), fps128_flags=mk(N), ball1=mk(N, 32), ball2=mk(N, 64), ball2_count=mk(N), crowded=mk(N))
    check(lib().dgdm_debug_pointnet_indices(dyn._h, dptr(x), N, dptr(pm), pm.numel(), *[dptr(v) for v in out.values()], stream_ptr()))
    return {k: v.cpu().numpy() for k, v in out.items()}


def make_objective(name: Optional[str], object_index: int = 0, row_field: bool = False, lin: Sequence[float] = (0.0, 0.0, 0.0),
                   quad: Sequence[float] = (0.0, 0.0, 0.0)) -> _lib.Objective:
    o = _lib.Objective()
    o.object = object_index
    if row_field:
        if name is not None:
            raise ValueError("a row-field objective has no reference name (pass name=None)")
        for j in range(3):
            o.lin[j], o.quad[j] = float(lin[j]), float(quad[j])
        o.use_rowcoef = _lib.OBJ_ROWFIELD
        return o
    check(lib().dgdm_objective_from_name(name.encode(), C.byref(o)))
    return o


class Guidance:

    def __init__(self, dyn: Dynamics, batch: int, grid_size: int, num_pos: int, ori_range: Sequence[float], max_chains: int,
                 num_train_timesteps: int, num_object_points: int, sub_batch_size: int = 0, max_objects: int = 8,
                 contraction_dtype: str = "f32"):
        cfg = _lib.GuidanceConfig(batch, grid_size, num_pos, float(ori_range[0]), float(ori_range[1]), max_chains,
                                  num_train_timesteps, sub_batch_size, num_object_points, max_objects)
        h = C.c_void_p()
        check(lib().dgdm_guidance_create(C.byref(h), dyn._h, C.byref(cfg)))
        self._h, self.dyn, self.cfg = h, dyn, cfg
        self.rows = int(lib().dgdm_guidance_rows(h))
        self.starts_per_call = int(lib().dgdm_guidance_starts_per_call(h))
        self.sweep_rows = batch * grid_size
        self.n_objects = 0
        self._row_field: Optional[torch.Tensor] = None
        self.set_contraction_dtype(contraction_dtype)

    def set_contraction_dtype(self, dtype: str) -> None:
        codes = {"f32": 0, "bf16": 1, "f32_mfma": 2, "f32_f16x3": 3}
        if dtype not in codes:
            raise ValueError(f"contraction dtype {dtype!r} not supported")
        check(lib().dgdm_guidance_set_contraction_dtype(self._h, codes[dtype]))
        self.contraction_dtype = dtype

    def __del__(self):
        if getattr(self, "_h", None) and lib is not None:
            lib().dgdm_guidance_destroy(self._h)
            self._h = None

    def set_objects(self, objects: torch.Tensor, wait: bool = False) -> None:
        o = _f32(objects)
        check(lib().dgdm_guidance_set_objects(self._h, dptr(o), o.shape[0], stream_ptr()))
        self._objects_ref = o
        if wait:
            torch.cuda.current_stream().synchronize()
        self.n_objects = o.shape[0]

    def debug_fps_path(self, mode):
        ok = (C.c_int32 * max(1, self.n_objects))()
        check(lib().dgdm_guidance_debug_fps_path(self._h, int(mode), ok))
        return [bool(v) for v in ok][:self.n_objects]

    def debug_partials(self, n_chains: int) -> torch.Tensor:
        tp, w = C.c_int32(), C.c_int32()
        check(lib().dgdm_guidance_debug_partials(self._h, n_chains, None, C.byref(tp), C.byref(w), stream_ptr()))
        out = torch.empty((n_chains, self.cfg.batch, tp.value, w.value), dtype=torch.float32, device="cuda")
        check(lib().dgdm_guidance_debug_partials(self._h, n_chains, dptr(out), None, None, stream_ptr()))
        return out

    def rowcoef(self, centers: torch.Tensor) -> np.ndarray:
        c = np.ascontiguousarray(centers.detach().cpu().numpy().astype(np.int64))
        out = np.empty(self.rows, dtype=np.float32)
        sub = self.cfg.sub_batch_size if self.dyn.kind == 3 else 0
        check(lib().dgdm_convergence_rowcoef(c.ctypes.data, len(c), self.cfg.grid_size, self.cfg.num_pos, self.rows, sub, out.ctypes.data))
        return out

    def goal_field(self, goals: torch.Tensor, specs: Sequence[_lib.GoalSpec]) -> torch.Tensor:
        dev = torch.device("cuda", torch.cuda.current_device())
        gl = torch.as_tensor(goals).detach().to(device=dev, dtype=torch.float32).contiguous()
        n = len(specs)
        if gl.shape != (n, self.cfg.batch, 3):
            raise ValueError(f"goal_field: goals of shape {tuple(gl.shape)} for {n} specs (need ({n}, {self.cfg.batch}, 3))")
        arr = (_lib.GoalSpec * n)(*specs)
        out = torch.empty((n, self.rows, 3), dtype=torch.float32, device=dev)
        _check_value(lib().dgdm_guidance_goal_field(self._h, dptr(gl), arr, n, dptr(out), stream_ptr()))
        return out

    def set_row_field(self, field: Optional[torch.Tensor]) -> None:
        if field is None:
            check(lib().dgdm_guidance_set_row_field(self._h, None, 0, stream_ptr()))
            self._row_field = None
            return
        if not (field.is_cuda and field.dtype == torch.float32 and field.is_contiguous() and field.dim() == 3 and
                tuple(field.shape[1:]) == (self.rows, 3)):
            raise ValueError(f"set_row_field: a contiguous float32 device tensor (n, {self.rows}, 3) expected, got {tuple(field.shape)} {field.dtype}")
        check(lib().dgdm_guidance_set_row_field(self._h, dptr(field), field.shape[0], stream_ptr()))
        self._row_field = field

    def grad(self, x: torch.Tensor, timestep: int, objectives: Sequence[_lib.Objective], rowcoef: Optional[torch.Tensor] = None,
             starts: Optional[np.ndarray] = None) -> torch.Tensor:
        x = _f32(x)
        nc = x.shape[0]
        assert nc == len(objectives)
        arr = (_lib.Objective * nc)(*objectives)
        out = torch.empty_like(x)
        rc_ptr = dptr(rowcoef) if rowcoef is not None else None
        if self.dyn.kind == 2:
            check(lib().dgdm_dyn2d_guidance_grad(self._h, dptr(x), int(timestep), arr, rc_ptr, nc, dptr(out), stream_ptr()))
        else:
            assert starts is not None and starts.dtype == np.int64 and starts.size == nc * self.starts_per_call
            starts = np.ascontiguousarray(starts)
            check(lib().dgdm_dyn3d_guidance_grad(self._h, dptr(x), int(timestep), arr, rc_ptr, starts.ctypes.data, nc, dptr(out), stream_ptr()))
        return out

    def score(self, x: torch.Tensor, object_of_chain: Sequence[int], threshold_std: Sequence[float], timestep: int = 0,
              starts: Optional[np.ndarray] = None, want_logits: bool = False):
        x = _f32(x)
        nc, B = x.shape[0], self.cfg.batch
        oc = (C.c_int32 * nc)(*[int(o) for o in object_of_chain])
        thr = (C.c_float * 3)(*[float(v) for v in threshold_std])
        counts = torch.empty((nc, B, 3, 3, 3), dtype=torch.int32, device=x.device)
        sums = torch.empty((nc, B, 4), dtype=torch.float32, device=x.device)
        logits = torch.empty((nc, self.rows, 3), dtype=torch.float32, device=x.device) if want_logits else None
        sp = None
        if self.dyn.kind == 3:
            assert starts is not None and starts.dtype == np.int64 and starts.size == nc * self.starts_per_call
            starts = np.ascontiguousarray(starts)
            sp = starts.ctypes.data
        check(lib().dgdm_guidance_score(self._h, dptr(x), int(timestep), oc, sp, thr, nc, dptr(logits), dptr(counts), dptr(sums), stream_ptr()))
        return (counts, sums, logits) if want_logits else (counts, sums)

    def sweep(self, x: torch.Tensor, object_of_chain: Sequence[int], starts: Optional[np.ndarray] = None) -> torch.Tensor:
        x = _f32(x)
        nc = x.shape[0]
        oc = (C.c_int32 * nc)(*object_of_chain)
        out = torch.empty((nc, self.sweep_rows, 3), dtype=torch.float32, device=x.device)
        sp = None
        if self.dyn.kind == 3:
            assert starts is not None and starts.dtype == np.int64 and starts.size == nc * 2 * self.sweep_rows
            starts = np.ascontiguousarray(starts)
            sp = starts.ctypes.data
        check(lib().dgdm_guidance_orientation_sweep(self._h, dptr(x), oc, sp, nc, dptr(out), stream_ptr()))
        return out

    def rollout(self, x: torch.Tensor, object_of_chain: Sequence[int], std: Sequence[float], n_interactions: int,
                starts: Optional[np.ndarray] = None, want_trajectory: bool = False):
        from .dynamics.dataloader import POS_NORM
        x = _f32(x)
        nc, K, R = x.shape[0], int(n_interactions), self.sweep_rows
        oc = (C.c_int32 * nc)(*[int(o) for o in object_of_chain])
        scale = (C.c_double * 3)(float(std[0]) / np.pi, float(std[1]) / POS_NORM, float(std[2]) / POS_NORM)
        dev = x.device
        final = torch.empty((nc, R, 3), dtype=torch.float64, device=dev)
        first = torch.empty((nc, R, 3), dtype=torch.float32, device=dev)
        left = torch.empty((nc, R), dtype=torch.int32, device=dev)
        tp = torch.empty((max(K, 0) + 1, nc, R, 3), dtype=torch.float64, device=dev) if want_trajectory else None
        tl = torch.empty((max(K, 0), nc, R, 3), dtype=torch.float32, device=dev) if want_trajectory else None
        sp = None
        if self.dyn.kind == 3:
            assert starts is not None and starts.dtype == np.int64 and starts.size == max(K, 0) * nc * 2 * R
            starts = np.ascontiguousarray(starts)
            sp = starts.ctypes.data
        check(lib().dgdm_guidance_rollout(self._h, dptr(x), oc, sp, scale, K, nc, dptr(final), dptr(first), dptr(left), dptr(tp), dptr(tl), stream_ptr()))
        return (final, first, left, tp, tl) if want_trajectory else (final, first, left)

    def debug_rollout_table(self, n_chains: int):
        tpf, w = C.c_int32(), C.c_int32()
        check(lib().dgdm_guidance_debug_rollout_table(self._h, n_chains, None, None, C.byref(tpf), C.byref(w), stream_ptr()))
        a = torch.empty((n_chains, self.cfg.batch, tpf.value, w.value * 32), dtype=torch.float32, device="cuda")
        b = torch.empty((tpf.value, w.value * 32), dtype=torch.float32, device="cuda")
        check(lib().dgdm_guidance_debug_rollout_table(self._h, n_chains, dptr(a), dptr(b), None, None, stream_ptr()))
        return a, b


def ddim_guided_step(x: torch.Tensor, eps: torch.Tensor, grad: Optional[torch.Tensor], n_grad: int, coef: Tuple[float, float, float, float],
                     scale: float) -> torch.Tensor:
    x, eps = _f32(x), _f32(eps)
    out = torch.empty_like(x)
    g = _f32(grad) if grad is not None else None
    check(lib().dgdm_ddim_guided_step(dptr(x), dptr(eps), dptr(g), n_grad, dptr(out), x.numel(), *[float(c) for c in coef], float(scale), stream_ptr()))
    return out


def guided_chains_run(unet: "Unet1d", guid: "Guidance", noise: torch.Tensor, n_chains: int, n_grad: int, objectives: Sequence[_lib.Objective],
                      rowcoef: Optional[torch.Tensor], starts: Optional[np.ndarray], timesteps: Sequence[int],
                      coefs: Sequence[Tuple[float, float, float, float]], scales: Sequence[float], global_cond: Optional[torch.Tensor] = None,
                      cfg_weight: float = 1.0) -> torch.Tensor:
    cond, cond_stride = chain_cond_layout(global_cond, unet.global_cond_dim, n_chains, noise.shape[0])
    x0 = _f32(noise).reshape(noise.shape[0], -1)
    B, L = x0.shape
    if cond is not None:
        cond = _f32(cond).to(x0.device)
    S = len(timesteps)
    assert len(objectives) == n_chains * n_grad and len(scales) == n_chains and len(coefs) == S
    arr = (_lib.Objective * len(objectives))(*objectives)
    ts = (C.c_int32 * S)(*[int(t) for t in timesteps])
    cf = (C.c_float * (4 * S))(*[float(v) for c in coefs for v in c])
    sc = (C.c_float * n_chains)(*[float(v) for v in scales])
    sp = None
    if guid.dyn.kind == 3:
        assert starts is not None and starts.dtype == np.int64 and starts.size == S * n_chains * n_grad * guid.starts_per_call
        starts = np.ascontiguousarray(starts)
        sp = starts.ctypes.data
    out = torch.empty((n_chains, B, L), dtype=torch.float32, device=x0.device)
    check(lib().dgdm_guided_chains_run_cond(unet._h, guid._h, dptr(x0), n_chains, n_grad, arr, dptr(rowcoef) if rowcoef is not None else None, sp,
                                            ts, cf, sc, S, dptr(out), dptr(cond), int(cond_stride), float(cfg_weight), stream_ptr()))
    return out

# ... 332 lines not shown
```

### include/dgdm_hip.h

```cpp
#ifndef DGDM_HIP_H
#define DGDM_HIP_H

#include <stdint.h>

#ifdef __cplusplus
extern "C" {
#endif

#define DGDM_OK            0
#define DGDM_EINVAL       -1
#define DGDM_EKEY         -2
#define DGDM_EHIP         -3
#define DGDM_EOBJECTIVE   -4
#define DGDM_EMODE        -5
#define DGDM_ENODEVICE    -6

enum { DGDM_DTYPE_F32 = 0, DGDM_DTYPE_BF16 = 1, DGDM_DTYPE_F32_MFMA = 2, DGDM_DTYPE_F32_F16X3 = 3 };

typedef struct DgdmTensor {
    const char *name;
    const void *data;
    int64_t     numel;
    int32_t     dtype;
} DgdmTensor;

typedef struct DgdmUnet1d   DgdmUnet1d;
typedef struct DgdmDynamics DgdmDynamics;
typedef struct DgdmGuidance DgdmGuidance;

#define DGDM_OBJ_ROWFIELD 2
typedef struct DgdmObjective {
    float   lin[3];
    float   quad[3];
    int32_t use_rowcoef;
    int32_t object;
} DgdmObjective;

int         dgdm_version(void);
const char *dgdm_last_error(void);
int         dgdm_device_init(int ordinal);
int         dgdm_objective_from_name(const char *opt_obj, DgdmObjective *out);

int dgdm_unet1d_create(DgdmUnet1d **out, const DgdmTensor *state_dict, int n_tensors,
                       const int32_t *down_dims, int n_down, int step_embed_dim, int kernel_size, int n_groups);
void dgdm_unet1d_destroy(DgdmUnet1d *m);
int dgdm_unet1d_global_cond_dim(const DgdmUnet1d *m);
int dgdm_unet1d_forward(DgdmUnet1d *m, const float *sample_dev, const int32_t *timestep_dev, float *eps_dev,
                        int B, int L, void *stream);
int dgdm_unet1d_forward_cond(DgdmUnet1d *m, const float *sample_dev, const int32_t *timestep_dev, const float *global_cond_dev,
                             float *eps_dev, int B, int L, void *stream);
int dgdm_cfg_mix(const float *eps_c_dev, const float *eps_u_dev, float w, float *out_dev, int64_t numel, void *stream);
int dgdm_unet1d_set_contraction_dtype(DgdmUnet1d *m, int dtype);
int dgdm_unet1d_effective_form(const DgdmUnet1d *m, int B, int L);

int dgdm_ddim_guided_step(const float *x_dev, const float *eps_dev, const float *grad_dev, int n_grad,
                          float *x_next_dev, int64_t n, float sqrt_abar_t, float sqrt_1m_abar_t,
                          float sqrt_abar_prev, float sqrt_1m_abar_prev, float guidance_scale, void *stream);
int dgdm_ddim_add_noise(const float *x0_dev, const float *noise_dev, float *out_dev, int64_t n,
                        float sqrt_abar, float sqrt_1m_abar, void *stream);

int dgdm_dynamics_create(DgdmDynamics **out, int kind, const DgdmTensor *state_dict, int n_tensors,
                         int params_ch, int object_ch);
void dgdm_dynamics_destroy(DgdmDynamics *m);

int dgdm_dyn2d_forward(DgdmDynamics *m, const float *x_ctrl_dev, const float *x_ori_dev, const float *x_pos_dev,
                       const float *t_dev, const float *object_dev, float *logits_dev, int rows, void *stream);

int dgdm_pointnet2_forward(DgdmDynamics *m, const float *xyz_dev, const int64_t *start_sa1_host,
                           const int64_t *start_sa2_host, float *emb_dev, int rows, int N, void *stream);

int dgdm_dyn3d_forward(DgdmDynamics *m, const float *x_ctrl_dev, const float *x_ori_dev, const float *x_pos_dev,
                       const float *t_dev, const float *xyz_dev, const int64_t *start_sa1_host,
                       const int64_t *start_sa2_host, float *logits_dev, int rows, int N, void *stream);

int dgdm_farthest_point_sample(const float *xyz_dev, const int64_t *start_host, int B, int N, int npoint, int32_t *out_dev, void *stream);
int dgdm_query_ball_point(float radius_squared, int nsample, const float *xyz_dev, const float *new_xyz_dev, int B, int N, int S,
                          int32_t *out_dev, void *stream);
int dgdm_square_distance(const float *src_dev, const float *dst_dev, int B, int S, int N, float *out_dev, void *stream);
int dgdm_index_points(const float *points_dev, const int32_t *idx_dev, int B, int N, int M, int C, float *out_dev, void *stream);
int dgdm_linear_act(const float *x_dev, int ldx, const float *wt_dev, const float *bias_dev, float *y_dev, int ldy, int rows, int K, int N,
                    int act, void *stream);
int dgdm_group_max(const float *x_dev, int64_t groups, int nsample, int C, float *out_dev, void *stream);

typedef struct DgdmGuidanceConfig {
    int32_t batch;
    int32_t grid_size;
    int32_t num_pos;
    float   ori_lo, ori_hi;
    int32_t max_chains;
    int32_t num_train_timesteps;
    int32_t sub_batch_size;
    int32_t num_object_points;
    int32_t max_objects;
} DgdmGuidanceConfig;

int  dgdm_guidance_create(DgdmGuidance **out, DgdmDynamics *model, const DgdmGuidanceConfig *cfg);
void dgdm_guidance_destroy(DgdmGuidance *g);
int  dgdm_guidance_set_contraction_dtype(DgdmGuidance *g, int dtype);
int  dgdm_guidance_set_objects(DgdmGuidance *g, const float *objects_dev, int n_objects, void *stream);
int64_t dgdm_guidance_rows(const DgdmGuidance *g);
int64_t dgdm_guidance_starts_per_call(const DgdmGuidance *g);

int dgdm_dyn2d_guidance_grad(DgdmGuidance *g, const float *x_dev, int timestep, const DgdmObjective *objectives,
                             const float *rowcoef_dev, int n_chains, float *grad_dev, void *stream);
int dgdm_dyn3d_guidance_grad(DgdmGuidance *g, const float *x_dev, int timestep, const DgdmObjective *objectives,
                             const float *rowcoef_dev, const int64_t *starts_host, int n_chains, float *grad_dev,
                             void *stream);

int dgdm_guidance_set_row_field(DgdmGuidance *g, const float *field_dev, int n_chains, void *stream);

typedef struct DgdmGoalSpec { float weight[3]; float ori_window; float pos_window; int32_t profile;  } DgdmGoalSpec;
int dgdm_guidance_goal_field(DgdmGuidance *g, const float *goals_dev, const DgdmGoalSpec *specs_host, int n_chains, float *field_dev, void *stream);

int dgdm_guidance_score(DgdmGuidance *g, const float *x_dev, int timestep, const int32_t *object_of_chain,
                        const int64_t *starts_host, const float thr[3], int n_chains, float *logits_dev, int32_t *counts_dev,
                        float *sums_dev, void *stream);

int dgdm_guided_chains_run(DgdmUnet1d *unet, DgdmGuidance *g, const float *noise_dev, int n_chains, int n_grad,
                           const DgdmObjective *objectives, const float *rowcoef_dev, const int64_t *starts_host,
                           const int32_t *timesteps, const float *coef, const float *scales, int n_steps, float *x_out_dev, void *stream);
int dgdm_guided_chains_run_cond(DgdmUnet1d *unet, DgdmGuidance *g, const float *noise_dev, int n_chains, int n_grad,
                                const DgdmObjective *objectives, const float *rowcoef_dev, const int64_t *starts_host,
                                const int32_t *timesteps, const float *coef, const float *scales, int n_steps, float *x_out_dev,
                                const float *global_cond_dev, int64_t cond_chain_stride, float cfg_weight, void *stream);

int dgdm_guidance_orientation_sweep(DgdmGuidance *g, const float *x_dev, const int32_t *object_of_chain,
                                    const int64_t *starts_host, int n_chains, float *logits_dev, void *stream);

int dgdm_guidance_rollout(DgdmGuidance *g, const float *x_dev, const int32_t *object_of_chain, const int64_t *starts_host,
                          const double scale[3], int n_interactions, int n_chains, double *final_dev, float *first_logits_dev,
                          int32_t *left_dev, double *traj_pose_dev, float *traj_logits_dev, void *stream);

int dgdm_convergence_rowcoef(const int64_t *centers_host, int n_centers, int grid_size, int num_pos,
                             int64_t total_rows, int64_t sub_batch_size , float *rowcoef_host);

int dgdm_torch_rng_seed(uint8_t *state, int64_t state_bytes, uint64_t seed);
int dgdm_torch_rng_randint(uint8_t *state, int64_t state_bytes, uint32_t high, int64_t n,
                           int64_t *out_host );
int dgdm_torch_rng_fps_starts(uint8_t *state, int64_t state_bytes, int num_points, int64_t sub_batch_size, int64_t rows,
                              int64_t n_calls, int64_t *out_host ,
                              int64_t out_call_stride );

#define DGDM_DECODE_2D_SCALE 0.03f
#define DGDM_DECODE_2D_OFFSET (-0.015f)
#define DGDM_DECODE_3D_SCALE 0.05f
#define DGDM_DECODE_3D_OFFSET (-0.05f)
int dgdm_finger_decode_2d(const float *samples_dev, int batch, int num_ctrl, int num_points, float scale, float offset,
                          float *curve_dev, void *stream);
int dgdm_finger_decode_3d(const float *samples_dev, int batch, int num_ctrl, int sample_size, float scale, float offset,
                          float *surface_dev, void *stream);

typedef struct DgdmMesh DgdmMesh;
int     dgdm_mesh_read_obj(const char *path, DgdmMesh **out);
int64_t dgdm_mesh_num_vertices(const DgdmMesh *m);
int64_t dgdm_mesh_num_triangles(const DgdmMesh *m);
int     dgdm_mesh_copy(const DgdmMesh *m, double *verts_host, int32_t *tris_host);
void    dgdm_mesh_destroy(DgdmMesh *m);
int64_t dgdm_mesh_sample_workspace_bytes(const int64_t *tri_offsets_host, int num_meshes);
int     dgdm_mesh_sample_points(const double *verts_dev, const int32_t *tris_dev, const int64_t *vert_offsets_host,
                                const int64_t *tri_offsets_host, int num_meshes, uint64_t seed, const uint64_t *keys_host,
                                int64_t num_points, double *out_dev, void *workspace_dev, int64_t workspace_bytes, void *stream);

enum { DGDM_FINGER_MESH_2D = 2, DGDM_FINGER_MESH_3D = 3, DGDM_FINGER_PIECE_2D = 12, DGDM_FINGER_PIECE_3D = 13 };
int dgdm_finger_mesh_counts(int kind, int n, int64_t *verts, int64_t *tris);
int dgdm_finger_mesh_faces(int kind, int n, int32_t *tris_host);
int dgdm_finger_mesh_vertices_2d(const float *samples_dev, int batch, int num_ctrl, int num_points, float scale, float offset,
                                 float width, float height, float *verts_dev, void *stream);
int dgdm_finger_mesh_vertices_3d(const float *samples_dev, int batch, int num_ctrl, int sample_size, float scale, float offset,
                                 float width, float *verts_dev, void *stream);
int dgdm_finger_mesh_stats(const float *verts_dev, const int32_t *tris_dev, int64_t meshes, int V, int T, double area_eps,
                           double *stats_dev, void *stream);
int dgdm_finger_pieces_2d(const float *verts_dev, int batch, int num_points, int pieces, float *out_dev, double *chord_err_dev, void *stream);
int dgdm_finger_pieces_3d(const float *verts_dev, int batch, int sample_size, int pu, int pv, float *out_dev, double *chord_err_dev,
                          void *stream);
int dgdm_mesh_write_obj(const char *path, const float *verts_host, int64_t V, const int32_t *tris_host, int64_t T);

int64_t dgdm_icon_workspace_bytes(int num_images);
int dgdm_icon_trace(const uint8_t *images_dev, int num_images, int height, int width, int channels, void *workspace_dev,
                    int64_t workspace_bytes, int64_t *num_points_host, void *stream);
int dgdm_icon_fetch_contours(void *workspace_dev, int64_t workspace_bytes, int num_images, const int64_t *offsets_host,
                             int32_t *points_dev, void *resample_workspace_dev, int64_t resample_workspace_bytes, void *stream);
int64_t dgdm_contour_resample_workspace_bytes(const int64_t *offsets_host, int num_contours);
int dgdm_contour_resample(const int32_t *points_dev, const int64_t *offsets_host, int num_contours, int num_out, int rescale,
                          void *out_dev, void *workspace_dev, int64_t workspace_bytes, void *stream);

int dgdm_polygon_triangulate(const int32_t *points_dev, int batch, int n, int32_t *status_dev, int32_t *count_dev, int32_t *ring_dev,
                             int64_t *area2_dev, int32_t *triangles_dev, void *stream);
int dgdm_polygon_convex_pieces(const int32_t *points_dev, int batch, int n, int32_t *status_dev, int32_t *count_dev, int32_t *ring_dev,
                               int64_t *area2_dev, int32_t *triangles_dev, int32_t *piece_count_dev, int32_t *piece_offsets_dev,
                               int32_t *piece_index_dev, void *stream);

int64_t dgdm_render_workspace_bytes(const int64_t *vert_offsets_host, const int64_t *tri_offsets_host, int n_meshes,
                                    const int32_t *inst_mesh_host, int n_inst, int n_views);
int dgdm_render_meshes(const float *verts_dev, const int32_t *tris_dev, const int64_t *vert_offsets_host, const int64_t *tri_offsets_host,
                       int n_meshes, const int32_t *inst_view_host, const int32_t *inst_mesh_host, const float *inst_matrix_host,
                       const int32_t *inst_id_host, const float *inst_rgb_host, const float *inst_eye_host, int n_inst, int n_views,
                       int width, int height, int32_t *ids_dev, float *depth_dev, uint8_t *rgb_dev, int32_t *rejected_dev,
                       int32_t *snapped_dev, void *workspace_dev, int64_t workspace_bytes, void *stream);

enum {
    DGDM_STAGE_TRUNK = 0,
    DGDM_STAGE_UNET,
    DGDM_STAGE_XOBJ,
    DGDM_STAGE_TABLES,
    DGDM_STAGE_GUIDE_MISC,
    DGDM_STAGE_DDIM,
    DGDM_STAGE_COUNT
};
int dgdm_prof_enable(int on);
int dgdm_guidance_debug_fps_path(DgdmGuidance *g, int mode, int32_t *out_fast_ok);
int dgdm_guidance_debug_partials(DgdmGuidance *g, int n_chains, float *out_dev, int32_t *tiles_per_finger, int32_t *width, void *stream);
int dgdm_guidance_debug_rollout_table(DgdmGuidance *g, int n_chains, float *rollout_tiles_dev, float *sweep_tiles_dev,
                                      int32_t *tiles_per_finger, int32_t *width, void *stream);
int dgdm_prof_read(int64_t *launches, double *total_ms, double *total_flops);
int dgdm_prof_read_stage(int stage, int64_t *launches, double *total_ms, double *total_work);
int dgdm_debug_chain_layer(const float *W_host, const float *bias_host, const float *X_dev, float *Y_dev, void *stream);

int dgdm_debug_pointnet_indices(DgdmDynamics *m, const float *xyz_dev, int N, const int32_t *perm_dev, int perm_len,
                                int32_t *fps512_dev, int32_t *fps128_dev, int32_t *fps128_flags_dev, int32_t *ball1_dev,
                                int32_t *ball2_dev, int32_t *ball2_count_dev, int32_t *crowded_dev, void *stream);

typedef struct DgdmTrainer2d DgdmTrainer2d;
int dgdm_trainer2d_create(DgdmTrainer2d **out, const DgdmTensor *state_dict, int n_tensors, int params_ch, int object_ch,
                          float beta1, float beta2, float eps, float weight_decay);
void dgdm_trainer2d_destroy(DgdmTrainer2d *m);
int dgdm_trainer2d_step(DgdmTrainer2d *m, const float *ctrl_dev, const float *noise_dev, const float *sqrt_abar_dev,
                        const float *sqrt_1m_abar_dev, const float *t_dev, const float *ori_dev, const float *pos_dev,
                        const float *object_dev, const float *score_dev, int64_t rows, float lr, int train, float *pred_dev,
                        float *loss_host, void *stream);
typedef struct DgdmTrainGroups {
    const int32_t *t_index_dev;
    const float   *t_values_dev;
    int32_t        n_t;
    int32_t        rows_per_object;
} DgdmTrainGroups;
// ... 76 lines not shown
```

Baseline: 20420 samples/s.

## Overlap table builds and eps net on side streams; batch rows in f64 post kernel

Object table construction (FPS tables, per-object builds, readback) now runs on non-blocking build streams and is joined lazily before embedding, so it no longer blocks the main stream. The denoiser eps-net forward in the DDIM chain is forked onto a side stream so it can run beside the guidance gradient, and embedding can be hoisted out of the step loop. The f64 post-gradient kernel now handles several rows per block with double-buffered weight loads, and the f64 linear kernel prefetches weights in two halves. Debug entry points are added, plus an env switch to serialize. The extra streams and events add synchronization complexity and a risk of races.

```diff
diff --git a/dgdm_amd/_lib.py b/dgdm_amd/_lib.py
--- a/dgdm_amd/_lib.py
+++ b/dgdm_amd/_lib.py
@@ -73,6 +73,8 @@
     "dgdm_index_points": (C.c_int, [_P, _P, C.c_int, C.c_int, C.c_int, C.c_int, _P, _P]),
     "dgdm_linear_act": (C.c_int, [_P, C.c_int, _P, _P, _P, C.c_int, C.c_int, C.c_int, C.c_int, C.c_int, _P]),
     "dgdm_group_max": (C.c_int, [_P, C.c_int64, C.c_int, C.c_int, _P, _P]),
+    "dgdm_debug_linear64": (C.c_int, [_P, C.c_int, _P, _P, _P, C.c_int, C.c_int, C.c_int, C.c_int, C.c_int, _P]),
+    "dgdm_debug_dyn_post64": (C.c_int, [C.c_int, _P, C.c_int, _P, _P, _P, _P, _P, C.c_int, C.c_int, _P]),
     "dgdm_guidance_create": (C.c_int, [C.POINTER(_P), _P, C.POINTER(GuidanceConfig)]),
     "dgdm_guidance_destroy": (None, [_P]),
     "dgdm_debug_chain_layer": (C.c_int, [_P, _P, _P, _P, _P]),
diff --git a/dgdm_amd/csrc/common.h b/dgdm_amd/csrc/common.h
--- a/dgdm_amd/csrc/common.h
+++ b/dgdm_amd/csrc/common.h
@@ -96,5 +96,6 @@
 constexpr int PROF_BUCKETS = DGDM_STAGE_COUNT;
 void prof_begin(hipStream_t s, int stage);
 void prof_end(hipStream_t s, int stage, double work);
+bool prof_on();
 
 }
diff --git a/dgdm_amd/csrc/debug.hip b/dgdm_amd/csrc/debug.hip
--- a/dgdm_amd/csrc/debug.hip
+++ b/dgdm_amd/csrc/debug.hip
@@ -115,6 +115,23 @@
     return linear(x_dev, ldx, wt_dev, bias_dev, nullptr, 1, y_dev, ldy, rows, K, N, act, false, (hipStream_t)stream);
 }
 
+extern "C" int dgdm_debug_linear64(const double *x_dev, int ldx, const double *wt_dev, const double *bias_dev, double *y_dev, int ldy, int rows, int K,
+                                   int N, int act, void *stream) {
+    using namespace dgdm;
+    DGDM_REQUIRE(x_dev && wt_dev && y_dev && rows >= 0 && K > 0 && N > 0 && ldx >= K && ldy >= N, DGDM_EINVAL, "dgdm_debug_linear64: bad argument");
+    DGDM_REQUIRE(act == ACT_NONE || act == ACT_RELU || act == ACT_SILU, DGDM_EINVAL, "dgdm_debug_linear64: activation %d", act);
+    return linear64(nullptr, x_dev, ldx, wt_dev, bias_dev, nullptr, 1, y_dev, nullptr, ldy, rows, K, N, act, (hipStream_t)stream);
+}
+
+extern "C" int dgdm_debug_dyn_post64(int W1, const float *partial_dev, int tiles_per_b, const double *w1c_dev, const double *g2w_dev,
+                                     const double *g0w_dev, const double *V_dev, float *grad_dev, int rows, int L, void *stream) {
+    using namespace dgdm;
+    DGDM_REQUIRE(partial_dev && w1c_dev && g2w_dev && g0w_dev && V_dev && grad_dev && rows >= 0 && tiles_per_b > 0 && L > 0, DGDM_EINVAL,
+                 "dgdm_debug_dyn_post64: bad argument");
+    DGDM_REQUIRE(W1 == 256 || W1 == 512, DGDM_EINVAL, "dgdm_debug_dyn_post64: W1 %d (256 or 512)", W1);
+    return dyn_post64(W1, partial_dev, tiles_per_b, w1c_dev, g2w_dev, g0w_dev, V_dev, grad_dev, rows, L, (hipStream_t)stream);
+}
+
 extern "C" int dgdm_group_max(const float *x_dev, int64_t groups, int nsample, int C, float *out_dev, void *stream) {
     using namespace dgdm;
     DGDM_REQUIRE(x_dev && out_dev && groups >= 0 && nsample > 0 && C > 0, DGDM_EINVAL, "dgdm_group_max: bad argument");
diff --git a/dgdm_amd/csrc/guidance_api.hip b/dgdm_amd/csrc/guidance_api.hip
--- a/dgdm_amd/csrc/guidance_api.hip
+++ b/dgdm_amd/csrc/guidance_api.hip
@@ -67,6 +67,7 @@
     hipEvent_t bev[NBUILD] = {}, bstart = nullptr, pooled = nullptr, ldone = nullptr;
     DevBuf V, genc, atab, chainbias, timepart, ttmp, ttmp64, partial, objdev, objidx, xobj, xobj16, starts, order, xchains, todo, groupoff;
     DevBuf loopx[2], loopeps, loopgrad, loopxrep, loopts;
+    DevBuf loopeps1;
     DevBuf loopcond, loopx2, loopeps2;
     DevBuf scorelogits;
     DevBuf sweep_ori, rollstate, rolllogits, rolltiles, rollpmax;
@@ -88,7 +89,31 @@
     int *ro_host = nullptr; size_t ro_ints = 0; hipEvent_t ro_ev = nullptr; bool ro_pending = false;
     int finish_objects();
     hipStream_t cstream = nullptr; hipEvent_t up_ready = nullptr, up_consumed = nullptr; bool consumed_recorded = false;
+    int serial = 0;
+    bool tables_off_stream() const { return !(serial & 3) && !prof_on(); }
+    bool eps_beside() const { return !(serial & 5) && !prof_on(); }
+    bool hoist_x_only() const { return !(serial & 1) && !prof_on(); }
+    bool built_off_stream = false, join_pending = false, built_once = false;
+    hipStream_t joined_stream = nullptr;
+    hipEvent_t fork_ev = nullptr, side_ev = nullptr;
+    int join_tables(hipStream_t s) {
+        if (!built_off_stream || (!join_pending && s == joined_stream)) return DGDM_OK;
+        DGDM_HIP_CHECK(hipStreamWaitEvent(s, ro_ev, 0));
+        join_pending = false; joined_stream = s;
+        return DGDM_OK;
+    }
+    int side_stream(hipStream_t *side) {
+        if (!bstream[0]) DGDM_HIP_CHECK(hipStreamCreateWithFlags(&bstream[0], hipStreamNonBlocking));
+        if (!fork_ev) DGDM_HIP_CHECK(hipEventCreateWithFlags(&fork_ev, hipEventDisableTiming));
+        if (!side_ev) DGDM_HIP_CHECK(hipEventCreateWithFlags(&side_ev, hipEventDisableTiming));
+        *side = bstream[0];
+        return DGDM_OK;
+    }
     ~DgdmGuidance() {
+        for (int i = 0; i < NBUILD; ++i)
+            if (bstream[i]) (void)hipStreamSynchronize(bstream[i]);
+        if (fork_ev) (void)hipEventDestroy(fork_ev);
+        if (side_ev) (void)hipEventDestroy(side_ev);
         if (pinned) (void)hipHostFree(pinned);
         if (pinned_ev) (void)hipEventDestroy(pinned_ev);
         if (ro_host) (void)hipHostFree(ro_host);
@@ -125,7 +150,7 @@
                    bool want16, Embedded *e, hipStream_t s);
     int embed(const int *objidx_host, int n_chains, const int64_t *starts_host, int n_calls, int64_t call_stride, Embedded *e, hipStream_t s);
     int trunk_front(int kind, const float *x_dev, int timestep, const int *objidx_host, const int64_t *starts_host, int n_chains, const Embedded *emb,
-                    int call, dgdm::TrunkParams *p, hipStream_t s);
+                    int call, dgdm::TrunkParams *p, hipStream_t s, bool pre_done = false);
 };
 
 int DgdmGuidance::build_pose_table(const std::vector<float> &ori, const std::vector<float> &pos, PoseGrid *dst, hipStream_t s) {
@@ -172,6 +197,7 @@
     std::unique_ptr<DgdmGuidance> g(new DgdmGuidance());
     g->m = model; g->cfg = *cfg;
     g->B = cfg->batch;
+    if (const char *e = getenv("DGDM_SERIAL_STEP")) g->serial = atoi(e);
     const int G = cfg->grid_size, P = cfg->num_pos, C = G * P * P;
     const std::vector<float> lo = linspace_f32(cfg->ori_lo, cfg->ori_hi, G), lp = linspace_f32(-1.f, 1.f, P);
     std::vector<float> ori(C), pos(2 * (size_t)C);
@@ -357,9 +383,12 @@
             if ((rc = g->vlist.upload(v.data(), sizeof(int) * N))) return rc;
         }
         const int nb = std::min<int>(DgdmGuidance::NBUILD, n_objects);
+        const bool off = g->tables_off_stream();
+        const int ns = off ? std::max(nb, 2) : nb;
+        if (!off && (rc = g->join_tables(s))) return rc;
         if (!g->bstart) DGDM_HIP_CHECK(hipEventCreateWithFlags(&g->bstart, hipEventDisableTiming));
         if (!g->ldone) DGDM_HIP_CHECK(hipEventCreateWithFlags(&g->ldone, hipEventDisableTiming));
-        for (int i = 0; i < nb; ++i) {
+        for (int i = 0; i < ns; ++i) {
             if (!g->bstream[i]) DGDM_HIP_CHECK(hipStreamCreateWithFlags(&g->bstream[i], hipStreamNonBlocking));
             if (!g->bev[i]) DGDM_HIP_CHECK(hipEventCreateWithFlags(&g->bev[i], hipEventDisableTiming));
         }
@@ -374,8 +403,17 @@
         if (!g->pooled) DGDM_HIP_CHECK(hipEventCreateWithFlags(&g->pooled, hipEventDisableTiming));
         DGDM_HIP_CHECK(hipMemcpyAsync(g->pool_xyz.p, objects_dev, no * N * 3 * 4, hipMemcpyDeviceToDevice, s));
         DGDM_HIP_CHECK(hipEventRecord(g->pooled, s));
-        if ((rc = pn_fps_tables(g->pool_xyz.as<float>(), N, N, g->pool_fps1.as<int>(), g->pool_fps2.as<int>(), g->pool_flags.as<int>(), s, n_objects)))
+        hipStream_t fs = s;
+        if (off) {
+            fs = g->bstream[ns - 1];
+            for (int i = 1; i < ns; ++i) {
+                DGDM_HIP_CHECK(hipStreamWaitEvent(g->bstream[i], g->pooled, 0));
+                if (g->built_once) DGDM_HIP_CHECK(hipStreamWaitEvent(g->bstream[i], g->ro_ev, 0));
+            }
+        }
+        if ((rc = pn_fps_tables(g->pool_xyz.as<float>(), N, N, g->pool_fps1.as<int>(), g->pool_fps2.as<int>(), g->pool_flags.as<int>(), fs, n_objects)))
             return rc;
+        DGDM_HIP_CHECK(hipEventRecord(g->bstart, fs));
         for (int i = 0; i < n_objects; ++i) {
             ObjectTables &t = *g->tables[i];
             t.xyz = g->pool_xyz.as<float>() + (size_t)i * N * 3; t.fps1 = g->pool_fps1.as<int>() + (size_t)i * N * 512;
@@ -401,16 +439,16 @@
             }
             DGDM_HIP_CHECK(hipEventRecord(g->ldone, ls));
         }
-        DGDM_HIP_CHECK(hipEventRecord(g->bstart, s));
         for (int i = 0; i < nb; ++i) {
             DGDM_HIP_CHECK(hipStreamWaitEvent(g->bstream[i], g->bstart, 0));
             DGDM_HIP_CHECK(hipStreamWaitEvent(g->bstream[i], g->ldone, 0));
         }
         for (int i = 0; i < n_objects; ++i)
             if ((rc = g->build_object(i, i % nb, g->bstream[i % nb]))) return rc;
-        for (int i = 0; i < nb; ++i) {
+        hipStream_t es = off ? g->bstream[0] : s;
+        for (int i = off ? 1 : 0; i < nb; ++i) {
             DGDM_HIP_CHECK(hipEventRecord(g->bev[i], g->bstream[i]));
-            DGDM_HIP_CHECK(hipStreamWaitEvent(s, g->bev[i], 0));
+            DGDM_HIP_CHECK(hipStreamWaitEvent(es, g->bev[i], 0));
         }
         prof_end(s, DGDM_STAGE_TABLES, 0.0);
         const size_t need = no * N + no;
@@ -421,10 +459,11 @@
             g->ro_ints = need;
         }
         if (!g->ro_ev) DGDM_HIP_CHECK(hipEventCreateWithFlags(&g->ro_ev, hipEventDisableTiming));
-        DGDM_HIP_CHECK(hipMemcpyAsync(g->ro_host, g->pool_flags.p, sizeof(int) * no * N, hipMemcpyDeviceToHost, s));
-        DGDM_HIP_CHECK(hipMemcpyAsync(g->ro_host + no * N, g->pool_ncr.p, sizeof(int) * no, hipMemcpyDeviceToHost, s));
-        DGDM_HIP_CHECK(hipEventRecord(g->ro_ev, s));
+        DGDM_HIP_CHECK(hipMemcpyAsync(g->ro_host, g->pool_flags.p, sizeof(int) * no * N, hipMemcpyDeviceToHost, es));
+        DGDM_HIP_CHECK(hipMemcpyAsync(g->ro_host + no * N, g->pool_ncr.p, sizeof(int) * no, hipMemcpyDeviceToHost, es));
+        DGDM_HIP_CHECK(hipEventRecord(g->ro_ev, es));
         g->ro_pending = true;
+        g->built_once = true; g->built_off_stream = off; g->join_pending = off;
     }
     g->n_objects = n_objects;
     g->grads_since_set = 0;
@@ -626,6 +665,7 @@
     for (int i = 0; i < n_chains && tab; ++i) tab = want16 ? tables[oidx[i]]->has_x16 : tables[oidx[i]]->has_x;
     const int64_t rt = rows_per_call * n_calls;
     int rc;
+    if ((rc = join_tables(s))) return rc;
     if ((rc = upload_starts(starts_host, n_chains, rows_per_call, s, !tab, n_calls, call_stride))) return rc;
     if ((rc = finish_objects())) return rc;
     e->tab = tab; e->used16 = want16; e->rows_per_chain = rt;
@@ -651,6 +691,7 @@
 int DgdmGuidance::embed(const int *oidx, int n_chains, const int64_t *starts_host, int n_calls, int64_t call_stride, Embedded *e, hipStream_t s) {
     DGDM_REQUIRE(starts_host, DGDM_EINVAL, "3-D guidance needs the FPS start indices");
     int rc;
+    if ((rc = join_tables(s))) return rc;
     prof_begin(s, DGDM_STAGE_XOBJ);
     if (tables_wanted()) {
         const bool crosses = grads_since_set <= XTAB_AFTER && grads_since_set + n_calls > XTAB_AFTER;
@@ -667,13 +708,15 @@
 }
 
 int DgdmGuidance::trunk_front(int kind, const float *x_dev, int timestep, const int *oidx, const int64_t *starts_host, int n_chains, const Embedded *emb,
-                              int call, TrunkParams *pp, hipStream_t s) {
+                              int call, TrunkParams *pp, hipStream_t s, bool pre_done) {
     const float t_scaled = (float)timestep / (float)cfg.num_train_timesteps;
     int rc;
     if ((rc = check_objects(oidx, n_chains))) return rc;
-    prof_begin(s, DGDM_STAGE_GUIDE_MISC);
-    if ((rc = common_pre(x_dev, t_scaled, oidx, n_chains, s))) return rc;
-    prof_end(s, DGDM_STAGE_GUIDE_MISC, 0.0);
+    if (!pre_done) {
+        prof_begin(s, DGDM_STAGE_GUIDE_MISC);
+        if ((rc = common_pre(x_dev, t_scaled, oidx, n_chains, s))) return rc;
+        prof_end(s, DGDM_STAGE_GUIDE_MISC, 0.0);
+    }
     m->fill_trunk(pp);
     set_grid(pp, grid, n_chains);
     if (kind == 3) {
@@ -703,7 +746,7 @@
 
 static int guidance_grad(DgdmGuidance *g, int kind, const float *x_dev, int timestep, const DgdmObjective *objectives, const float *rowcoef_dev,
                          const int64_t *starts_host, int n_chains, float *grad_dev, hipStream_t s, const DgdmGuidance::Embedded *emb = nullptr,
-                         int call = 0) {
+                         int call = 0, bool pre_done = false) {
     DGDM_REQUIRE(g && x_dev && objectives && grad_dev, DGDM_EINVAL, "guidance_grad: null argument");
     if (g->m->kind != kind) { set_error("model type not supported: %d-D entry point on a %d-D model", kind, g->m->kind); return DGDM_EMODE; }
     DGDM_REQUIRE(n_chains > 0 && n_chains <= g->cfg.max_chains, DGDM_EINVAL, "n_chains %d outside 1..%d", n_chains, g->cfg.max_chains);
@@ -717,7 +760,7 @@
         tob[i].use_rowcoef = objectives[i].use_rowcoef; tob[i].pad = 0;
     }
     TrunkParams p;
-    if ((rc = g->trunk_front(kind, x_dev, timestep, oidx.data(), starts_host, n_chains, emb, call, &p, s))) return rc;
+    if ((rc = g->trunk_front(kind, x_dev, timestep, oidx.data(), starts_host, n_chains, emb, call, &p, s, pre_done))) return rc;
     DGDM_HIP_CHECK(hipMemcpyAsync(g->objdev.p, tob.data(), sizeof(TrunkObjective) * n_chains, hipMemcpyHostToDevice, s));
     p.obj = g->objdev.as<TrunkObjective>(); p.rowcoef = rowcoef_dev; p.rowfield = g->rowfield;
     p.partial = g->partial.as<float>();
@@ -889,52 +932,77 @@
     const int64_t call_stride = (int64_t)n_chains * n_grad * spc;
     int cpe = kind == 3 ? (int)std::min<int64_t>(n_steps, std::max<int64_t>(1, (((int64_t)1 << 22) - 1) / std::max<int64_t>(1, g->grid.rows))) : n_steps;
     if (const char *e = getenv("DGDM_EMBED_CALLS")) cpe = std::max(1, std::min(cpe, atoi(e)));
-    if (kind == 3) {
-        for (int i = 0; i < n_chains * n_grad; ++i) oidx[i] = objectives[i].object;
-        if ((rc = g->check_objects(oidx.data(), n_chains * n_grad))) return rc;
-    }
-    for (int si = 0; si < n_steps; ++si) {
+    for (int i = 0; i < n_chains * n_grad; ++i) oidx[i] = objectives[i].object;
+    if ((rc = g->check_objects(oidx.data(), n_chains * n_grad))) return rc;
+    DGDM_REQUIRE(same_scale || n_grad == 1, DGDM_EINVAL, "per-chain guidance scales with averaged gradients are not supported");
+    const bool hoist = g->hoist_x_only(), beside = g->eps_beside();
+    hipStream_t side = s;
+    if (beside && (rc = g->side_stream(&side))) return rc;
+    if ((rc = g->loopeps1.alloc(per_chain * 4))) return rc;
+    auto step = [&](int si) -> int {
+        int rc;
         float *x = g->loopx[si & 1].as<float>(), *xn = (si + 1 == n_steps) ? x_out_dev : g->loopx[(si + 1) & 1].as<float>();
         const int t = timesteps[si];
-        if (kind == 3 && si % cpe == 0 &&
+        const bool embed_due = kind == 3 && si % cpe == 0;
+        if (embed_due && !hoist &&
             (rc = g->embed(oidx.data(), n_chains * n_grad, starts_host + (size_t)si * call_stride, std::min(cpe, n_steps - si), call_stride, &emb, s))) return rc;
         const int nb = (si == 0 && n_chains > 1 && !per_chain_cond) ? B : n_chains * B;
         const int ne = cfg == 2 ? 2 * nb : nb;
-        hipLaunchKernelGGL(fill_i32_kernel, dim3((ne + 255) / 256), dim3(256), 0, s, g->loopts.as<int>(), t, ne);
+        const bool fork = beside && !(kind == 3 && si == 0);
+        const hipStream_t es = fork ? side : s;
+        if (fork) {
+            DGDM_HIP_CHECK(hipEventRecord(g->fork_ev, s));
+            DGDM_HIP_CHECK(hipStreamWaitEvent(es, g->fork_ev, 0));
+        }
+        float *eps_dst = nb != n_chains * B ? g->loopeps1.as<float>() : g->loopeps.as<float>();
+        hipLaunchKernelGGL(fill_i32_kernel, dim3((ne + 255) / 256), dim3(256), 0, es, g->loopts.as<int>(), t, ne);
         if (cfg == 2) {
             const size_t n = (size_t)nb * L, nc = (size_t)nb * gc;
             float *x2 = g->loopx2.as<float>(), *e2 = g->loopeps2.as<float>(), *c2 = g->loopcond.as<float>();
-            DGDM_HIP_CHECK(hipMemcpyAsync(x2, x, n * 4, hipMemcpyDeviceToDevice, s));
-            DGDM_HIP_CHECK(hipMemcpyAsync(x2 + n, x, n * 4, hipMemcpyDeviceToDevice, s));
-            if (nc != ncond) DGDM_HIP_CHECK(hipMemsetAsync(c2 + nc, 0, nc * 4, s));
-            if ((rc = dgdm_unet1d_forward_cond(unet, x2, g->loopts.as<int>(), c2, e2, 2 * nb, L, s))) return rc;
+            DGDM_HIP_CHECK(hipMemcpyAsync(x2, x, n * 4, hipMemcpyDeviceToDevice, es));
+            DGDM_HIP_CHECK(hipMemcpyAsync(x2 + n, x, n * 4, hipMemcpyDeviceToDevice, es));
+            if (nc != ncond) DGDM_HIP_CHECK(hipMemsetAsync(c2 + nc, 0, nc * 4, es));
+            if ((rc = dgdm_unet1d_forward_cond(unet, x2, g->loopts.as<int>(), c2, e2, 2 * nb, L, es))) return rc;
             if (nc != ncond) {
-                if (cond_chain_stride == 0) hipLaunchKernelGGL(repeat_rows_kernel, dim3((unsigned)((ncond + 255) / 256)), dim3(256), 0, s, global_cond_dev, c2, (int64_t)B * gc, n_chains);
-                else DGDM_HIP_CHECK(hipMemcpyAsync(c2, global_cond_dev, ncond * 4, hipMemcpyDeviceToDevice, s));
+                if (cond_chain_stride == 0) hipLaunchKernelGGL(repeat_rows_kernel, dim3((unsigned)((ncond + 255) / 256)), dim3(256), 0, es, global_cond_dev, c2, (int64_t)B * gc, n_chains);
+                else DGDM_HIP_CHECK(hipMemcpyAsync(c2, global_cond_dev, ncond * 4, hipMemcpyDeviceToDevice, es));
             }
-            if ((rc = dgdm_cfg_mix(e2, e2 + n, cfg_weight, g->loopeps.as<float>(), (int64_t)n, s))) return rc;
-        } else if ((rc = dgdm_unet1d_forward_cond(unet, x, g->loopts.as<int>(), cfg == 0 ? zero_rows : cond_rows, g->loopeps.as<float>(), nb, L, s))) return rc;
-        if (nb != n_chains * B) {
-            hipLaunchKernelGGL(repeat_rows_kernel, dim3((unsigned)((nx + 255) / 256)), dim3(256), 0, s, g->loopeps.as<float>(), g->loopgrad.as<float>(), (int64_t)per_chain, n_chains);
-            DGDM_HIP_CHECK(hipMemcpyAsync(g->loopeps.p, g->loopgrad.p, nx * 4, hipMemcpyDeviceToDevice, s));
-        }
+            if ((rc = dgdm_cfg_mix(e2, e2 + n, cfg_weight, eps_dst, (int64_t)n, es))) return rc;
+        } else if ((rc = dgdm_unet1d_forward_cond(unet, x, g->loopts.as<int>(), cfg == 0 ? zero_rows : cond_rows, eps_dst, nb, L, es))) return rc;
+        if (nb != n_chains * B)
+            hipLaunchKernelGGL(repeat_rows_kernel, dim3((unsigned)((nx + 255) / 256)), dim3(256), 0, es, eps_dst, g->loopeps.as<float>(), (int64_t)per_chain, n_chains);
+        if (fork) DGDM_HIP_CHECK(hipEventRecord(g->side_ev, es));
         const float *xg = x;
         if (n_grad > 1) {
             hipLaunchKernelGGL(repeat_rows_kernel, dim3((unsigned)((ng + 255) / 256)), dim3(256), 0, s, x, g->loopxrep.as<float>(), (int64_t)nx, n_grad);
             xg = g->loopxrep.as<float>();
         }
+        if (hoist) {
+            if ((rc = g->common_pre(xg, (float)t / (float)g->cfg.num_train_timesteps, oidx.data(), n_chains * n_grad, s))) return rc;
+            if (embed_due &&
+                (rc = g->embed(oidx.data(), n_chains * n_grad, starts_host + (size_t)si * call_stride, std::min(cpe, n_steps - si), call_stride, &emb, s))) return rc;
+        }
+        if (fork) DGDM_HIP_CHECK(hipStreamWaitEvent(s, g->side_ev, 0));
         if ((rc = guidance_grad(g, kind, xg, t, objectives, rowcoef_dev, nullptr, n_chains * n_grad, g->loopgrad.as<float>(), s,
-                                kind == 3 ? &emb : nullptr, si % cpe))) return rc;
+                                kind == 3 ? &emb : nullptr, si % cpe, hoist))) return rc;
         const float *cf = coef + 4 * si;
         if (same_scale) {
             if ((rc = dgdm_ddim_guided_step(x, g->loopeps.as<float>(), g->loopgrad.as<float>(), n_grad, xn, (int64_t)nx, cf[0], cf[1], cf[2], cf[3], scales[0], s))) return rc;
         } else {
-            DGDM_REQUIRE(n_grad == 1, DGDM_EINVAL, "per-chain guidance scales with averaged gradients are not supported");
             for (int c = 0; c < n_chains; ++c)
                 if ((rc = dgdm_ddim_guided_step(x + c * per_chain, g->loopeps.as<float>() + c * per_chain, g->loopgrad.as<float>() + c * per_chain, 1,
                                                 xn + c * per_chain, (int64_t)per_chain, cf[0], cf[1], cf[2], cf[3], scales[c], s))) return rc;
         }
-    }
+        return DGDM_OK;
+    };
+    for (int si = 0; si < n_steps; ++si)
+        if ((rc = step(si))) {
+            if (beside) {
+                (void)hipEventRecord(g->side_ev, side);
+                (void)hipStreamWaitEvent(s, g->side_ev, 0);
+            }
+            return rc;
+        }
     DGDM_HIP_CHECK(hipGetLastError());
     return DGDM_OK;
 }
diff --git a/dgdm_amd/csrc/host_util.hip b/dgdm_amd/csrc/host_util.hip
--- a/dgdm_amd/csrc/host_util.hip
+++ b/dgdm_amd/csrc/host_util.hip
@@ -141,6 +141,8 @@
 struct ProfRec { hipEvent_t a, b; double work; };
 static bool g_prof_on = false;
 static std::vector<ProfRec> g_prof[PROF_BUCKETS];
+
+bool prof_on() { return g_prof_on; }
 
 void prof_begin(hipStream_t s, int bucket) {
     if (!g_prof_on) return;
diff --git a/dgdm_amd/csrc/smallnet.hip b/dgdm_amd/csrc/smallnet.hip
--- a/dgdm_amd/csrc/smallnet.hip
+++ b/dgdm_amd/csrc/smallnet.hip
@@ -184,7 +184,7 @@
                                                        const double *__restrict__ WT, const double *__restrict__ bias,
                                                        const double *__restrict__ rowbias, int rb_div, double *__restrict__ Yd,
                                                        float *__restrict__ Yf, int ldy, int rows, int K, int N) {
-    constexpr int KC = 64;
+    constexpr int KC = 64, KU = KC / 2;
     __shared__ double xs[RB][KC];
     const int r0 = blockIdx.x * RB;
     const int n = blockIdx.y * 256 + threadIdx.x;
@@ -194,6 +194,10 @@
     for (int r = 0; r < RB; ++r) acc[r] = 0.0;
     for (int k0 = 0; k0 < K; k0 += KC) {
         const int kc = min(KC, K - k0);
+        const double *wp = WT + (size_t)k0 * N + nn;
+        double w0[KU], w1[KU];
+#pragma unroll
+        for (int j = 0; j < KU; ++j) w0[j] = wp[(size_t)min(j, kc - 1) * N];
         __syncthreads();
         for (int i = threadIdx.x; i < RB * KC; i += 256) {
             const int r = i / KC, k = i - r * KC;
@@ -202,16 +206,23 @@
             xs[r][k] = v;
         }
         __syncthreads();
-        const double *wp = WT + (size_t)k0 * N + nn;
-        for (int k = 0; k < kc; k += 8) {
-            double w[8];
-#pragma unroll
-            for (int j = 0; j < 8; ++j) w[j] = wp[(size_t)min(k + j, kc - 1) * N];
-#pragma unroll
-            for (int j = 0; j < 8; ++j) {
-                if (k + j < kc) {
-#pragma unroll
-                    for (int r = 0; r < RB; ++r) acc[r] = fma(xs[r][k + j], w[j], acc[r]);
+        if (kc > KU) {
+#pragma unroll
+            for (int j = 0; j < KU; ++j) w1[j] = wp[(size_t)min(KU + j, kc - 1) * N];
+        }
+#pragma unroll
+        for (int j = 0; j < KU; ++j) {
+            if (j < kc) {
+#pragma unroll
+                for (int r = 0; r < RB; ++r) acc[r] = fma(xs[r][j], w0[j], acc[r]);
+            }
+        }
+        if (kc > KU) {
+#pragma unroll
+            for (int j = 0; j < KU; ++j) {
+                if (KU + j < kc) {
+#pragma unroll
+                    for (int r = 0; r < RB; ++r) acc[r] = fma(xs[r][KU + j], w1[j], acc[r]);
                 }
             }
         }
@@ -260,51 +271,85 @@
     return DGDM_OK;
 }
 
-template <int W1>
+template <int W1, int RB>
 __global__ __launch_bounds__(256) void dyn_post64_kernel(const float *__restrict__ partial, int tiles_per_b,
                                                          const double *__restrict__ w1c ,
                                                          const double *__restrict__ g2w ,
                                                          const double *__restrict__ g0w ,
                                                          const double *__restrict__ V ,
-                                                         float *__restrict__ grad , int L) {
-    __shared__ double da[W1];
-    __shared__ double v1[256];
-    __shared__ double v2[256];
-    const int row = blockIdx.x, t = threadIdx.x;
-    for (int f = t; f < W1; f += 256) {
-        const float *src = partial + (size_t)row * tiles_per_b * W1 + f;
+                                                         float *__restrict__ grad , int rows, int L) {
+    __shared__ __attribute__((aligned(16))) double da[W1][RB];
+    __shared__ __attribute__((aligned(16))) double v1[256][RB];
+    __shared__ __attribute__((aligned(16))) double v2[256][RB];
+    const int r0 = blockIdx.x * RB, t = threadIdx.x;
+    constexpr int CU = 12;
+    for (int i = t; i < RB * W1; i += 256) {
+        const int r = i / W1, f = i - r * W1;
+        const float *src = partial + (size_t)min(r0 + r, rows - 1) * tiles_per_b * W1 + f;
         double acc = 0.0;
-        for (int ct = 0; ct < tiles_per_b; ++ct) acc += (double)src[(size_t)ct * W1];
-        da[f] = acc;
-    }
-    __syncthreads();
-    auto dot = [&](const double *__restrict__ w, int ld, const double *x, int F) {
-        double acc = 0.0;
-        for (int f = 0; f < F; f += 8) {
-            double wv[8];
-#pragma unroll
-            for (int j = 0; j < 8; ++j) wv[j] = w[(size_t)(f + j) * ld + t];
-#pragma unroll
-            for (int j = 0; j < 8; ++j) acc = fma(wv[j], x[f + j], acc);
-        }
-        return acc;
+        for (int c0 = 0; c0 < tiles_per_b; c0 += CU) {
+            float pv[CU];
+#pragma unroll
+            for (int j = 0; j < CU; ++j) pv[j] = src[(size_t)min(c0 + j, tiles_per_b - 1) * W1];
+#pragma unroll
+            for (int j = 0; j < CU; ++j)
+                if (c0 + j < tiles_per_b) acc += (double)pv[j];
+        }
+        da[f][r] = acc;
+    }
+    __syncthreads();
+    constexpr int U = 16;
+    auto dot = [&](const double *__restrict__ w, int ld, const double (*x)[RB], int F, double (&acc)[RB]) {
+        double wa[U], wb[U];
+#pragma unroll
+        for (int r = 0; r < RB; ++r) acc[r] = 0.0;
+#pragma unroll
+        for (int j = 0; j < U; ++j) wa[j] = w[(size_t)j * ld + t];
+        for (int f = 0; f < F; f += 2 * U) {
+#pragma unroll
+            for (int j = 0; j < U; ++j) wb[j] = w[(size_t)(f + U + j) * ld + t];
+#pragma unroll
+            for (int j = 0; j < U; ++j)
+#pragma unroll
+                for (int r = 0; r < RB; ++r) acc[r] = fma(wa[j], x[f + j][r], acc[r]);
+            if (f + 2 * U < F) {
+#pragma unroll
+                for (int j = 0; j < U; ++j) wa[j] = w[(size_t)(f + 2 * U + j) * ld + t];
+            }
+#pragma unroll
+            for (int j = 0; j < U; ++j)
+#pragma unroll
+                for (int r = 0; r < RB; ++r) acc[r] = fma(wb[j], x[f + U + j][r], acc[r]);
+        }
     };
-    v1[t] = dot(w1c, 256, da, W1);
-    __syncthreads();
-    const double a2 = dot(g2w, 256, v1, 256);
-    v2[t] = V[(size_t)row * 256 + t] > 0.0 ? a2 : 0.0;
-    __syncthreads();
-    if (t < L) grad[(size_t)row * L + t] = (float)dot(g0w, L, v2, 256);
+    static_assert(W1 % (2 * U) == 0 && 256 % (2 * U) == 0, "dyn_post64_kernel: dot product lengths are multiples of 2 U");
+    double acc[RB];
+    dot(w1c, 256, da, W1, acc);
+#pragma unroll
+    for (int r = 0; r < RB; ++r) v1[t][r] = acc[r];
+    __syncthreads();
+    dot(g2w, 256, v1, 256, acc);
+#pragma unroll
+    for (int r = 0; r < RB; ++r) v2[t][r] = V[(size_t)min(r0 + r, rows - 1) * 256 + t] > 0.0 ? acc[r] : 0.0;
+    __syncthreads();
+    if (t < L) {
+        dot(g0w, L, v2, 256, acc);
+#pragma unroll
+        for (int r = 0; r < RB; ++r)
+            if (r0 + r < rows) grad[(size_t)(r0 + r) * L + t] = (float)acc[r];
+    }
 }
 
 int dyn_post64(int W1, const float *partial, int tiles_per_b, const double *w1c, const double *g2w, const double *g0w, const double *V64,
                float *grad, int rows, int L, hipStream_t s) {
     if (rows <= 0) return DGDM_OK;
     DGDM_REQUIRE(L <= 256, DGDM_EINVAL, "params_ch %d > 256 not supported", L);
+    constexpr int RB = 4;
+    const dim3 grid((rows + RB - 1) / RB);
     if (W1 == 256)
-        hipLaunchKernelGGL(dyn_post64_kernel<256>, dim3(rows), dim3(256), 0, s, partial, tiles_per_b, w1c, g2w, g0w, V64, grad, L);
+        hipLaunchKernelGGL((dyn_post64_kernel<256, RB>), grid, dim3(256), 0, s, partial, tiles_per_b, w1c, g2w, g0w, V64, grad, rows, L);
     else
-        hipLaunchKernelGGL(dyn_post64_kernel<512>, dim3(rows), dim3(256), 0, s, partial, tiles_per_b, w1c, g2w, g0w, V64, grad, L);
+        hipLaunchKernelGGL((dyn_post64_kernel<512, RB>), grid, dim3(256), 0, s, partial, tiles_per_b, w1c, g2w, g0w, V64, grad, rows, L);
     DGDM_HIP_CHECK(hipGetLastError());
     return DGDM_OK;
 }
diff --git a/dgdm_amd/engine.py b/dgdm_amd/engine.py
--- a/dgdm_amd/engine.py
+++ b/dgdm_amd/engine.py
@@ -289,7 +289,7 @@
         check(lib().dgdm_guidance_set_objects(self._h, dptr(o), o.shape[0], stream_ptr()))
         self._objects_ref = o
         if wait:
-            torch.cuda.current_stream().synchronize()
+            torch.cuda.synchronize()
         self.n_objects = o.shape[0]
 
     def debug_fps_path(self, mode):
diff --git a/include/dgdm_hip.h b/include/dgdm_hip.h
--- a/include/dgdm_hip.h
+++ b/include/dgdm_hip.h
@@ -81,6 +81,10 @@
 int dgdm_linear_act(const float *x_dev, int ldx, const float *wt_dev, const float *bias_dev, float *y_dev, int ldy, int rows, int K, int N,
                     int act, void *stream);
 int dgdm_group_max(const float *x_dev, int64_t groups, int nsample, int C, float *out_dev, void *stream);
+int dgdm_debug_linear64(const double *x_dev, int ldx, const double *wt_dev, const double *bias_dev, double *y_dev, int ldy, int rows, int K,
+                        int N, int act, void *stream);
+int dgdm_debug_dyn_post64(int W1, const float *partial_dev, int tiles_per_b, const double *w1c_dev, const double *g2w_dev,
+                          const double *g0w_dev, const double *V_dev, float *grad_dev, int rows, int L, void *stream);
 
 typedef struct DgdmGuidanceConfig {
     int32_t batch;
```

Result: faster. 21120 samples/s (median of 6 runs) (+3.4%).
